# numamma/numamma

Measured on AMD Instinct MI355X. Metric: PEBS samples/s analysed (device-resident), higher is better.
Workload: dtype u64

## Files before the change

numamma_amd/csrc/nmg_engine_impl.h:

```cpp
#pragma once

#include <dlfcn.h>
#include <hip/hip_runtime.h>
#include <rccl/rccl.h>
#include <rocprofiler-sdk-roctx/roctx.h>

#include <algorithm>
#include <chrono>
#include <cinttypes>
#include <functional>
#include <cstdio>
#include <cstdlib>
#include <cstddef>
#include <cstring>
#include <condition_variable>
#include <memory>
#include <mutex>
#include <string>
#include <thread>
#include <vector>

#include "nmg_buffer.h"
#include "nmg_kernels.h"
#include "nmg_route.h"

using namespace nmg;

struct Range {
  explicit Range(const char* what) { roctxRangePushA(what); }
  ~Range() { roctxRangePop(); }
  Range(const Range&) = delete;
  Range& operator=(const Range&) = delete;
};

struct CopyPool {
  std::vector<std::thread> workers;
  std::mutex m;
  std::condition_variable wake, idle;
  std::function<void(uint32_t)> job;
  uint64_t gen = 0;
  uint32_t pending = 0;
  bool stop = false;

  explicit CopyPool(uint32_t n) {
    for (uint32_t w = 1; w < n; w++)
      workers.emplace_back([this, w] {
        uint64_t seen = 0;
        for (;;) {
          std::function<void(uint32_t)> f;
          {
            std::unique_lock<std::mutex> lk(m);
            wake.wait(lk, [&] { return stop || gen != seen; });
            if (stop) return;
            seen = gen;
            f = job;
          }
          f(w);
          std::lock_guard<std::mutex> lk(m);
          if (--pending == 0) idle.notify_one();
        }
      });
  }
  void run(const std::function<void(uint32_t)>& f) {
    {
      std::lock_guard<std::mutex> lk(m);
      job = f;
      pending = (uint32_t)workers.size();
      gen++;
    }
    wake.notify_all();
    f(0);
    std::unique_lock<std::mutex> lk(m);
    idle.wait(lk, [&] { return pending == 0; });
  }
  ~CopyPool() {
    {
      std::lock_guard<std::mutex> lk(m);
      stop = true;
    }
    wake.notify_all();
    for (auto& t : workers) t.join();
  }
};

struct nmg_engine;

struct LookupSet {
  DevBuf<uint64_t> keys;
  DevBuf<DevEntry> nodes;
  DevBuf<uint64_t> efences;
  DevBuf<DevEntry> enodes;
  DevBuf<uint64_t> ffences;
  DevBuf<uint8_t> fshift;
  DevBuf<uint2> dir;
  DevBuf<DevEntry> own_chain;
  DevEntry* chain = nullptr;
  uint32_t K = 0, elevels = 0, nb_fences = 0, fence_log2 = 0, dir_log2 = 0;
};

struct RouteTable {
  bool ok = false;
  uint32_t nparts = 0;
  DevBuf<PartInfo> d_parts;
  DevBuf<uint64_t> d_pbounds;
  DevBuf<uint16_t> d_pdir;
  DevBuf<uint32_t> d_pdead;
  DevBuf<uint64_t> d_pe_keys;
  DevBuf<uint4> d_pe_nodes;
  DevBuf<uint4> d_pe_pnode;
  DevBuf<uint4> d_pe_old;
  DevBuf<uint32_t> d_pe_oinf;
  DevBuf<uint2> d_pe_info;
  DevBuf<uint4> d_pe_dir;
  DevBuf<uint32_t> d_pe_ids;
  DevBuf<uint32_t> d_pe_lrel;
  DevBuf<uint32_t> d_pe_cmap;
};

struct RoutePool {
  DevBuf<uint4> d_rec16;
  DevBuf<uint32_t> d_cmeta;
  DevBuf<unsigned long long> d_cmatch;
  DevBuf<uint32_t> d_clist;
  DevBuf<uint4> d_items;
  DevBuf<uint32_t> d_chunk0;
  DevBuf<uint32_t> d_used;
  DevBuf<uint32_t> d_pcnt;
  DevBuf<uint32_t> d_pbase;
  DevBuf<uint32_t> d_ctl;
  DevBuf<uint4> d_ovf16;
  DevBuf<unsigned long long> d_ovfx;
};

struct EntryTable {
  std::vector<uint64_t> hist_base;
  std::vector<uint64_t> npages;
  std::vector<uint64_t> buffer_size, entry_addr;
  std::vector<nmg_object> objects;
  std::vector<DevEntry> dev_entries;
  std::vector<uint32_t> sparse_entries;
  CellCursor cur;

  uint64_t cells() const { return cur.cells; }
  void resize(uint32_t E) {
    const size_t E0 = dev_entries.size();
    hist_base.resize(E, kHistSparse);
    npages.resize(E, 1);
    buffer_size.resize(E, 0);
    entry_addr.resize(E, 0);
    objects.resize(E, nmg_object{0, 0, 0, 0});
    dev_entries.resize(E, DevEntry{0, 0, 0, 0, kHistSparse, ~0u, 0, 0, 0, 0});
    for (size_t e = E0; e < E; e++) dev_entries[e].id = (uint32_t)e;
  }
  void truncate(uint32_t E, const CellCursor& c) {
    resize(E);
    sparse_entries.resize(c.nsparse);
    cur = c;
  }
  void describe(uint32_t id, const nmg_object& o) {
    objects[id] = o;
    buffer_size[id] = o.buffer_size;
    entry_addr[id] = o.buffer_addr;
  }
  DevEntry dev_entry(uint32_t id, const nmg_object& o) const {
    DevEntry d = dev_entries[id];
    d.addr = o.buffer_addr;
    d.end = o.buffer_addr + o.buffer_size;
    d.alloc = o.alloc_date;
    d.free = o.free_date;
    return d;
  }
  Placement place(uint32_t id, uint64_t np, bool must_be_dense) {
    DevEntry& d = dev_entries[id];
    uint64_t base = kHistSparse;
    const Placement how = cur.place(np, must_be_dense, &base, &d.sidx);
    if (how == kPlaceDense) d.hist = hist_base[id] = base;
    if (how == kPlaceSparse) sparse_entries.push_back(id);
    return how;
  }
};

struct Counters {
  DevBuf<uint64_t> d_sum64, d_min64, d_max64;
  uint64_t n_sum64 = 0, n_min64 = 0, n_max64 = 0;
  void set_sizes(uint64_t E, bool levels) {
    n_sum64 = sum64_words(E, levels);
    n_min64 = min64_words(E);
    n_max64 = max64_words();
  }
  DevBuf<uint32_t> d_hist;
  DevBuf<uint64_t> d_sparse_keys;
  DevBuf<uint32_t> d_sparse_vals;
  DevBuf<uint64_t> d_objcw;
  DevBuf<uint64_t> d_sparse_ck;
  DevBuf<uint32_t> d_sparse_dirty;
  DevBuf<unsigned long long> d_pk64;
  DevBuf<uint4> d_tlog;
  DevBuf<uint32_t> d_tlog_cnt;
};

struct CellLayout {
  uint64_t E = 0, nsent = 0;
  bool meta_dirty = true;
  DevBuf<uint64_t> d_base, d_off, d_part, d_soff;
  DevBuf<uint32_t> d_np, d_cnt, d_sent;
  int ensure(nmg_engine* h, uint64_t E, uint64_t nsent);
};

struct Timeline {
  bool on = false;
  nmg_timeline_options opt{};
  uint64_t ncells = 0;
  uint32_t rounds = kTlRounds;
  DevBuf<uint32_t> d_cells;
  std::vector<uint32_t> ids, base, nrows;
  DevBuf<uint32_t> d_ids, d_base, d_nrows;
  DevBuf<uint32_t> d_cnt, d_rows;
  DevBuf<uint64_t> d_off, d_part;
  uint64_t rows_epoch = 0;
  int64_t n = 0;
};

struct nmg_engine {
  int device = 0;
  uint32_t flags = NMG_F_DEFAULT;
  uint32_t T = 1;
  hipStream_t stream = nullptr;
  hipEvent_t ev0 = nullptr, ev1 = nullptr;
  static constexpr int kRing = 64;
  hipEvent_t ring0[kRing] = {}, ring1[kRing] = {};
  hipEvent_t ringm[kRing] = {};
  hipEvent_t ringr[kRing] = {};
  uint64_t nlaunch = 0;
  int num_cus = 256;
  int blocks_per_cu = 0;
  bool launched = false;

  bool have_table = false;
  uint64_t epoch = 1, cells_epoch = 0;
  bool counters_fresh = false;
  struct HostReg {
    uintptr_t lo, hi;
    uint64_t dev;
    void* pages;
  };
  std::vector<HostReg> hostregs;
  std::vector<uint64_t> zc_dev;
  struct ResSnap {
    hipStream_t stream = nullptr;
    hipEvent_t ready = nullptr, copied = nullptr;
    bool pending = false;
    CellLayout lay;
    DevBuf<uint64_t> d_sum, d_min, d_max, d_objcw, d_found;
    DevBuf<uint32_t> d_bufcnt;
    DevBuf<uint64_t> d_ck;
    DevBuf<uint4> d_rows;
    PinBuf<uint64_t> h_sum, h_min, h_max, h_objcw, h_small, h_soff;
    PinBuf<uint32_t> h_bufcnt;
    PinBuf<uint32_t> h_rows;
    std::vector<uint32_t> sent_entry;
  } snap;
  uint64_t snap_nb = 0;
  struct CellsPrep {
    CellLayout lay;
    DevBuf<uint4> d_rows;
    int64_t n = 0;
    std::vector<uint64_t> sparse_kv, soff;
    std::vector<uint32_t> sent_entry;
  } cprep;
  uint32_t E = 0;
  LookupSet lk;
  DevBuf<DevEntry> d_entries;
  EntryTable tab;
  std::vector<uint32_t> order;
  uint64_t hist_budget = 4ull << 30;
  uint64_t sparse_cap = 1u << 20;

  Counters cnt;
  DevBuf<unsigned long long> d_found;
  DevBuf<uint64_t> d_scratch;
  DevBuf<uint32_t> d_smatch;
  Timeline tl;
  uint64_t nreset = 0;

  std::vector<BufDesc> descs;
  std::vector<uint64_t> buf_bytes;
  PinBuf<uint8_t> h_stage;
  size_t stage_len = 0;
  DevBuf<uint8_t> d_arena;
  const uint8_t* d_data = nullptr;
  bool external = false;
  bool staged_dirty = false;
  DevBuf<BufDesc> d_descs;
  DevBuf<BufDesc> d_sdescs;
  DevBuf<uint32_t> d_ranges;
  PinBuf<uint8_t> up_pin;
  size_t up_off = 0;
  hipEvent_t up_ev = nullptr;
  bool up_recorded = false;
  uint32_t sched_grid = 0;
  bool descs_dirty = false;
  bool multi_staged = false;
  DevBuf<uint32_t> d_bufcnt;
  size_t bufcnt_stride = 0;

  struct StreamSlot {
    PinBuf<uint8_t> h_stage;
    size_t len = 0;
    DevBuf<uint8_t> d_arena;
    PinBuf<uint8_t> h_sched;
    DevBuf<uint8_t> d_sched;
    std::vector<BufDesc> descs;
    hipEvent_t copied = nullptr;
    hipEvent_t done = nullptr;
    bool used = false;
  };
  bool streaming = false, streamed = false;
  uint64_t chunk_cap = 0;
  uint32_t copy_threads = 1;
  std::unique_ptr<CopyPool> pool;
  StreamSlot slots[2];
  int cur_slot = 0;
  hipStream_t copy_stream = nullptr;

  bool counts_override = false;
  std::vector<uint32_t> ov_samples, ov_found;
  std::vector<uint64_t> ov_bytes;

  std::string last_error;
  float last_ms = 0.f;

  std::vector<nmg_engine*> workers;
  std::vector<int> devices;
  bool multi = false, multi_distinct = false, multi_pending = false;
  uint64_t multi_found = 0;
  hipEvent_t merge_ev0 = nullptr, merge_ev1 = nullptr;
  bool merge_timed = false;
  uint64_t merge_bytes = 0;
  std::vector<void*> comms;
  std::vector<DevBuf<uint8_t>> warena;

  RouteTable rt;
  uint64_t route_launches = 0;
  RSeg rsegs[kRouteSegs];
  uint64_t route_tbase = 0;
  uint32_t nrsegs = 0;
  RoutePool rpool;
  bool sched_route = false;
  uint32_t route_sched_key = 0;
  bool route_pending = false;
  uint32_t route_grid = 0;
  XLayout route_xl{};

  DevBuf<uint64_t> d_dbg;
  size_t dbg_len = 0;
};

#define HIP_TRY(h, expr)                                                        \
  do {                                                                          \
    hipError_t _e = (expr);                                                     \
    if (_e != hipSuccess) {                                                     \
      (h)->last_error = std::string(#expr) + ": " + hipGetErrorString(_e);      \
      return NMG_ERR_HIP;                                                       \
    }                                                                           \
  } while (0)

struct CopyTask {
  uint8_t* dst;
  const uint8_t* src;
  uint64_t len;
};

struct RouteJob {
  const std::vector<BufDesc>* descs;
  const uint8_t* data;
  const BufDesc* sdescs;
  const uint32_t* ranges;
  const uint32_t* chunk0;
  uint32_t grid, index_base;
  bool settle_now;
};

#pragma GCC visibility push(hidden)
extern thread_local std::string g_create_error;
int fail(nmg_engine* h, int code, const std::string& msg);
int stage_h2d(nmg_engine* h, void* d_dst, const void* src, size_t n);
void stage_reset(nmg_engine* h);
void free_table(nmg_engine* h);
template <class T>
hipError_t alloc_copy(nmg_engine* h, DevBuf<T>& b, const T* src, size_t n) {
  const hipError_t e = b.alloc(n);
  if (e != hipSuccess || !n) return e;
  return hipMemcpyAsync(b, src, n * sizeof(T), hipMemcpyHostToDevice, h->stream);
}
template <class T>
hipError_t alloc_copy(nmg_engine* h, DevBuf<T>& b, const std::vector<T>& src) {
  return alloc_copy(h, b, src.data(), src.size());
}
int check_table(nmg_engine* h, const uint64_t* keys, const uint32_t* entry_off, uint32_t nb_keys,
                       uint32_t n);
int build_lookup(nmg_engine* h, LookupSet& l, const uint64_t* keys, const uint32_t* entry_off, uint32_t nb_keys,
                 const std::vector<DevEntry>& chain, DevEntry* chain_dev);
void route_segments(const uint64_t* b, uint32_t P, RSeg* seg, uint32_t* nseg, std::vector<uint16_t>& dir);
int build_partitions(nmg_engine* h, const uint64_t* keys, const uint32_t* entry_off, uint32_t K,
                            const std::vector<DevEntry>& dev, const uint32_t* ids);
int grow_entries(nmg_engine* h, uint32_t newE, const uint32_t* ids, const nmg_object* objs, uint32_t n);
int stage_reserve(nmg_engine* h, size_t need);
int append_desc(nmg_engine* h, uint64_t len, uint32_t thread_rank, uint32_t access);
uint64_t zero_copy_dev(nmg_engine* h, const void* p, uint64_t len);
int append_desc_zc(nmg_engine* h, uint64_t dev, uint64_t len, uint32_t thread_rank, uint32_t access);
int check_buffer_args(nmg_engine* h, uint64_t len, uint32_t thread_rank, uint32_t access);
void run_copies(nmg_engine* h, const std::vector<CopyTask>& tasks);
int slot_acquire(nmg_engine* h, int s);
int ensure_bufcnt(nmg_engine* h, size_t need);
int ensure_dbg(nmg_engine* h, size_t words);
int stream_flush(nmg_engine* h);
int stream_dst(nmg_engine* h, uint64_t len, uint8_t** dst, std::vector<CopyTask>* pending);
int stream_append(nmg_engine* h, uint64_t len, uint32_t thread_rank, uint32_t access);
int upload_buffers(nmg_engine* h);
void make_schedule(const std::vector<BufDesc>& descs, uint32_t grid, uint32_t index_base, BufDesc* sorted,
                          uint32_t* ranges, bool by_stream);
int build_schedule(nmg_engine* h, uint32_t grid, bool by_stream = true);
void ensure_occupancy(nmg_engine* h);
uint32_t attribution_grid(nmg_engine* h, uint32_t nb);
Params base_params(nmg_engine* h, const uint8_t* data, const BufDesc* sdescs, const uint32_t* ranges);
int launch_events(nmg_engine* h, int* slot_out);
int launch_attribution(nmg_engine* h, const uint8_t* data, const BufDesc* sdescs, const uint32_t* ranges,
                              uint32_t nb, uint32_t grid, uint64_t nbytes);
uint32_t bits_for(uint64_t v);
bool route_layout(nmg_engine* h, const std::vector<BufDesc>& descs, XLayout& xl);
bool route_eligible(nmg_engine* h, const std::vector<BufDesc>& descs);
bool route_eligible(nmg_engine* h);
int route_pool(nmg_engine* h, const std::vector<BufDesc>& descs, uint32_t grid, const uint32_t* ranges,
                      std::vector<uint32_t>& c0);
int route_prepare(nmg_engine* h, uint32_t grid, const std::vector<uint32_t>& ranges);
int route_analyze(nmg_engine* h, uint32_t nb, uint32_t grid);
int route_analyze_job(nmg_engine* h, const RouteJob& job);
int route_settle(nmg_engine* h);
int decode_error_word(nmg_engine* h, uint64_t w);
int cells_prepare(nmg_engine* h);
int cells_fill(nmg_engine* h, uint32_t* rows);
int collect_page_cells(nmg_engine* h, std::vector<uint32_t>* rows, int64_t* count);
int timeline_prepare(nmg_engine* h);
int collect_timeline_cells(nmg_engine* h, std::vector<uint32_t>* rows, int64_t* count);
void* array_ptr(nmg_engine* h, int which, size_t* bytes);
int scratch_u64(nmg_engine* h);
int sparse_nonempty(nmg_engine* h, bool* out);
int sparse_download(nmg_engine* h, std::vector<uint64_t>& k, std::vector<uint32_t>& v);
int multi_create(nmg_engine* h, const nmg_options* opt);
void multi_destroy(nmg_engine* h);
int multi_analyze(nmg_engine* h);
int multi_finish(nmg_engine* h);
int multi_buffer_found(nmg_engine* h, std::vector<uint32_t>& nf);
#pragma GCC visibility pop
```

numamma_amd/csrc/nmg_route.h:

```cpp
#pragma once

#include "nmg_kernels.h"

namespace nmg {

constexpr uint32_t kChunk = 64;
constexpr uint32_t kPartLevels = 11;
constexpr uint32_t kMaxParts = (1u << kPartLevels) - 1;
constexpr uint32_t kRouteDir = 4096;
constexpr uint32_t kRouteSegs = 8;
constexpr uint32_t kDirCntSat = 31;
struct RSeg {
  uint64_t start;
  uint32_t base;
  uint32_t nslots;
  uint32_t shift;
  uint32_t qlast;
};
constexpr uint32_t kPartKeys = 1023;
constexpr uint32_t kPartSlots = 1024;
constexpr uint32_t kPartDir = 1024;
constexpr uint32_t kDirInline = 6;
constexpr uint32_t kPnQShift = 8;
constexpr uint32_t kPnOlder = 1u << 11, kPnExact = 1u << 12;
constexpr uint32_t kOldLds = 512;
constexpr uint32_t kPnOldLds = 1u << 13, kPnOldShift = 16;
constexpr uint32_t kPartEntries = 1536;
constexpr uint32_t kPartCells = 28672;
constexpr uint32_t kItemChunks = 1023;
static_assert((uint64_t)kItemChunks * kChunk < (1ull << (64 - kPackShift)), "packed count per item");
static_assert((uint64_t)kItemChunks * kChunk < 65536u, "a u16 page cell cannot wrap within one item");
constexpr uint32_t kChunkIdBits = 25;
constexpr uint32_t kFoundLds = 16384;
constexpr uint32_t kDbgNoRoute = 0x10000;
constexpr uint32_t kDbgTinyPool = 0x20000;
constexpr uint32_t kDbgTinyOvf = 0x80000;
constexpr uint32_t kDbgLapNoWait = 0x100000;
constexpr uint32_t kDbgLocalNoWork = 0x400000;
constexpr uint32_t kDbgRouteTiming = 0x800000;
constexpr uint32_t kDbgLocalNoObj = 0x1000000;
constexpr uint32_t kDbgLocalNoPage = 0x2000000;
constexpr uint32_t kDbgLocalNoGlobal = 0x4000000;
constexpr uint32_t kDbgLocalNoSearch = 0x8000000;
constexpr uint32_t kDbgNoLines = 0x20000000;
constexpr uint32_t kDbgLocalAtomics = 0x80000000u;
constexpr uint32_t kDbgLocalTiming = 0x10000000;
constexpr int kRouteTimingWords = 16;

struct PartInfo {
  uint32_t k0, nk, e0, ne;
  uint64_t cb;
  uint32_t span;
  uint32_t dshift;
  uint32_t pages_lds;
  uint32_t cmap;
  uint32_t pad[2];
};
static_assert(sizeof(PartInfo) == 48, "PartInfo");

constexpr uint32_t kAddrBits = 40;
constexpr uint32_t kMinWeightBits = 11;
constexpr uint32_t kTsBits = 40;
struct XLayout {
  uint32_t gbits, obits, tbits, wbits;
  uint64_t wesc;
  uint64_t tbase;
};

struct RouteParams {
  Params p;
  const uint64_t* pbounds;
  const uint16_t* pdir;
  const uint32_t* pdead;
  RSeg seg[kRouteSegs];
  uint32_t nseg;
  uint32_t nparts;
  XLayout xl;
  uint64_t seq0;
  uint4* rec16;
  uint32_t* cmeta;
  const uint32_t* chunk0;
  uint32_t* used;
  uint4* ovf16;
  unsigned long long* ovfx;
  uint32_t* ovf_cnt;
  uint32_t ovf_cap;
};

struct PlanParams {
  uint32_t* pcnt;
  uint32_t* pbase;
  uint4* items;
  uint32_t* ctl;
  uint32_t grid, nparts;
};

struct ScatterParams {
  const uint32_t* cmeta;
  const uint32_t* chunk0;
  const uint32_t* used;
  const uint32_t* pcnt;
  const uint32_t* pbase;
  uint32_t* clist;
  uint32_t nparts;
};

struct LocalParams {
  Params p;
  const PartInfo* parts;
  const uint64_t* pe_keys;
  const uint4* pe_nodes;
  const uint4* pe_pnode;
  const uint4* pe_old;
  const uint32_t* pe_oinf;
  const uint2* pe_info;
  const uint4* pe_dir;
  const uint32_t* pe_ids;
  const uint32_t* pe_lrel;
  const uint32_t* pe_cmap;
  const uint4* rec16;
  const uint32_t* cmeta;
  const uint32_t* clist;
  const uint4* items;
  uint32_t* ctl;
  unsigned long long* cmatch;
  const BufDesc* descs;
  XLayout xl;
  uint64_t seq0;
  uint32_t fresh;
};

struct FoundParams {
  const uint32_t* ranges;
  const uint32_t* chunk0;
  const uint32_t* used;
  const uint32_t* cmeta;
  const unsigned long long* cmatch;
  const uint4* rec16;
  uint32_t* bufcnt;
  uint32_t nb_bufs, gbits, gshift;
};

hipError_t launch_route(uint32_t grid, hipStream_t s, const RouteParams& r);
hipError_t launch_overflow(hipStream_t s, const RouteParams& r);
struct CountParams {
  ScatterParams sc;
};
hipError_t launch_count(uint32_t grid, hipStream_t s, const CountParams& r);
hipError_t launch_plan(hipStream_t s, const PlanParams& r);
hipError_t launch_scatter(uint32_t grid, hipStream_t s, const ScatterParams& r);
hipError_t launch_local(uint32_t grid, hipStream_t s, const LocalParams& r);
hipError_t launch_found(uint32_t grid, hipStream_t s, const FoundParams& r);

}
```

numamma_amd/csrc/nmg_route.hip:

```cpp
#include <algorithm>

#include "nmg_device.h"
#include "nmg_route.h"

namespace nmg {

static_assert((uint64_t)kItemChunks * kChunk * kLaneMaxWeight < (1ull << kPackShift), "packed weight per item");


struct XRec {
  uint64_t addr, ts, w;
  uint64_t loc;
  uint32_t th, acc;
  bool esc;
  __device__ __forceinline__ uint32_t g(const XLayout& xl) const { return uint32_t(loc >> xl.obits); }
  __device__ __forceinline__ uint32_t off(const XLayout& xl) const {
    return uint32_t(loc & ((1ull << xl.obits) - 1)) << 3;
  }
};

__device__ __forceinline__ uint4 x_encode(const XLayout& xl, uint64_t pb, uint64_t addr, uint64_t ts, uint64_t w,
                                          uint32_t g, uint32_t off, uint32_t th, uint32_t acc) {
  const uint64_t ar = addr - pb, tr = ts - xl.tbase;
  const bool fit = (ar >> kAddrBits) == 0 && ts >= xl.tbase && (tr >> kTsBits) == 0 && w < xl.wesc;
  const uint64_t a = fit ? ar : 0ull, t = fit ? tr : 0ull, wq = fit ? w : xl.wesc;
  const uint64_t loc = uint64_t(off >> 3) | (uint64_t(g) << xl.obits);
  const uint64_t lo = a | (t << kAddrBits);
  const uint64_t hi = (t >> (64 - kAddrBits)) | (wq << 16) | (loc << (16 + xl.wbits)) |
                      (uint64_t(th) << (63 - xl.tbits)) | (uint64_t(acc) << 63);
  return make_uint4((uint32_t)lo, (uint32_t)(lo >> 32), (uint32_t)hi, (uint32_t)(hi >> 32));
}

__device__ __forceinline__ XRec x_decode_rel(const XLayout& xl, uint4 v) {
  XRec r;
  r.addr = u64of(v.x, v.y & 0xffu);
  r.ts = u64of(__builtin_amdgcn_alignbit(v.z, v.y, 8), (v.z >> 8) & 0xffu);
  const uint32_t wesc = (uint32_t)xl.wesc;
  r.w = __builtin_amdgcn_alignbit(v.w, v.z, 16) & wesc;
  r.esc = r.w == wesc;
  r.loc = (u64of(v.z, v.w) >> (16 + xl.wbits)) & ((1ull << (xl.obits + xl.gbits)) - 1);
  r.th = (v.w >> (31 - xl.tbits)) & ((1u << xl.tbits) - 1);
  r.acc = v.w >> 31;
  return r;
}

__device__ __forceinline__ XRec x_decode(const XLayout& xl, uint64_t pb, uint4 v) {
  XRec r = x_decode_rel(xl, v);
  r.addr += pb;
  r.ts += xl.tbase;
  return r;
}

__device__ __forceinline__ void x_resolve(XRec& r, const XLayout& xl, const uint8_t* data, const BufDesc* descs) {
  const uint64_t* q = reinterpret_cast<const uint64_t*>(data + descs[r.g(xl)].offset + r.off(xl));
  r.ts = q[1];
  r.addr = q[2];
  r.w = q[3];
}

__device__ __forceinline__ uint32_t raw_mem_lvl(const uint8_t* data, uint64_t pos) {
  return uint32_t(reinterpret_cast<const uint64_t*>(data + pos)[4] >> 5) & 0x3fff;
}

template <bool TL>
__device__ __forceinline__ void direct_attribute(const Params& p, uint64_t addr, uint64_t ts, uint64_t w, uint32_t th,
                                                 uint32_t acc, uint32_t lvl, uint64_t seq, uint32_t off,
                                                 uint32_t slot) {
  if (p.nb_keys == 0 || p.keys[0] > addr) return;
  uint32_t lo = 0, n = p.nb_keys;
  while (n > 1) {
    const uint32_t half = n >> 1;
    if (p.keys[lo + half] <= addr) {
      lo += half;
      n -= half;
    } else {
      n = half;
    }
  }
  const uint4* q = reinterpret_cast<const uint4*>(p.nodes + lo);
  const uint4 a = q[0], b = q[1], c = q[2];
  Match m;
  m.e = -1;
  m.baddr = 0;
  m.hist = kHistSparse;
  if (entry_match(a, b, addr, ts)) {
    m.e = c.w;
    m.baddr = u64of(a.x, a.y);
    m.hist = u64of(c.x, c.y);
  } else {
    const uint4 d = q[3];
    if (d.x > 1) match_older(p, d.y, d.x, addr, ts, m);
  }
  if (p.smatch) p.smatch[(p.sbufs[slot].offset + off) >> 3] = m.e >= 0 ? (uint32_t)m.e + 1u : 0u;
  if (m.e < 0) return;
  const uint64_t e = (uint64_t)m.e;
  if (p.flags & NMG_F_OBJECT_LEVELS) level_count(p, e, acc, lvl, w);
  atomicAdd(p.bufcnt + p.nb_bufs + slot, 1u);
  atomicAdd(p.found, 1ull);
  atomicAdd(reinterpret_cast<unsigned long long*>(p.sum64 + objcw_index(e, acc, 0, p.nb_entries)), 1ull);
  if (w) atomicAdd(reinterpret_cast<unsigned long long*>(p.sum64 + objcw_index(e, acc, 1, p.nb_entries)),
                   (unsigned long long)w);
  atomicMin(reinterpret_cast<unsigned long long*>(p.min64 + kFirstBase + e), (unsigned long long)((seq << 32) | off));
  if (!(p.flags & NMG_F_PAGE_HIST)) return;
  const uint32_t page = uint32_t(int(uint64_t(addr - m.baddr) / kPageSize));
  if (m.hist != kHistSparse) {
    atomicAdd(p.hist + uint64_t(th) * p.hist_cells + m.hist + page, 1u);
  } else {
    const uint32_t sidx = p.entries[e].sidx;
    if (sidx != ~0u) sparse_add(p, sparse_key(sidx, th, page), seq, off, 1u);
  }
  if (TL && p.tl) {
    const uint64_t pad = p.entries[e].pad1;
    timeline_add(p, pad != kTlNone, timeline_cell(p, pad, ts, th, page), 0);
  }
}


struct RDesc {
  uint64_t offset;
  uint32_t len, ta, pad;
  __device__ __forceinline__ uint32_t thread_rank() const { return ta & 0xffffu; }
  __device__ __forceinline__ uint32_t access() const { return ta >> 16; }
};

constexpr int kRtGroups = 7;
__device__ __forceinline__ uint32_t rt_class(uint32_t lvl) {
  const uint32_t x = lvl >> 3;
  return (lvl & LVL_HIT) ? x : (lvl & LVL_MISS) ? x << 11 : 0u;
}
constexpr uint32_t kRtMask[kRtGroups] = {1u, 2u, 4u, 8u, 16u, 0x60u, 8u << 11};
constexpr uint32_t kRtBucketNib = 0xB542130u;
constexpr uint32_t kRtKnown = 0x7fu | (8u << 11);
constexpr uint32_t kRouteDrain = 128;
constexpr uint32_t kRtOne = 1u << 24;
struct RouteAcc {
  uint32_t tot, na, g[kRtGroups];
};
__device__ __forceinline__ void racc_clear(RouteAcc& a) {
  a.tot = a.na = 0;
#pragma unroll
  for (int g = 0; g < kRtGroups; g++) a.g[g] = 0;
}

template <uint32_t ACC>
__device__ __forceinline__ void route_count(RouteAcc& a, unsigned long long (*sums)[kGlobalSums],
                                            unsigned long long (*mins)[kBuckets], unsigned long long (*maxs)[kBuckets],
                                            bool valid, uint32_t lvl, uint64_t w) {
  const uint32_t cls = rt_class(lvl);
  const bool big = w >= (1u << 16);
  const uint32_t term = (valid && !big) ? (uint32_t)w + kRtOne : 0u;
  a.tot += term;
  a.na += (valid && !big) ? (lvl & LVL_NA) : 0u;
  uint32_t gm = 0;
#pragma unroll
  for (int g = 0; g < kRtGroups; g++) {
    const bool in = (cls & kRtMask[g]) != 0;
    a.g[g] += in ? term : 0u;
    gm |= in ? 1u << g : 0u;
  }
  const uint32_t fb = gm ? (kRtBucketNib >> (4 * __builtin_ctz(gm))) & 15u : 0xffu;
  if (valid && gm && !big) {
    const unsigned long long mn = mins[ACC][fb], mx = maxs[ACC][fb];
    if (w < mn) atomicMin(&mins[ACC][fb], (unsigned long long)w);
    if (w > mx) atomicMax(&maxs[ACC][fb], (unsigned long long)w);
  }
  const bool rare = valid && (big || (cls & ~kRtKnown) || (gm & (gm - 1)));
  if (__ballot(rare)) {
    if (rare) {
      if (big) {
        atomicAdd(&sums[ACC][0], 1ull);
        atomicAdd(&sums[ACC][1], (unsigned long long)w);
        if (lvl & LVL_NA) atomicAdd(&sums[ACC][2], 1ull);
      }
      for (uint32_t m = bucket_mask(lvl); m; m &= m - 1) {
        const uint32_t bk = (uint32_t)__builtin_ctz(m);
        bool reg = false;
#pragma unroll
        for (int g = 0; g < kRtGroups; g++) reg |= ((gm >> g) & 1u) && ((kRtBucketNib >> (4 * g)) & 15u) == bk;
        if (big || !reg) {
          atomicAdd(&sums[ACC][3 + 2 * bk], 1ull);
          if (w) atomicAdd(&sums[ACC][4 + 2 * bk], (unsigned long long)w);
        }
        if (bk != fb || big) {
          atomicMin(&mins[ACC][bk], (unsigned long long)w);
          atomicMax(&maxs[ACC][bk], (unsigned long long)w);
        }
      }
    }
  }
}

__device__ __forceinline__ void racc_drain(RouteAcc& a, unsigned long long* sums, int lane) {
  if (__ballot(a.tot != 0) == 0) {
    racc_clear(a);
    return;
  }
  auto add = [&](uint32_t v, int word) {
    if (__ballot(v != 0) == 0) return;
    const uint32_t c = wave_sum_u32(v >> 24), wt = wave_sum_u32(v & (kRtOne - 1));
    if (lane == 0) {
      atomicAdd(&sums[word], (unsigned long long)c);
      if (wt) atomicAdd(&sums[word + 1], (unsigned long long)wt);
    }
  };
  add(a.tot, 0);
  const uint32_t na = wave_sum_u32(a.na);
  if (lane == 0 && na) atomicAdd(&sums[2], (unsigned long long)na);
#pragma unroll
  for (int g = 0; g < kRtGroups; g++) add(a.g[g], 3 + 2 * int((kRtBucketNib >> (4 * g)) & 15u));
  racc_clear(a);
}

struct RTimer {
  uint64_t acc[12];
  uint64_t last;
};
template <bool TIMING>
__device__ __forceinline__ void rt_stamp(RTimer& t, int i) {
  if (TIMING) {
    const uint64_t now = stamp();
    t.acc[i] += now - t.last;
    t.last = now;
  }
}

constexpr uint32_t kDescLds = 512;

__device__ __forceinline__ RDesc route_desc(const RouteParams& rp, const uint4* s_desc, uint32_t r0, uint32_t i) {
  RDesc d;
  if (i - r0 < kDescLds) {
    const uint4 l = s_desc[i - r0];
    d.offset = u64of(__builtin_amdgcn_readfirstlane(l.x), __builtin_amdgcn_readfirstlane(l.y));
    d.len = __builtin_amdgcn_readfirstlane(l.z);
    d.ta = __builtin_amdgcn_readfirstlane(l.w);
    d.pad = i;
    return d;
  }
  const BufDesc g = rp.p.sbufs[i];
  vm_drain();
  d.offset = u64of(__builtin_amdgcn_readfirstlane((uint32_t)g.offset),
                   __builtin_amdgcn_readfirstlane((uint32_t)(g.offset >> 32)));
  d.len = __builtin_amdgcn_readfirstlane(g.len);
  d.ta = __builtin_amdgcn_readfirstlane(g.thread_rank | (g.access << 16));
  d.pad = i;
  return d;
}


constexpr uint32_t kR2WG = 768;
constexpr uint32_t kLineParts = 1280;
typedef unsigned long long LineWord;
constexpr uint32_t kLwMaskShift = 24, kLwSShift = 52, kLwLineMask = 4095, kLwAhead = 8;
constexpr LineWord kLwBroken = 1ull << 28;
constexpr LineWord kLwOne = 1;
__device__ __forceinline__ uint32_t lw_count(LineWord w, uint32_t l) { return uint32_t(w >> (3 * (l & (kLwAhead - 1)))) & 7u; }
__device__ __forceinline__ uint32_t lw_s(LineWord w) { return uint32_t(w >> kLwSShift); }
__device__ __forceinline__ uint32_t lw_mask(LineWord w) { return uint32_t(w >> kLwMaskShift) & 15u; }
constexpr uint32_t kWaves = kR2WG / 64;
constexpr uint32_t kWaveWinBytes = 64 * kRecBytes;
constexpr uint32_t kNoBuf = 0xffffffffu;

__device__ __forceinline__ RDesc no_buf() {
  RDesc d;
  d.offset = 0;
  d.len = 0;
  d.ta = 0;
  d.pad = kNoBuf;
  return d;
}

__device__ __forceinline__ void wload(const uint8_t* data, uint64_t off, uint32_t len, uint32_t c, int lane,
                                      RawRec& r) {
  off = u64of(__builtin_amdgcn_readfirstlane((uint32_t)off), __builtin_amdgcn_readfirstlane((uint32_t)(off >> 32)));
  len = __builtin_amdgcn_readfirstlane(len);
  c = __builtin_amdgcn_readfirstlane(c);
  const __amdgpu_buffer_rsrc_t rs =
      __builtin_amdgcn_make_buffer_rsrc((void*)(data + off), (short)0, (int)len, 0x00020000);
  const uint32_t pos = c + uint32_t(lane) * kRecBytes;
  const uint32_t odd = (pos >> 3) & 1;
  const auto x = __builtin_amdgcn_raw_buffer_load_b128(rs, pos + (odd ? 8 : 0), 0, 0);
  const auto y = __builtin_amdgcn_raw_buffer_load_b128(rs, pos + (odd ? 24 : 16), 0, 0);
  const auto z = __builtin_amdgcn_raw_buffer_load_b64(rs, pos + (odd ? 0 : 32), 0, 0);
  r.x = make_uint4(x[0], x[1], x[2], x[3]);
  r.y = make_uint4(y[0], y[1], y[2], y[3]);
  r.z = make_uint2(z[0], z[1]);
}

struct SegL {
  uint4 a;
  uint4 b;
};
__device__ __forceinline__ uint32_t route_partition_l(const SegL* s_seg, const uint64_t* s_segst, uint32_t nseg,
                                                      const uint64_t* s_pb, const uint16_t* s_pdir, uint64_t addr) {
  uint32_t k = 0;
  uint64_t st[kRouteSegs];
#pragma unroll
  for (uint32_t j = 1; j < kRouteSegs; j++) st[j] = s_segst[j];
#pragma unroll
  for (uint32_t j = 1; j < kRouteSegs; j++) k += (uint32_t)(addr >= st[j]);
  k = min(k, nseg - 1);
  const uint4 ak = s_seg[k].a, bk = s_seg[k].b;
  const uint64_t s0 = u64of(ak.x, ak.y);
  const uint32_t base = ak.z, ns = ak.w, sh = bk.x, ql = bk.y;
  const uint64_t rel = (addr - s0) >> sh;
  const uint32_t e = s_pdir[base + (rel < ns ? (uint32_t)rel : ns - 1)];
  uint32_t q = e & 2047u;
  const uint32_t c = e >> 11;
  uint32_t n = (c == kDirCntSat ? ql - q : c) + 1;
  while (n > 1) {
    const uint32_t half = n >> 1;
    if (s_pb[q + half] <= addr) {
      q += half;
      n -= half;
    } else {
      n = half;
    }
  }
  return q;
}

constexpr uint32_t kStNone = 0xfffffu, kStOvf = 0xffffeu, kStMaxLocal = 0xffffdu;
__device__ __forceinline__ uint32_t st_cnt(uint64_t s) { return uint32_t(s) & 0xffffu; }
__device__ __forceinline__ uint32_t st_gen(uint64_t s) { return (uint32_t(s) >> 16) & 0xffu; }
__device__ __forceinline__ uint32_t st_next(uint64_t s) { return uint32_t(s >> 24) & 0xfffffu; }
__device__ __forceinline__ uint32_t st_cur(uint64_t s) { return uint32_t(s >> 44); }
__device__ __forceinline__ uint64_t st_pack(uint32_t cur, uint32_t next, uint32_t gen, uint32_t cnt) {
  return (uint64_t(cur) << 44) | (uint64_t(next) << 24) | (uint64_t(gen & 0xffu) << 16) | cnt;
}
__device__ __forceinline__ uint32_t route2_take(uint32_t& taken, uint32_t cap) {
  const uint32_t t = atomicAdd(&taken, 1u);
  return t < cap ? t : kStOvf;
}
__device__ __forceinline__ void route2_advance(unsigned long long* st, uint32_t g, uint32_t n1, uint32_t n2,
                                               bool first, unsigned long long hint) {
  unsigned long long cur = hint;
  while (true) {
    const uint32_t f = st_cnt(cur);
    const unsigned long long nw = first ? st_pack(n1, n2, g + 1, 1u)
                                        : st_pack(st_next(cur), n2, g + 1, min(f, 2 * kChunk) - kChunk);
    const unsigned long long prev = atomicCAS(st, cur, nw);
    if (prev == cur) break;
    cur = prev;
  }
}

struct Claim {
  uint64_t dst;
  uint32_t lid, waitg;
  bool ovf, ok;
};
__device__ __forceinline__ Claim route2_settle(uint64_t old, uint32_t q, unsigned long long* s_state, uint32_t& taken,
                                               uint32_t capl, uint32_t* cmeta, uint32_t c0) {
  Claim r;
  r.dst = ~0ull;
  r.lid = 0;
  r.waitg = 0;
  r.ovf = false;
  r.ok = true;
  const uint32_t f = st_cnt(old), g = st_gen(old), cu = st_cur(old), nx = st_next(old);
  if (cu != kStNone && f < 2 * kChunk) {
    const uint32_t c = f < kChunk ? cu : nx;
    if (c == kStOvf) r.ovf = true;
    else r.dst = uint64_t(c0 + c) * kChunk + (f & (kChunk - 1));
    r.lid = ((g << 6) + f) >> 2;
    if (f == kChunk + kChunk / 2) {
      const uint32_t n2 = route2_take(taken, capl);
      if (n2 != kStOvf) cmeta[c0 + n2] = q | (kChunk << 24);
      route2_advance(&s_state[q], g, n2, n2, false, old + 1);
    }
  } else if (cu == kStNone && f == 2 * kChunk) {
    const uint32_t n1 = route2_take(taken, capl);
    const uint32_t n2 = n1 == kStOvf ? kStOvf : route2_take(taken, capl);
    if (n1 != kStOvf) cmeta[c0 + n1] = q | (kChunk << 24);
    if (n2 != kStOvf) cmeta[c0 + n2] = q | (kChunk << 24);
    route2_advance(&s_state[q], g, n1, n2, true, old + 1);
    if (n1 == kStOvf) r.ovf = true;
    else r.dst = uint64_t(c0 + n1) * kChunk;
    r.lid = (g + 1) << 4;
  } else {
    r.waitg = g;
    r.ok = false;
  }
  return r;
}

struct XF {
  uint4 a;
  uint32_t q;
  uint32_t lvl;
  bool routed;
};

template <bool TIMING, bool TL>
__global__ __launch_bounds__(kR2WG, 1) void route2_kernel(RouteParams rp) {
  __shared__ uint64_t s_pb[kMaxParts + 1];
  __shared__ uint16_t s_pdir[kRouteDir];
  __shared__ uint32_t s_dead[(kMaxParts + 1) / 32];
  __shared__ unsigned long long s_state[kMaxParts + 1];
  __shared__ uint4 s_desc[kDescLds];
  __shared__ uint32_t s_wlist[kWaves][64];
  __shared__ uint32_t s_taken, s_bnext;
  __shared__ unsigned long long s_gsums[2][kGlobalSums], s_gmins[2][kBuckets], s_gmaxs[2][kBuckets];
  __shared__ SegL s_seg[kRouteSegs];
  __shared__ uint64_t s_segst[kRouteSegs];
  __shared__ uint4 s_line[kLineParts * 4];
  __shared__ LineWord s_lw[kLineParts];
  __shared__ uint32_t s_ldst[kLineParts];
  __shared__ uint2 s_tab[kWaves][64];

  Params& p = rp.p;
  const int tid = threadIdx.x;
  const int lane = tid & 63, wave = tid >> 6;
  if (tid < (int)kRouteSegs) {
    const RSeg g = rp.seg[tid];
    s_seg[tid].a = make_uint4((uint32_t)g.start, (uint32_t)(g.start >> 32), g.base, g.nslots);
    s_seg[tid].b = make_uint4(g.shift, g.qlast, 0, 0);
    s_segst[tid] = tid < rp.nseg ? g.start : ~0ull;
  }
  const uint32_t nseg = rp.nseg;
  const uint64_t first_start = rp.seg[0].start;
  const uint32_t P = rp.nparts;
  const uint32_t c0 = rp.chunk0[blockIdx.x];
  const uint32_t cap = rp.chunk0[blockIdx.x + 1] - c0;
  const uint32_t capl = min(cap, kStMaxLocal + 1);
  for (uint32_t i = tid; i < kMaxParts + 1; i += kR2WG) s_pb[i] = rp.pbounds[i];
  for (uint32_t i = tid; i < kRouteDir; i += kR2WG) s_pdir[i] = rp.pdir[i];
  if (tid < (int)((kMaxParts + 1) / 32)) s_dead[tid] = rp.pdead[tid];
  for (uint32_t i = tid; i < P; i += kR2WG) s_state[i] = st_pack(kStNone, kStNone, 0, 2 * kChunk);
  const uint32_t nlp = !(p.flags & kDbgNoLines) ? min(P, kLineParts) : 0u;
  for (uint32_t i = tid; i < nlp; i += kR2WG) s_lw[i] = LineWord(kChunk / 4) << kLwSShift;
  const uint32_t ahead_max = (p.flags & kDbgLapNoWait) ? 1u : kLwAhead;
  const uint32_t r0 = p.ranges[blockIdx.x], r1 = p.ranges[blockIdx.x + 1];
  for (uint32_t i = r0 + tid; i < r1 && i - r0 < kDescLds; i += kR2WG) {
    const BufDesc d = p.sbufs[i];
    s_desc[i - r0] = make_uint4((uint32_t)d.offset, (uint32_t)(d.offset >> 32), d.len, d.thread_rank | (d.access << 16));
  }
  if (tid == 0) {
    s_taken = 0;
    s_bnext = r0;
  }
  if (tid < (int)kGlobalSums) s_gsums[0][tid] = s_gsums[1][tid] = 0;
  if (tid < (int)kBuckets) {
    s_gmins[0][tid] = s_gmins[1][tid] = ~0ull;
    s_gmaxs[0][tid] = s_gmaxs[1][tid] = 0;
  }
  RouteAcc gacc[2];
  racc_clear(gacc[0]);
  racc_clear(gacc[1]);
  uint32_t gwin = 0;
  lds_sync();

  if (r0 < r1) {
    auto dequeue = [&](RDesc& d) {
      uint32_t i = 0;
      if (lane == 0) i = atomicAdd(&s_bnext, 1u);
      i = __builtin_amdgcn_readfirstlane(i);
      if (i < r1) d = route_desc(rp, s_desc, r0, i);
      else d = no_buf();
    };
    RDesc d0, d1 = no_buf();
    dequeue(d0);
    bool have1 = false;
    uint32_t cur = 0;
    uint32_t ns = 0;
    uint32_t pidx, pcur;
    uint64_t eoff;
    uint32_t elen;
    auto predict = [&]() {
      if (d0.pad == kNoBuf) {
        pidx = kNoBuf;
        pcur = 0;
        eoff = 0;
        elen = 0;
      } else if (cur + kWaveWinBytes < d0.len) {
        pidx = d0.pad;
        pcur = cur + kWaveWinBytes;
        eoff = d0.offset;
        elen = d0.len;
      } else {
        if (!have1) {
          dequeue(d1);
          have1 = true;
        }
        pidx = d1.pad;
        pcur = 0;
        eoff = d1.offset;
        elen = d1.len;
      }
    };
    RawRec ra, rb;
    wload(p.data, d0.offset, d0.len, 0, lane, ra);
    predict();
    wload(p.data, eoff, elen, pcur, lane, rb);

    RTimer rt;
#pragma unroll
    for (int k = 0; k < 12; k++) rt.acc[k] = 0;
    rt.last = TIMING ? stamp() : 0;
    uint32_t nwin = 0;

    auto uni = [&](RDesc& d) {
      d.offset = u64of(__builtin_amdgcn_readfirstlane((uint32_t)d.offset),
                       __builtin_amdgcn_readfirstlane((uint32_t)(d.offset >> 32)));
      d.len = __builtin_amdgcn_readfirstlane(d.len);
      d.ta = __builtin_amdgcn_readfirstlane(d.ta);
      d.pad = __builtin_amdgcn_readfirstlane(d.pad);
    };
    auto front = [&](RawRec& A, RawRec& B, XF& X) {
      uni(d0);
      uni(d1);
      cur = __builtin_amdgcn_readfirstlane(cur);
      ns = __builtin_amdgcn_readfirstlane(ns);
      const RDesc dw = d0;
      const uint32_t pos = cur + uint32_t(lane) * kRecBytes;
      const bool cand = pos < dw.len;
      if (TIMING) {
        asm volatile("s_waitcnt vmcnt(3)" ::: "memory");
        nwin++;
      }
      rt_stamp<TIMING>(rt, 0);
      Rec rec = decode_rec(A, pos);
      const bool bad = cand && (uint64_t(pos) + kRecBytes > dw.len || (rec.hdr >> 48) != kRecBytes);
      bool valid;
      uint32_t roff = pos, ncur;
      if (!__ballot(bad) && !(cur & 7)) {
        valid = cand && uint32_t(rec.hdr) == kSampleType;
        ncur = cur + kWaveWinBytes;
      } else {
        const uint8_t* base = p.data + dw.offset;
        const uint64_t len = dw.len;
        uint64_t q0 = cur;
        uint32_t n = 0, err = 0;
        if (cur & 7) err = kErrUnaligned;
        while (!err && q0 < len && n < 64) {
          const uint64_t q = q0 + uint64_t(lane) * kRecBytes;
          const uint64_t hdr = (q + 8 <= len) ? *reinterpret_cast<const uint64_t*>(base + q) : 0;
          const bool reg = q + kRecBytes <= len && (hdr >> 48) == kRecBytes;
          const uint64_t rm = __ballot(reg);
          const uint32_t run = ~rm ? (uint32_t)__builtin_ctzll(~rm) : 64u;
          const uint32_t take = min(run, 64u - n);
          const bool smp = (uint32_t)lane < take && uint32_t(hdr) == kSampleType;
          const uint64_t sm = __ballot(smp);
          if (smp) s_wlist[wave][n + (uint32_t)__popcll(sm & ((1ull << lane) - 1))] = (uint32_t)q;
          n += (uint32_t)__popcll(sm);
          q0 += uint64_t(take) * kRecBytes;
          if (take < run || run == 64 || q0 >= len || n >= 64) continue;
          if (q0 + 8 > len) {
            err = kErrTruncated;
            break;
          }
          const uint64_t h = (uint64_t)__shfl(hdr, (int)run, 64);
          const uint32_t size = uint32_t(h >> 48);
          if (size == 0) {
            err = kErrZeroSize;
            break;
          }
          if (size & 7) {
            err = kErrUnaligned;
            break;
          }
          if (uint32_t(h) == kSampleType) {
            if (q0 + kRecBytes > len || q0 + size > len) {
              err = kErrTruncated;
              break;
            }
            if (lane == 0) s_wlist[wave][n] = (uint32_t)q0;
            n++;
          }
          q0 += size;
        }
        if (err && lane == 0) set_error(p, rp.seq0 + dw.pad, (uint32_t)q0, err);
        __builtin_amdgcn_fence(__ATOMIC_RELEASE, "wavefront", "local");
        __builtin_amdgcn_wave_barrier();
        __builtin_amdgcn_fence(__ATOMIC_ACQUIRE, "wavefront", "local");
        ncur = err ? (uint32_t)len : (uint32_t)min(q0, len);
        valid = (uint32_t)lane < n;
        roff = valid ? s_wlist[wave][lane] : 0u;
        RawRec rr;
        load_rec(base, roff, valid ? len : 0, rr);
        rec = decode_rec(rr, roff);
        vm_drain();
      }
      ns += (uint32_t)__popcll(__ballot(valid));
      if (dw.pad != kNoBuf) {
        if (ncur >= dw.len) {
          if (lane == 0 && ns) atomicAdd(p.bufcnt + dw.pad, ns);
          ns = 0;
          cur = 0;
          if (have1) {
            d0 = d1;
          } else {
            dequeue(d0);
          }
          have1 = false;
          d1 = no_buf();
        } else {
          cur = ncur;
        }
      }
      if (d0.pad != pidx || (d0.pad != kNoBuf && cur != pcur)) {
        wload(p.data, d0.offset, d0.len, cur, lane, B);
        vm_drain();
      }
      predict();
      wload(p.data, eoff, elen, pcur, lane, A);

      rt_stamp<TIMING>(rt, 1);
      const uint32_t acc_l = dw.access();
      if (acc_l == 0) {
        route_count<0>(gacc[0], s_gsums, s_gmins, s_gmaxs, valid, uint32_t(rec.dsrc >> 5) & 0x3fff, rec.w);
      } else {
        route_count<1>(gacc[1], s_gsums, s_gmins, s_gmaxs, valid, uint32_t(rec.dsrc >> 5) & 0x3fff, rec.w);
      }
      if (++gwin == kRouteDrain) {
        racc_drain(gacc[0], s_gsums[0], lane);
        racc_drain(gacc[1], s_gsums[1], lane);
        gwin = 0;
      }
      rt_stamp<TIMING>(rt, 2);
      bool routed = valid && rec.addr >= first_start;
      const uint32_t q = routed ? route_partition_l(s_seg, s_segst, nseg, s_pb, s_pdir, rec.addr) : 0u;
      routed = routed && (rec.ts == 0 || !((s_dead[q >> 5] >> (q & 31)) & 1u));
      if (TIMING) (void)__builtin_amdgcn_readfirstlane(__ballot(q != 0));
      rt_stamp<TIMING>(rt, 3);
      X.a = make_uint4(0, 0, 0, 0);
      X.q = q;
      X.lvl = uint32_t(rec.dsrc >> 5) & 0x3fff;
      X.routed = routed;
      if (routed) X.a = x_encode(rp.xl, s_pb[q], rec.addr, rec.ts, rec.w, dw.pad, roff, dw.thread_rank(), acc_l);
      rt_stamp<TIMING>(rt, 4);
    };

    auto back = [&](const XF& X) {
      uint64_t dst = ~0ull;
      uint32_t lid = 0;
      bool ovf = false, todo = false;
      uint32_t waitg = 0;
      const bool lined = X.routed && X.q < nlp;
      const LineWord lw = lined ? s_lw[X.q] : LineWord(0);
      const unsigned long long old = X.routed ? atomicAdd(&s_state[X.q], 1ull) : 0ull;
      auto settle = [&](unsigned long long st) {
        const Claim c = route2_settle(st, X.q, s_state, s_taken, capl, rp.cmeta, c0);
        dst = c.dst;
        lid = c.lid;
        ovf = c.ovf;
        waitg = c.waitg;
        todo = !c.ok;
      };
      if (X.routed) settle(old);
      {
        bool spin = todo;
        while (__ballot(todo)) {
          if (!todo) continue;
          if (!spin) {
            settle(atomicAdd(&s_state[X.q], 1ull));
            spin = todo;
          } else {
            const uint64_t st = __hip_atomic_load(&s_state[X.q], __ATOMIC_RELAXED, __HIP_MEMORY_SCOPE_WORKGROUP);
            spin = st_gen(st) == waitg;
          }
        }
      }
      rt_stamp<TIMING>(rt, 5);
      bool staged = false, counts = false;
      if (__ballot(lined)) {
        lid &= kLwLineMask;
        const uint32_t j = (uint32_t)dst & 3u, S = lw_s(lw), ahead = (lid - S) & kLwLineMask;
        counts = lined && !(lw & kLwBroken) && ahead < ahead_max;
        staged = counts && ahead == 0 && dst != ~0ull;
        if (lined && !(lw & kLwBroken) && ahead >= ahead_max) atomicOr(&s_lw[X.q], kLwBroken);
        if (staged) {
          s_line[X.q * 4 + j] = X.a;
          s_ldst[X.q] = (uint32_t)(dst >> 2);
        }
        __builtin_amdgcn_fence(__ATOMIC_RELEASE, "workgroup", "local");
        LineWord o = 0;
        if (counts)
          o = atomicAdd(&s_lw[X.q], (kLwOne << (3 * (lid & (kLwAhead - 1)))) +
                                        (staged ? kLwOne << (kLwMaskShift + j) : LineWord(0)));
        const bool done = counts && lw_count(o, lid) == 3 && lw_s(o) == lid;
        const uint32_t dmask = counts ? lw_mask(o) | (staged ? 1u << j : 0u) : 0u;
        if (TIMING) rt.acc[8] += (uint64_t)__popcll(__ballot(counts && !staged));
        const uint64_t dm = __ballot(done);
        if (dm) {
          if (done)
            s_tab[wave][__popcll(dm & ((1ull << lane) - 1))] =
                make_uint2(X.q | (dmask << 11) | (lid << 16), (uint32_t)(dst >> 2));
          __builtin_amdgcn_fence(__ATOMIC_RELEASE, "wavefront", "local");
          __builtin_amdgcn_wave_barrier();
          __builtin_amdgcn_fence(__ATOMIC_ACQUIRE, "wavefront", "local");
          const uint32_t nd = (uint32_t)__popcll(dm);
          auto piece_done = [&](uint2 t, uint32_t k) {
            __builtin_amdgcn_fence(__ATOMIC_RELEASE, "workgroup", "local");
            if (k == 0) {
              const uint32_t tq = t.x & 2047u;
              uint32_t l = t.x >> 16, m = (t.x >> 11) & 15u;
              while (true) {
                const LineWord ow = atomicAdd(&s_lw[tq], (kLwOne << kLwSShift) - (LineWord(4) << (3 * (l & (kLwAhead - 1)))) -
                                                            (LineWord(m) << kLwMaskShift));
                l = (l + 1) & kLwLineMask;
                if (lw_count(ow, l) != 4) break;
                m = 0;
              }
            }
          };
          for (uint32_t j0 = 0; j0 < nd; j0 += 16) {
            const uint32_t jj = j0 + ((uint32_t)lane >> 2);
            if (jj < nd) {
              const uint2 t = s_tab[wave][jj];
              const uint32_t tq = t.x & 2047u, tm = (t.x >> 11) & 15u, k = lane & 3;
              if ((tm >> k) & 1) rp.rec16[uint64_t(t.y) * 4 + k] = s_line[tq * 4 + k];
              piece_done(t, k);
            }
          }
          __builtin_amdgcn_fence(__ATOMIC_RELEASE, "wavefront", "local");
          __builtin_amdgcn_wave_barrier();
          __builtin_amdgcn_fence(__ATOMIC_ACQUIRE, "wavefront", "local");
        }
      }
      rt_stamp<TIMING>(rt, 9);
      const bool straight = dst != ~0ull && !counts;
      const bool alone = straight || (counts && !staged && dst != ~0ull);
      if (alone) rp.rec16[dst] = X.a;
      if (TIMING) {
        rt.acc[6] += (uint64_t)__popcll(__ballot(staged));
        rt.acc[7] += (uint64_t)__popcll(__ballot(straight));
      }
      if (__ballot(ovf)) {
        if (ovf) {
          const uint64_t pbq = s_pb[X.q];
          const uint32_t o = atomicAdd(rp.ovf_cnt, 1u);
          if (o < rp.ovf_cap) {
            rp.ovf16[o] = X.a;
            rp.ovfx[o] = pbq;
          } else {
            XRec xr = x_decode(rp.xl, pbq, X.a);
            if (xr.esc) x_resolve(xr, rp.xl, p.data, p.sbufs);
            direct_attribute<TL>(p, xr.addr, xr.ts, xr.w, xr.th, xr.acc, X.lvl, rp.seq0 + xr.g(rp.xl), xr.off(rp.xl),
                             xr.g(rp.xl));
          }
        }
        vm_drain();
      }
      rt_stamp<TIMING>(rt, 10);
    };

    XF X;
    do {
      front(ra, rb, X);
      back(X);
      front(rb, ra, X);
      back(X);
    } while (d0.pad != kNoBuf);

    if (TIMING && lane == 0) {
      unsigned long long* o = p.dbg + (uint64_t(blockIdx.x) * (kWG / 64) + tid / 64) * kRouteTimingWords;
      for (int k = 0; k < 9; k++) o[k] = rt.acc[k];
      o[9] = nwin;
      uint32_t nb = 0;
      if (wave == 0)
        for (uint32_t q = 0; q < nlp; q++) nb += (s_lw[q] & kLwBroken) ? 1u : 0u;
      o[10] = nb;
      o[11] = rt.acc[9];
      o[12] = rt.acc[10];
    }
  }
  racc_drain(gacc[0], s_gsums[0], lane);
  racc_drain(gacc[1], s_gsums[1], lane);
  lds_sync();
#pragma unroll
  for (uint32_t a = 0; a < 2; a++) {
    if (tid < (int)kGlobalSums && s_gsums[a][tid])
      atomicAdd(reinterpret_cast<unsigned long long*>(p.sum64 + gsum_index(a, tid)), s_gsums[a][tid]);
    if (tid < (int)kBuckets && s_gsums[a][3 + 2 * tid]) {
      atomicMin(reinterpret_cast<unsigned long long*>(p.min64 + a * kBuckets + tid), s_gmins[a][tid]);
      atomicMax(reinterpret_cast<unsigned long long*>(p.max64 + a * kBuckets + tid), s_gmaxs[a][tid]);
    }
  }
  for (uint32_t q = tid; q < P; q += kR2WG) {
    const unsigned long long st = s_state[q];
    const uint32_t f = st_cnt(st), cu = st_cur(st), nx = st_next(st);
    if (cu == kStNone) continue;
    if (cu != kStOvf) rp.cmeta[c0 + cu] = q | (min(f, kChunk) << 24);
    if (nx != kStOvf) rp.cmeta[c0 + nx] = q | ((f > kChunk ? f - kChunk : 0u) << 24);
    if (q < nlp) {
      const uint32_t m = lw_mask(s_lw[q]);
      for (uint32_t j = 0; j < 4; j++)
        if ((m >> j) & 1u) rp.rec16[uint64_t(s_ldst[q]) * 4 + j] = s_line[q * 4 + j];
    }
  }
  if (tid == 0) rp.used[blockIdx.x] = min(s_taken, capl);
}


__global__ __launch_bounds__(256) void overflow_kernel(RouteParams rp) {
  const uint32_t n = min(*rp.ovf_cnt, rp.ovf_cap);
  for (uint32_t i = blockIdx.x * 256 + threadIdx.x; i < n; i += gridDim.x * 256) {
    XRec xr = x_decode(rp.xl, rp.ovfx[i], rp.ovf16[i]);
    if (xr.esc) x_resolve(xr, rp.xl, rp.p.data, rp.p.sbufs);
    const uint32_t lvl = (rp.p.flags & NMG_F_OBJECT_LEVELS)
                             ? raw_mem_lvl(rp.p.data, rp.p.sbufs[xr.g(rp.xl)].offset + xr.off(rp.xl))
                             : 0u;
    direct_attribute<true>(rp.p, xr.addr, xr.ts, xr.w, xr.th, xr.acc, lvl, rp.seq0 + xr.g(rp.xl), xr.off(rp.xl),
                     xr.g(rp.xl));
  }
}


__global__ __launch_bounds__(kWG) void count_kernel(CountParams cp) {
  __shared__ uint32_t s_cnt[kMaxParts + 1];
  const ScatterParams& r = cp.sc;
  const uint32_t tid = threadIdx.x, w = blockIdx.x, P = r.nparts;
  for (uint32_t q = tid; q < P; q += kWG) s_cnt[q] = 0;
  __syncthreads();
  const uint32_t c0 = r.chunk0[w], n = r.used[w];
  constexpr uint32_t kU = 8;
  for (uint32_t b = 0; b < n; b += kU * kWG) {
    uint32_t m[kU];
#pragma unroll
    for (uint32_t u = 0; u < kU; u++) {
      const uint32_t i = b + u * kWG + tid;
      m[u] = i < n ? r.cmeta[c0 + i] : 0u;
    }
#pragma unroll
    for (uint32_t u = 0; u < kU; u++)
      if (m[u] >> 24) atomicAdd(&s_cnt[m[u] & 0xffffffu], 1u);
  }
  __syncthreads();
  uint32_t* out = const_cast<uint32_t*>(r.pcnt) + uint64_t(w) * P;
  for (uint32_t q = tid; q < P; q += kWG) out[q] = s_cnt[q];
}

constexpr uint32_t kPlanRowGroups = kWG / 64;
__global__ __launch_bounds__(kWG) void plan_cols_kernel(PlanParams r) {
  __shared__ uint32_t s_sum[kPlanRowGroups][64];
  const uint32_t tid = threadIdx.x, c = tid & 63, rg = tid >> 6;
  const uint32_t P = r.nparts, q = blockIdx.x * 64 + c;
  const uint32_t per = (r.grid + kPlanRowGroups - 1) / kPlanRowGroups, w0 = rg * per;
  constexpr uint32_t kU = 16;
  uint32_t sum = 0;
  for (uint32_t b = 0; b < per; b += kU) {
    uint32_t v[kU];
#pragma unroll
    for (uint32_t u = 0; u < kU; u++) {
      const uint32_t w = w0 + b + u;
      v[u] = (q < P && b + u < per && w < r.grid) ? r.pcnt[uint64_t(w) * P + q] : 0u;
    }
#pragma unroll
    for (uint32_t u = 0; u < kU; u++) sum += v[u];
  }
  s_sum[rg][c] = sum;
  __syncthreads();
  uint32_t run = 0;
  for (uint32_t g = 0; g < rg; g++) run += s_sum[g][c];
  for (uint32_t b = 0; b < per; b += kU) {
    uint32_t v[kU];
#pragma unroll
    for (uint32_t u = 0; u < kU; u++) {
      const uint32_t w = w0 + b + u;
      v[u] = (q < P && b + u < per && w < r.grid) ? r.pcnt[uint64_t(w) * P + q] : 0u;
    }
#pragma unroll
    for (uint32_t u = 0; u < kU; u++) {
      const uint32_t w = w0 + b + u;
      if (q < P && b + u < per && w < r.grid) r.pcnt[uint64_t(w) * P + q] = run;
      run += v[u];
    }
  }
  if (q < P && rg == kPlanRowGroups - 1) r.pbase[q] = run;
}

__global__ __launch_bounds__(kWG) void plan_kernel(PlanParams r) {
  __shared__ uint32_t s_tot[kMaxParts + 1], s_nit[kMaxParts + 1], s_wsum[2][kWG / 64];
  const int tid = threadIdx.x, lane = tid & 63, wave = tid >> 6;
  const uint32_t P = r.nparts;
  for (uint32_t q = tid; q < P; q += kWG) {
    const uint32_t run = r.pbase[q];
    s_tot[q] = run;
    s_nit[q] = (run + kItemChunks - 1) / kItemChunks;
  }
  __syncthreads();
  const uint32_t i0 = 2 * (uint32_t)tid;
  const uint32_t t0 = i0 < P ? s_tot[i0] : 0u, t1 = i0 + 1 < P ? s_tot[i0 + 1] : 0u;
  const uint32_t n0 = i0 < P ? s_nit[i0] : 0u, n1 = i0 + 1 < P ? s_nit[i0 + 1] : 0u;
  uint32_t it = t0 + t1, in = n0 + n1;
#pragma unroll
  for (int o = 1; o < 64; o <<= 1) {
    const uint32_t a = __shfl_up(it, o, 64), b = __shfl_up(in, o, 64);
    if (lane >= o) {
      it += a;
      in += b;
    }
  }
  if (lane == 63) {
    s_wsum[0][wave] = it;
    s_wsum[1][wave] = in;
  }
  __syncthreads();
  uint32_t wt = 0, wn = 0;
  for (int w2 = 0; w2 < wave; w2++) {
    wt += s_wsum[0][w2];
    wn += s_wsum[1][w2];
  }
  const uint32_t tb = wt + it - (t0 + t1), nb = wn + in - (n0 + n1);
  for (uint32_t k = 0; k < 2; k++) {
    const uint32_t q = i0 + k;
    if (q >= P) break;
    const uint32_t base = tb + (k ? t0 : 0u), ibase = nb + (k ? n0 : 0u), tot = k ? t1 : t0;
    r.pbase[q] = base;
    for (uint32_t j = 0; j * kItemChunks < tot; j++)
      r.items[ibase + j] = make_uint4(q, base + j * kItemChunks, base + min(tot, (j + 1) * kItemChunks),
                                      tot <= kItemChunks ? 1u : 0u);
  }
  if (tid == kWG - 1) {
    r.ctl[0] = wn + in;
    r.ctl[1] = 0;
    r.ctl[3] = r.ctl[2];
    r.ctl[2] = 0;
  }
}

__global__ __launch_bounds__(kWG) void scatter_kernel(ScatterParams r) {
  __shared__ uint32_t s_cnt[kMaxParts + 1];
  const uint32_t tid = threadIdx.x, w = blockIdx.x, P = r.nparts;
  const uint32_t* off = r.pcnt + uint64_t(w) * P;
  for (uint32_t q = tid; q < P; q += kWG) s_cnt[q] = r.pbase[q] + off[q];
  __syncthreads();
  const uint32_t c0 = r.chunk0[w], n = r.used[w];
  constexpr uint32_t kU = 8;
  for (uint32_t b = 0; b < n; b += kU * kWG) {
    uint32_t m[kU];
#pragma unroll
    for (uint32_t u = 0; u < kU; u++) {
      const uint32_t i = b + u * kWG + tid;
      m[u] = i < n ? r.cmeta[c0 + i] : 0u;
    }
#pragma unroll
    for (uint32_t u = 0; u < kU; u++) {
      if (!(m[u] >> 24)) continue;
      const uint32_t k = atomicAdd(&s_cnt[m[u] & 0xffffffu], 1u);
      r.clist[k] = (c0 + b + u * kWG + tid) | ((m[u] >> 24) << kChunkIdBits);
    }
  }
}


constexpr uint32_t kLWG = 1024;
constexpr int kLC = 2;

template <typename T>
__device__ __forceinline__ T l2_load(const T* p) {
  return __hip_atomic_load(p, __ATOMIC_RELAXED, __HIP_MEMORY_SCOPE_AGENT);
}

__device__ __forceinline__ uint64_t entry_id(const LocalParams& lp, uint32_t pos) {
  return lp.pe_ids ? lp.pe_ids[pos] : pos;
}

__device__ __forceinline__ int32_t match_older_pos(const Params& p, uint32_t first, uint32_t count, uint64_t addr,
                                                   uint64_t ts, uint64_t& baddr, uint64_t& hist) {
  for (uint32_t j = first + 1; j < first + count; j++) {
    const uint4* r = reinterpret_cast<const uint4*>(p.chain + j);
    const uint4 ra = r[0], rb = r[1];
    if (entry_match(ra, rb, addr, ts)) {
      const uint4 rc = r[2];
      baddr = u64of(ra.x, ra.y);
      hist = u64of(rc.x, rc.y);
      return (int32_t)j;
    }
  }
  return -1;
}

template <bool TIMING, bool PACKED, bool EXTRA>
__global__ __launch_bounds__(kLWG, 1) void local_kernel(LocalParams lp) {
  __shared__ uint64_t s_keys[kPartSlots];
  __shared__ uint4 s_pn[kPartSlots];
  __shared__ uint2 s_info[kPartSlots];
  __shared__ uint4 s_dir[kPartDir];
  __shared__ uint4 s_old[kOldLds];
  __shared__ uint32_t s_oinf[kOldLds];
  __shared__ unsigned long long s_owt[2][kPartEntries];
  __shared__ unsigned long long s_first[kPartEntries];
  __shared__ uint32_t s_pg[kPartCells / 2];
  __shared__ uint32_t s_clist[kItemChunks];
  __shared__ uint32_t s_item, s_cnext, s_nfound, s_big, s_took;
  __shared__ uint4 s_nx[4];

  Params& p = lp.p;
  const int tid = threadIdx.x, lane = tid & 63;
  const uint32_t nitems = lp.ctl[0];
  const uint32_t T = p.nb_threads;
  const bool pages = (p.flags & NMG_F_PAGE_HIST) != 0;
  RTimer rt;
#pragma unroll
  for (int k = 0; k < 12; k++) rt.acc[k] = 0;
  rt.last = TIMING ? stamp() : 0;
  uint32_t nchunks = 0, nit = 0;
  uint64_t textra = 0;
  uint32_t nfound = 0;
  if (tid == 0) s_nfound = 0;
  for (uint32_t i = tid; i < kPartEntries; i += kLWG) {
    s_owt[0][i] = s_owt[1][i] = 0;
    s_first[i] = ~0ull;
  }
  for (uint32_t i = tid; i < kPartCells / 2; i += kLWG) s_pg[i] = 0;
  static_assert(sizeof(PartInfo) == 48, "PartInfo: three uint4");
  auto take_next = [&]() {
    uint32_t idx = 0;
    if (lane == 0) idx = atomicAdd(lp.ctl + 1, 1u);
    idx = __builtin_amdgcn_readfirstlane(idx);
    if (lane == 0) s_item = idx;
    if (idx < nitems) {
      const uint4 nx = lp.items[idx];
      const uint32_t nq = __builtin_amdgcn_readfirstlane(nx.x);
      if (lane == 0) s_nx[0] = nx;
      if (lane < 3) s_nx[1 + lane] = reinterpret_cast<const uint4*>(lp.parts + nq)[lane];
    }
  };
  if (tid < 64) take_next();
  if (tid == 0) s_took = 0;
  while (true) {
    lds_sync();
    const uint32_t it = __builtin_amdgcn_readfirstlane(s_item);
    rt_stamp<TIMING>(rt, 6);
    if (it >= nitems) break;
    nit++;
    const uint4 item = s_nx[0];
    const uint32_t q = __builtin_amdgcn_readfirstlane(item.x);
    PartInfo pi;
    {
      uint4* pw = reinterpret_cast<uint4*>(&pi);
      pw[0] = s_nx[1];
      pw[1] = s_nx[2];
      pw[2] = s_nx[3];
    }
    const uint32_t dshift = __builtin_amdgcn_readfirstlane(pi.dshift);
    {
      static_assert(kPartKeys <= kLWG && kPartDir == kLWG && kOldLds <= kLWG, "one table element per thread");
      constexpr uint32_t kClPer = (kItemChunks + kLWG - 1) / kLWG;
      const uint32_t nk = pi.nk, nold = min(pi.ne - nk, kOldLds), ncl = item.z - item.y;
      uint64_t key = 0;
      uint4 pn = make_uint4(0, 0, 0, 0), od = pn;
      uint2 inf = make_uint2(0, 0);
      uint32_t oi = 0, cl[kClPer];
      if (tid < nk) {
        key = lp.pe_keys[uint64_t(q) * kPartSlots + tid];
        pn = lp.pe_pnode[uint64_t(q) * kPartSlots + tid];
        inf = lp.pe_info[uint64_t(q) * kPartSlots + tid];
      }
      const uint4 dd = lp.pe_dir[uint64_t(q) * kPartDir + tid];
      if (tid < nold) {
        od = lp.pe_old[uint64_t(q) * kOldLds + tid];
        oi = lp.pe_oinf[uint64_t(q) * kOldLds + tid];
      }
#pragma unroll
      for (uint32_t u = 0; u < kClPer; u++) cl[u] = tid + u * kLWG < ncl ? lp.clist[item.y + tid + u * kLWG] : 0u;
      if (tid < nk) {
        s_keys[tid] = key;
        s_pn[tid] = pn;
        s_info[tid] = inf;
      }
      s_dir[tid] = dd;
      if (tid < nold) {
        s_old[tid] = od;
        s_oinf[tid] = oi;
      }
#pragma unroll
      for (uint32_t u = 0; u < kClPer; u++)
        if (tid + u * kLWG < ncl) s_clist[tid + u * kLWG] = cl[u];
    }
    if (tid == 0) {
      s_cnext = 0;
      s_took = 0;
    }
    const uint32_t ncell = (pages && pi.pages_lds) ? T * pi.span : 0u;
    const bool excl = item.w != 0 && !(p.flags & kDbgLocalAtomics);
    if (tid == 0) s_big = 0;
    lds_sync();
    const uint64_t k0key = u64of(__builtin_amdgcn_readfirstlane((uint32_t)s_keys[0]),
                                 __builtin_amdgcn_readfirstlane((uint32_t)(s_keys[0] >> 32)));
    rt_stamp<TIMING>(rt, 7);

    const uint32_t nl = item.z - item.y;
    auto chunk_load = [&](uint32_t l, uint4& a) {
      const uint32_t e = l < nl ? s_clist[l] : 0u;
      a = lp.rec16[uint64_t(e & ((1u << kChunkIdBits) - 1)) * kChunk + lane];
    };
    auto process = [&](uint32_t l0, const uint4 (&a16)[kLC]) {
      uint32_t li[kLC];
      bool valid[kLC];
      uint64_t addr[kLC], ts[kLC], w[kLC];
      XRec xr[kLC];
#pragma unroll
      for (int j = 0; j < kLC; j++) {
        li[j] = l0 + j;
        const uint32_t fill = li[j] < nl ? s_clist[li[j]] >> kChunkIdBits : 0u;
        valid[j] = (uint32_t)lane < fill;
      }
      if (TIMING) {
        asm volatile("s_waitcnt vmcnt(2)" ::: "memory");
        nchunks += kLC;
      }
      rt_stamp<TIMING>(rt, 0);
      if (p.flags & kDbgLocalNoWork) {
#pragma unroll
        for (int j = 0; j < kLC; j++)
          if (lane == 0 && li[j] < nl)
            lp.cmatch[s_clist[li[j]] & ((1u << kChunkIdBits) - 1)] = a16[j].x ^ a16[j].y ^ a16[j].z ^ a16[j].w;
        return;
      }
      bool esc = false;
#pragma unroll
      for (int j = 0; j < kLC; j++) {
        xr[j] = x_decode_rel(lp.xl, a16[j]);
        esc |= valid[j] && xr[j].esc;
      }
      if (__ballot(esc)) {
#pragma unroll
        for (int j = 0; j < kLC; j++)
          if (valid[j] && xr[j].esc) {
            x_resolve(xr[j], lp.xl, p.data, lp.descs);
            xr[j].addr -= k0key;
          }
        vm_drain();
      }
#pragma unroll
      for (int j = 0; j < kLC; j++) {
        addr[j] = xr[j].addr;
        ts[j] = xr[j].ts;
        w[j] = valid[j] ? xr[j].w : 0ull;
      }
      rt_stamp<TIMING>(rt, 1);
      int32_t r[kLC];
      uint32_t sa[kLC], sn[kLC];
#pragma unroll
      for (int j = 0; j < kLC; j++) {
        r[j] = -1;
        sa[j] = sn[j] = 0;
        if (valid[j]) {
          const uint32_t slot = (uint32_t)min(addr[j] >> dshift, (uint64_t)(kPartDir - 1));
          const uint4 de = s_dir[slot];
          const uint32_t lo = de.x & 1023u, n = (de.x >> 10) & 2047u;
          uint32_t a = lo, m = n;
          if (n && ((de.x >> 21) & 1u)) {
            const uint64_t rs64 = addr[j] - (uint64_t(slot) << dshift);
            const uint32_t rs = rs64 >> 16 ? 0x10000u : (uint32_t)rs64;
            const uint32_t c = (uint32_t)((de.y & 0xffffu) <= rs) + (uint32_t)((de.y >> 16) <= rs) +
                               (uint32_t)((de.z & 0xffffu) <= rs) + (uint32_t)((de.z >> 16) <= rs) +
                               (uint32_t)((de.w & 0xffffu) <= rs) + (uint32_t)((de.w >> 16) <= rs);
            a = lo + min(c, n);
            m = (c == kDirInline && n > kDirInline) ? n - kDirInline : 0u;
          }
          sa[j] = a;
          sn[j] = m;
          r[j] = 0;
        }
      }
      if (TIMING) {
#pragma unroll
        for (int j = 0; j < kLC; j++) rt.acc[11] += (uint64_t)__popcll(__ballot(sn[j] != 0));
      }
#pragma unroll
      for (int j = 0; j < kLC; j++) {
        uint32_t a = sa[j], n = sn[j];
        while (n) {
          const uint32_t half = (n + 1) >> 1;
          if (s_keys[a + half] - k0key <= addr[j]) {
            a += half;
            n -= half;
          } else {
            n = half - 1;
          }
        }
        if (r[j] >= 0) r[j] = (int32_t)a;
      }
      if (TIMING) {
        bool any = false;
#pragma unroll
        for (int j = 0; j < kLC; j++) any |= r[j] >= 0;
        (void)__builtin_amdgcn_readfirstlane(__ballot(any));
      }
      rt_stamp<TIMING>(rt, 2);
      int32_t erel[kLC];
      uint64_t pofs[kLC];
      uint32_t hrel[kLC], pnw[kLC], tq[kLC];
      bool older[kLC], amb[kLC];
#pragma unroll
      for (int j = 0; j < kLC; j++) {
        erel[j] = -1;
        pofs[j] = 0;
        hrel[j] = kEmpty32;
        older[j] = false;
        amb[j] = false;
        pnw[j] = 0;
        tq[j] = __builtin_amdgcn_alignbit((uint32_t)(ts[j] >> 32), (uint32_t)ts[j], kPnQShift);
        if (r[j] >= 0 && !(p.flags & kDbgLocalNoSearch)) {
          const uint4 pn = s_pn[r[j]];
          const uint2 inf = s_info[r[j]];
          pnw[j] = pn.w;
          const bool in = addr[j] >= (uint64_t)inf.y && addr[j] < (uint64_t)pn.x;
          amb[j] = xr[j].esc || (pn.w & kPnExact) || (in && (tq[j] == pn.y || tq[j] == pn.z));
          if (!amb[j] && in && tq[j] > pn.y && tq[j] < pn.z) {
            erel[j] = (int32_t)(pn.w & 2047u);
            pofs[j] = addr[j] - inf.y;
            hrel[j] = inf.x;
          } else if (!amb[j]) {
            older[j] = (pn.w & kPnOlder) != 0;
          }
        }
      }
      bool anyamb = false;
#pragma unroll
      for (int j = 0; j < kLC; j++) {
        anyamb |= amb[j];
        if (TIMING) rt.acc[10] += (uint64_t)__popcll(__ballot(amb[j]));
      }
      if (__ballot(anyamb)) {
#pragma unroll
        for (int j = 0; j < kLC; j++) {
          if (!amb[j]) continue;
          const uint64_t fa = k0key + addr[j], ft = xr[j].esc ? ts[j] : lp.xl.tbase + ts[j];
          const uint4* gq = lp.pe_nodes + (uint64_t(q) * kPartSlots + (uint32_t)r[j]) * 2;
          const uint4 na = gq[0], nb = gq[1];
          if (entry_match(na, nb, fa, ft)) {
            erel[j] = (int32_t)(s_pn[r[j]].w & 2047u);
            pofs[j] = fa - u64of(na.x, na.y);
            hrel[j] = s_info[r[j]].x;
          } else {
            older[j] = (s_pn[r[j]].w & kPnOlder) != 0;
          }
        }
        vm_drain();
      }
      bool anyold = false;
#pragma unroll
      for (int j = 0; j < kLC; j++) anyold |= older[j];
      if (__ballot(anyold)) {
#pragma unroll
        for (int j = 0; j < kLC; j++) {
          if (!older[j] || xr[j].esc || !(pnw[j] & kPnOldLds)) continue;
          const uint32_t e = pnw[j] & 2047u, base = e - (uint32_t)r[j], c = (pnw[j] >> kPnOldShift) & 2047u;
          bool glob = false;
          for (uint32_t i = 0; i < c; i++) {
            const uint4 o = s_old[base + i];
            const bool in = addr[j] >= (uint64_t)o.w && addr[j] < (uint64_t)o.x;
            if (in && (tq[j] == o.y || tq[j] == o.z)) {
              glob = true;
              break;
            }
            if (in && tq[j] > o.y && tq[j] < o.z) {
              erel[j] = (int32_t)(e + 1 + i);
              pofs[j] = addr[j] - o.w;
              hrel[j] = s_oinf[base + i];
              break;
            }
          }
          older[j] = glob;
        }
        anyold = false;
#pragma unroll
        for (int j = 0; j < kLC; j++) anyold |= older[j];
      }
      if (__ballot(anyold)) {
#pragma unroll
        for (int j = 0; j < kLC; j++) {
          if (!older[j]) continue;
          const uint64_t fa = k0key + addr[j], ft = xr[j].esc ? ts[j] : lp.xl.tbase + ts[j];
          const uint4 d = reinterpret_cast<const uint4*>(p.nodes + pi.k0 + (uint32_t)r[j])[3];
          uint64_t hist = kHistSparse, baddr = 0;
          const int32_t pos = match_older_pos(p, d.y, d.x, fa, ft, baddr, hist);
          if (pos >= 0) {
            erel[j] = pos - (int32_t)pi.e0;
            pofs[j] = fa - baddr;
            hrel[j] = hist == kHistSparse ? kEmpty32
                      : PACKED && pi.cmap != ~0u ? lp.pe_lrel[pos]
                                         : (uint32_t)(hist - pi.cb);
          }
        }
        vm_drain();
      }
      {
        uint64_t mine = 0;
        uint32_t ml = 0;
#pragma unroll
        for (int j = 0; j < kLC; j++) {
          const uint64_t fm = __ballot(erel[j] >= 0);
          nfound += (uint32_t)__popcll(fm);
          mine = lane == j ? fm : mine;
          ml = lane == j ? li[j] : ml;
        }
        if (lane < kLC && ml < nl) lp.cmatch[s_clist[ml] & ((1u << kChunkIdBits) - 1)] = mine;
      }
      rt_stamp<TIMING>(rt, 3);
      const bool noobj = (p.flags & kDbgLocalNoObj) != 0;
#pragma unroll
      for (int j = 0; j < kLC; j++) {
        bool ok = erel[j] >= 0 && !noobj && w[j] < kLaneMaxWeight;
        if (ok) atomicAdd(&s_owt[xr[j].acc][erel[j]], (1ull << kPackShift) | w[j]);
      }
      bool anybig = false;
#pragma unroll
      for (int j = 0; j < kLC; j++) anybig |= erel[j] >= 0 && w[j] >= kLaneMaxWeight;
      if (__ballot(anybig) && !noobj) {
        if (lane == 0) s_big = 1;
#pragma unroll
        for (int j = 0; j < kLC; j++) {
          if (erel[j] < 0 || w[j] < kLaneMaxWeight) continue;
          const uint64_t e = entry_id(lp, pi.e0 + (uint32_t)erel[j]);
          atomicAdd(reinterpret_cast<unsigned long long*>(p.sum64 + objcw_index(e, xr[j].acc, 0, p.nb_entries)), 1ull);
          atomicAdd(reinterpret_cast<unsigned long long*>(p.sum64 + objcw_index(e, xr[j].acc, 1, p.nb_entries)),
                    (unsigned long long)w[j]);
        }
        vm_drain();
      }
      if (!noobj) {
        unsigned long long cur[kLC];
#pragma unroll
        for (int j = 0; j < kLC; j++) cur[j] = erel[j] >= 0 ? s_first[erel[j]] : 0ull;
#pragma unroll
        for (int j = 0; j < kLC; j++)
          if (erel[j] >= 0 && xr[j].loc < cur[j]) atomicMin(&s_first[erel[j]], (unsigned long long)xr[j].loc);
      }
      rt_stamp<TIMING>(rt, 4);
      if (pages && !(p.flags & kDbgLocalNoPage)) {
        uint32_t page[kLC];
        bool glob = false;
#pragma unroll
        for (int j = 0; j < kLC; j++) {
          page[j] = uint32_t(int(pofs[j] / kPageSize));
          if (erel[j] >= 0 && hrel[j] != kEmpty32 && ncell) {
            const uint32_t c = xr[j].th * pi.span + hrel[j] + page[j], sh = 16 * (c & 1);
            atomicAdd(&s_pg[c >> 1], 1u << sh);
          }
          glob |= erel[j] >= 0 && (hrel[j] == kEmpty32 || !ncell);
        }
        if (__ballot(glob)) {
#pragma unroll
          for (int j = 0; j < kLC; j++) {
            if (erel[j] < 0) continue;
            if (hrel[j] != kEmpty32 && !ncell) {
              atomicAdd(p.hist + uint64_t(xr[j].th) * p.hist_cells + pi.cb + hrel[j] + page[j], 1u);
            } else if (hrel[j] == kEmpty32) {
              const uint32_t sidx = p.entries[entry_id(lp, pi.e0 + (uint32_t)erel[j])].sidx;
              if (sidx != ~0u)
                sparse_add(p, sparse_key(sidx, xr[j].th, page[j]), lp.seq0 + xr[j].g(lp.xl), xr[j].off(lp.xl), 1u);
            }
          }
          vm_drain();
        }
      }
      rt_stamp<TIMING>(rt, 5);
      if (EXTRA) {
        const bool lev = (p.flags & NMG_F_OBJECT_LEVELS) != 0;
        const bool tlon = p.tl != nullptr;
        bool need[kLC], any = false;
#pragma unroll
        for (int j = 0; j < kLC; j++) {
          need[j] = valid[j] && (p.smatch != nullptr || ((lev || tlon) && erel[j] >= 0));
          any |= need[j];
        }
        if (__ballot(any)) {
          uint64_t eid[kLC];
          uint32_t lvl[kLC];
          bool row[kLC];
#pragma unroll
          for (int j = 0; j < kLC; j++) {
            eid[j] = 0;
            lvl[j] = 0;
            row[j] = false;
            if (!need[j]) continue;
            const uint64_t pos = lp.descs[xr[j].g(lp.xl)].offset + xr[j].off(lp.xl);
            const bool hit = erel[j] >= 0;
            if (hit) eid[j] = entry_id(lp, pi.e0 + (uint32_t)erel[j]);
            if (p.smatch) p.smatch[pos >> 3] = hit ? (uint32_t)eid[j] + 1u : 0u;
            if (lev && hit) {
              lvl[j] = raw_mem_lvl(p.data, pos);
              row[j] = true;
            }
          }
          if (lev) {
#pragma unroll
            for (int j = 0; j < kLC; j++) {
              const uint32_t key = ((uint32_t)erel[j] << 15) | (xr[j].acc << 14) | lvl[j];
              const bool small = row[j] && w[j] < kLaneMaxWeight;
              uint64_t todo = __ballot(small);
              while (todo) {
                const uint32_t lead = __builtin_amdgcn_readfirstlane((uint32_t)__builtin_ctzll(todo));
                const uint32_t k = (uint32_t)__builtin_amdgcn_readlane((int)key, (int)lead);
                const bool same = small && key == k;
                const uint64_t sm = __ballot(same);
                const uint32_t ws = wave_sum_u32(same ? (uint32_t)w[j] : 0u);
                if ((uint32_t)lane == lead)
                  level_count(p, eid[j], xr[j].acc, lvl[j], ws, (unsigned long long)__popcll(sm));
                todo &= ~sm;
              }
              if (row[j] && !small) level_count(p, eid[j], xr[j].acc, lvl[j], w[j]);
            }
          }
          if (tlon) {
            uint64_t pad[kLC];
#pragma unroll
            for (int j = 0; j < kLC; j++)
              pad[j] = need[j] && erel[j] >= 0 ? p.entries[eid[j]].pad1 : kTlNone;
#pragma unroll
            for (int j = 0; j < kLC; j++) {
              const uint64_t ft = xr[j].esc ? ts[j] : lp.xl.tbase + ts[j];
              timeline_add(p, pad[j] != kTlNone,
                           timeline_cell(p, pad[j], ft, xr[j].th, uint32_t(int(pofs[j] / kPageSize))), p.tl_rounds);
            }
          }
          vm_drain();
        }
        if (TIMING) {
          const uint64_t now = stamp();
          textra += now - rt.last;
          rt.last = now;
        }
      }
    };
    uint4 A[kLC], B[kLC];
    auto grab = [&]() -> uint32_t {
      uint32_t t = 0;
      if (lane == 0) t = atomicAdd(&s_cnext, (uint32_t)kLC);
      return __builtin_amdgcn_readfirstlane(t);
    };
    uint32_t la = grab(), lb = grab();
#pragma unroll
    for (int j = 0; j < kLC; j++) chunk_load(la + j, A[j]);
#pragma unroll
    for (int j = 0; j < kLC; j++) chunk_load(lb + j, B[j]);
    while (la < nl) {
      process(la, A);
      la = grab();
#pragma unroll
      for (int j = 0; j < kLC; j++) chunk_load(la + j, A[j]);
      if (lb < nl) process(lb, B);
      lb = grab();
#pragma unroll
      for (int j = 0; j < kLC; j++) chunk_load(lb + j, B[j]);
    }
    uint32_t won = 0;
    if (lane == 0) won = atomicExch(&s_took, 1u) == 0 ? 1u : 0u;
    if (__builtin_amdgcn_readfirstlane(won)) take_next();
    lds_sync();
    rt_stamp<TIMING>(rt, 9);
    const bool clean =excl && lp.fresh && __builtin_amdgcn_readfirstlane(lp.ctl[3]) == 0;
    const bool clean_obj = clean && __builtin_amdgcn_readfirstlane(s_big) == 0;
    for (uint32_t i = tid; i < pi.ne; i += kLWG) {
      const uint64_t e = entry_id(lp, pi.e0 + i);
#pragma unroll
      for (uint32_t a = 0; a < 2; a++) {
        const uint64_t v = s_owt[a][i];
        if (!v) continue;
        s_owt[a][i] = 0;
        const uint64_t cnt = v >> kPackShift, wt = v & ((1ull << kPackShift) - 1);
        uint64_t* pc = p.sum64 + objcw_index(e, a, 0, p.nb_entries);
        uint64_t* pw = p.sum64 + objcw_index(e, a, 1, p.nb_entries);
        if (clean_obj) {
          *pc = cnt;
          if (wt) *pw = wt;
        } else if (excl) {
          *pc = l2_load(pc) + cnt;
          if (wt) *pw = l2_load(pw) + wt;
        } else {
          atomicAdd(reinterpret_cast<unsigned long long*>(pc), (unsigned long long)cnt);
          if (wt) atomicAdd(reinterpret_cast<unsigned long long*>(pw), (unsigned long long)wt);
        }
      }
      const uint64_t floc = s_first[i];
      if (floc != ~0ull) {
        s_first[i] = ~0ull;
        const uint64_t fo = ((lp.seq0 + (floc >> lp.xl.obits)) << 32) | ((floc & ((1ull << lp.xl.obits) - 1)) << 3);
        uint64_t* pf = p.min64 + kFirstBase + e;
        if (clean) *pf = fo;
        else if (excl) *pf = min(l2_load(pf), fo);
        else atomicMin(reinterpret_cast<unsigned long long*>(pf), (unsigned long long)fo);
      }
    }
    {
      const uint32_t nw = (ncell + 1) / 2, span = pi.span;
      const uint32_t cmap = PACKED ? __builtin_amdgcn_readfirstlane(pi.cmap) : ~0u;
      const uint32_t smag = span ? 0xffffffffu / span + 1u : 0u;
      constexpr uint32_t kU = 4;
      for (uint32_t j0 = tid; j0 < nw; j0 += kU * kLWG) {
        uint32_t cnt[kU][2], old[kU][2];
        uint32_t* pc[kU][2];
#pragma unroll
        for (uint32_t u = 0; u < kU; u++) {
          const uint32_t j = j0 + u * kLWG;
          const uint32_t v = j < nw ? s_pg[j] : 0u;
          if (v) s_pg[j] = 0;
#pragma unroll
          for (uint32_t h = 0; h < 2; h++) {
            cnt[u][h] = (v >> (16 * h)) & 0xffffu;
            const uint32_t li = 2 * j + h, th = __umulhi(li, smag), rel = li - th * span;
            uint64_t cell = pi.cb + rel;
            if (cmap != ~0u) cell = cnt[u][h] ? lp.pe_cmap[cmap + rel] : 0u;
            pc[u][h] = p.hist + uint64_t(th) * p.hist_cells + cell;
            old[u][h] = (excl && !clean && cnt[u][h]) ? l2_load(pc[u][h]) : 0u;
          }
        }
#pragma unroll
        for (uint32_t u = 0; u < kU; u++)
#pragma unroll
          for (uint32_t h = 0; h < 2; h++) {
            if (!cnt[u][h]) continue;
            if (excl) *pc[u][h] = old[u][h] + cnt[u][h];
            else atomicAdd(pc[u][h], cnt[u][h]);
          }
      }
    }
    lds_sync();
    rt_stamp<TIMING>(rt, 8);
  }
  if (lane == 0 && nfound) atomicAdd(&s_nfound, nfound);
  lds_sync();
  if (tid == 0 && s_nfound) atomicAdd(p.found, (unsigned long long)s_nfound);
  if (TIMING && lane == 0) {
    unsigned long long* o = p.dbg + (uint64_t(blockIdx.x) * (kWG / 64) + tid / 64) * kRouteTimingWords;
    for (int k = 0; k < 9; k++) o[k] = rt.acc[k];
    o[9] = nchunks;
    o[10] = nit;
    o[11] = rt.acc[9];
    o[12] = rt.acc[10];
    o[13] = rt.acc[11];
    o[14] = textra;
  }
}


__global__ __launch_bounds__(kWG) void found_kernel(FoundParams r) {
  __shared__ uint32_t s_found[kFoundLds];
  const int tid = threadIdx.x, lane = tid & 63;
  const uint32_t w = blockIdx.x;
  const uint32_t g0 = r.ranges[w], nbuf = r.ranges[w + 1] - g0, nl = min(nbuf, kFoundLds);
  for (uint32_t i = tid; i < nl; i += kWG) s_found[i] = 0;
  __syncthreads();
  const uint64_t k0 = uint64_t(r.chunk0[w]) * kChunk, k1 = k0 + uint64_t(r.used[w]) * kChunk;
  const uint64_t gmask = (1ull << r.gbits) - 1;
  constexpr int kU = 4;
  for (uint64_t k = k0 + tid; k < k1; k += kU * kWG) {
    uint64_t bits[kU], xw[kU];
#pragma unroll
    for (int u = 0; u < kU; u++) {
      const uint64_t kk = k + u * kWG;
      bits[u] = kk < k1 && (r.cmeta[kk / kChunk] >> 24) ? r.cmatch[kk / kChunk] : 0ull;
      xw[u] = ((bits[u] >> lane) & 1) ? reinterpret_cast<const uint64_t*>(r.rec16)[2 * kk + 1] >> r.gshift : 0ull;
    }
#pragma unroll
    for (int u = 0; u < kU; u++) {
      if (!((bits[u] >> lane) & 1)) continue;
      const uint32_t g = (uint32_t)(xw[u] & gmask);
      if (g - g0 < nl) atomicAdd(&s_found[g - g0], 1u);
      else atomicAdd(r.bufcnt + r.nb_bufs + g, 1u);
    }
  }
  __syncthreads();
  for (uint32_t i = tid; i < nl; i += kWG)
    if (s_found[i]) atomicAdd(r.bufcnt + r.nb_bufs + g0 + i, s_found[i]);
}


hipError_t launch_route(uint32_t grid, hipStream_t s, const RouteParams& r) {
  const bool timing = (r.p.flags & kDbgRouteTiming) != 0, tl = r.p.tl != nullptr;
  if (timing && tl) hipLaunchKernelGGL((route2_kernel<true, true>), dim3(grid), dim3(kR2WG), 0, s, r);
  else if (timing) hipLaunchKernelGGL((route2_kernel<true, false>), dim3(grid), dim3(kR2WG), 0, s, r);
  else if (tl) hipLaunchKernelGGL((route2_kernel<false, true>), dim3(grid), dim3(kR2WG), 0, s, r);
  else hipLaunchKernelGGL((route2_kernel<false, false>), dim3(grid), dim3(kR2WG), 0, s, r);
  return hipGetLastError();
}

hipError_t launch_plan(hipStream_t s, const PlanParams& r) {
  if (r.nparts) hipLaunchKernelGGL(plan_cols_kernel, dim3((r.nparts + 63) / 64), dim3(kWG), 0, s, r);
  hipLaunchKernelGGL(plan_kernel, dim3(1), dim3(kWG), 0, s, r);
  return hipGetLastError();
}

hipError_t launch_overflow(hipStream_t s, const RouteParams& r) {
  hipLaunchKernelGGL(overflow_kernel, dim3(1024), dim3(256), 0, s, r);
  return hipGetLastError();
}

hipError_t launch_count(uint32_t grid, hipStream_t s, const CountParams& r) {
  hipLaunchKernelGGL(count_kernel, dim3(grid), dim3(kWG), 0, s, r);
  return hipGetLastError();
}

hipError_t launch_scatter(uint32_t grid, hipStream_t s, const ScatterParams& r) {
  hipLaunchKernelGGL(scatter_kernel, dim3(grid), dim3(kWG), 0, s, r);
  return hipGetLastError();
}

template <bool TIMING, bool PACKED>
static void launch_local_as(bool extra, uint32_t grid, hipStream_t s, const LocalParams& r) {
  if (extra) hipLaunchKernelGGL((local_kernel<TIMING, PACKED, true>), dim3(grid), dim3(kLWG), 0, s, r);
  else hipLaunchKernelGGL((local_kernel<TIMING, PACKED, false>), dim3(grid), dim3(kLWG), 0, s, r);
}

hipError_t launch_local(uint32_t grid, hipStream_t s, const LocalParams& r) {
  const bool timing = (r.p.flags & kDbgLocalTiming) != 0, packed = r.pe_cmap != nullptr;
  const bool extra = (r.p.flags & NMG_F_OBJECT_LEVELS) != 0 || r.p.smatch != nullptr || r.p.tl != nullptr;
  if (packed) {
    if (timing) launch_local_as<true, true>(extra, grid, s, r);
    else launch_local_as<false, true>(extra, grid, s, r);
  } else {
    if (timing) launch_local_as<true, false>(extra, grid, s, r);
    else launch_local_as<false, false>(extra, grid, s, r);
  }
  return hipGetLastError();
}

hipError_t launch_found(uint32_t grid, hipStream_t s, const FoundParams& r) {
  hipLaunchKernelGGL(found_kernel, dim3(grid), dim3(kWG), 0, s, r);
  return hipGetLastError();
}

}
```

numamma_amd/csrc/nmg_route_host.hip:

```cpp
#include "nmg_engine_impl.h"


uint32_t bits_for(uint64_t v) {
  uint32_t b = 0;
  while (b < 64 && (v >> b) != 0) b++;
  return b;
}

bool route_layout(nmg_engine* h, const std::vector<BufDesc>& descs, XLayout& xl) {
  uint64_t maxlen = 1;
  for (const BufDesc& d : descs) maxlen = std::max<uint64_t>(maxlen, d.len);
  xl.gbits = bits_for(descs.size() - 1);
  xl.obits = bits_for((maxlen - 1) / 8);
  xl.tbits = bits_for(h->T - 1);
  const uint32_t loc = xl.gbits + xl.obits + xl.tbits + 1;
  if (loc > 48 - kMinWeightBits || xl.gbits > 31 || xl.obits > 31 || xl.tbits > 31) return false;
  xl.wbits = std::min<uint32_t>(48 - loc, 16);
  xl.wesc = (1ull << xl.wbits) - 1;
  xl.tbase = h->route_tbase;
  return true;
}

bool route_eligible(nmg_engine* h, const std::vector<BufDesc>& descs) {
  constexpr uint32_t kLegacyOnly = kDbgLoadOnly | kDbgNoGlobal | kDbgNoFlush | kDbgNoTables | kDbgTiming |
                                   kDbgTinyLog | kDbgNoPack | kDbgNoDir | kDbgNoRoute | NMG_F_SINGLE_PASS;
  if (!h->rt.ok || (h->flags & kLegacyOnly) || descs.empty()) return false;
  uint64_t bytes = 0;
  for (size_t i = 0; i < descs.size(); i++) {
    if (descs[i].seq != descs[0].seq + i) return false;
    bytes += descs[i].len;
  }
  const uint64_t chunks = (bytes / kRecBytes + descs.size()) / kChunk + (uint64_t)h->num_cus * (2 * h->rt.nparts + 2);
  if (chunks >= (1ull << kChunkIdBits)) return false;
  XLayout xl;
  return route_layout(h, descs, xl);
}
bool route_eligible(nmg_engine* h) { return route_eligible(h, h->descs); }

int route_pool(nmg_engine* h, const std::vector<BufDesc>& descs, uint32_t grid, const uint32_t* ranges,
                      std::vector<uint32_t>& c0) {
  const uint32_t P = h->rt.nparts;
  c0.assign(grid + 1, 0);
  uint64_t tot = 0;
  for (uint32_t w = 0; w < grid; w++) {
    uint64_t rec = 0;
    for (uint32_t b = ranges[w]; b < ranges[w + 1]; b++) rec += (descs[b].len + kRecBytes - 1) / kRecBytes;
    const uint64_t cap = (h->flags & kDbgTinyPool) ? 2 : (rec + kChunk - 1) / kChunk + 2 * P;
    c0[w] = (uint32_t)tot;
    tot += cap;
  }
  c0[grid] = (uint32_t)tot;
  if (tot >= (1ull << kChunkIdBits)) return fail(h, NMG_ERR_RANGE, "partition-first chunk pool too large");
  const size_t items = tot / kItemChunks + P + 1;
  uint64_t recs = 0;
  for (const BufDesc& d : descs) recs += (d.len + kRecBytes - 1) / kRecBytes;
  const size_t ovf = (size_t)((h->flags & kDbgTinyPool) ? recs : recs / 4 + std::min<uint64_t>(3 * recs, 4u << 20)) + 65536;
  RoutePool& rp = h->rpool;
  if (tot > rp.d_cmeta.cap() || items > rp.d_items.cap() || grid > rp.d_used.cap() || ovf > rp.d_ovfx.cap()) {
    HIP_TRY(h, hipStreamSynchronize(h->stream));
    rp = RoutePool();
    const size_t cap = std::max<size_t>(tot, 1);
    HIP_TRY(h, rp.d_rec16.alloc(cap * kChunk));
    HIP_TRY(h, rp.d_cmeta.alloc(cap));
    HIP_TRY(h, rp.d_cmatch.alloc(cap));
    HIP_TRY(h, rp.d_clist.alloc(cap));
    HIP_TRY(h, rp.d_items.alloc(items));
    HIP_TRY(h, rp.d_chunk0.alloc(grid + 1));
    HIP_TRY(h, rp.d_used.alloc(grid));
    HIP_TRY(h, rp.d_pcnt.alloc((size_t)grid * (kMaxParts + 1)));
    HIP_TRY(h, rp.d_pbase.alloc(kMaxParts + 1));
    HIP_TRY(h, rp.d_ctl.alloc(4));
    HIP_TRY(h, hipMemset(rp.d_ctl, 0, 4 * 4));
    HIP_TRY(h, rp.d_ovf16.alloc(ovf));
    HIP_TRY(h, rp.d_ovfx.alloc(ovf));
  }
  return NMG_OK;
}

int route_prepare(nmg_engine* h, uint32_t grid, const std::vector<uint32_t>& ranges) {
  std::vector<uint32_t> c0;
  const int rc = route_pool(h, h->descs, grid, ranges.data(), c0);
  if (rc) return rc;
  const int rc2 = stage_h2d(h, h->rpool.d_chunk0, c0.data(), (grid + 1) * 4);
  if (rc2) return rc2;
  h->route_sched_key = h->rt.nparts | ((h->flags & kDbgTinyPool) ? 0x80000000u : 0u);
  return NMG_OK;
}


int route_analyze(nmg_engine* h, uint32_t nb, uint32_t grid) {
  (void)nb;
  RouteJob job{&h->descs, h->d_data, h->d_sdescs, h->d_ranges, h->rpool.d_chunk0, grid, 0, false};
  return route_analyze_job(h, job);
}

int route_analyze_job(nmg_engine* h, const RouteJob& job) {
  Range range("nmg_route");
  XLayout xl;
  if (!route_layout(h, *job.descs, xl)) return fail(h, NMG_ERR_STATE, "route layout");
  const uint32_t grid = job.grid;
  Params base = base_params(h, job.data, job.sdescs, job.ranges);
  base.bufcnt = h->d_bufcnt + job.index_base;
  const uint64_t seq0 = (*job.descs)[0].seq;
  h->route_launches++;
  int slot = 0;
  int rc = launch_events(h, &slot);
  if (rc) return rc;
  HIP_TRY(h, hipEventRecord(h->ring0[slot], h->stream));
  RouteParams rp;
  memset(&rp, 0, sizeof(rp));
  rp.p = base;
  rp.pbounds = h->rt.d_pbounds;
  rp.pdir = h->rt.d_pdir;
  rp.pdead = h->rt.d_pdead;
  for (uint32_t k = 0; k < kRouteSegs; k++) rp.seg[k] = h->rsegs[k];
  rp.nseg = h->nrsegs;
  rp.nparts = h->rt.nparts;
  rp.xl = xl;
  rp.seq0 = seq0;
  rp.rec16 = h->rpool.d_rec16;
  rp.cmeta = h->rpool.d_cmeta;
  rp.chunk0 = job.chunk0;
  rp.used = h->rpool.d_used;
  rp.ovf16 = h->rpool.d_ovf16;
  rp.ovfx = h->rpool.d_ovfx;
  rp.ovf_cnt = h->rpool.d_ctl + 2;
  rp.ovf_cap = (uint32_t)std::min<size_t>(h->rpool.d_ovfx.cap(), 0xffffffffu);
  if (h->flags & kDbgTinyOvf) rp.ovf_cap = std::min<uint32_t>(rp.ovf_cap, 64);
  if (h->flags & kDbgRouteTiming) {
    rc = ensure_dbg(h, (size_t)grid * (kWG / 64) * kRouteTimingWords);
    if (rc) return rc;
    rp.p.dbg = reinterpret_cast<unsigned long long*>(h->d_dbg.get());
  }
  HIP_TRY(h, launch_route(grid, h->stream, rp));
  HIP_TRY(h, hipEventRecord(h->ringr[slot], h->stream));
  HIP_TRY(h, launch_overflow(h->stream, rp));
  ScatterParams sc;
  sc.cmeta = h->rpool.d_cmeta;
  sc.chunk0 = job.chunk0;
  sc.used = h->rpool.d_used;
  sc.pcnt = h->rpool.d_pcnt;
  sc.pbase = h->rpool.d_pbase;
  sc.clist = h->rpool.d_clist;
  sc.nparts = h->rt.nparts;
  CountParams cp;
  memset(&cp, 0, sizeof(cp));
  cp.sc = sc;
  HIP_TRY(h, launch_count(grid, h->stream, cp));
  PlanParams pl;
  pl.pcnt = h->rpool.d_pcnt;
  pl.pbase = h->rpool.d_pbase;
  pl.items = h->rpool.d_items;
  pl.ctl = h->rpool.d_ctl;
  pl.grid = grid;
  pl.nparts = h->rt.nparts;
  HIP_TRY(h, launch_plan(h->stream, pl));
  HIP_TRY(h, launch_scatter(grid, h->stream, sc));
  LocalParams lp;
  memset(&lp, 0, sizeof(lp));
  lp.p = base;
  lp.parts = h->rt.d_parts;
  lp.pe_keys = h->rt.d_pe_keys;
  lp.pe_nodes = h->rt.d_pe_nodes;
  lp.pe_info = h->rt.d_pe_info;
  lp.pe_pnode = h->rt.d_pe_pnode;
  lp.pe_old = h->rt.d_pe_old;
  lp.pe_oinf = h->rt.d_pe_oinf;
  lp.pe_dir = h->rt.d_pe_dir;
  lp.pe_ids = h->rt.d_pe_ids;
  lp.pe_lrel = h->rt.d_pe_lrel;
  lp.pe_cmap = h->rt.d_pe_cmap;
  lp.rec16 = h->rpool.d_rec16;
  lp.cmeta = h->rpool.d_cmeta;
  lp.clist = h->rpool.d_clist;
  lp.items = h->rpool.d_items;
  lp.ctl = h->rpool.d_ctl;
  lp.cmatch = h->rpool.d_cmatch;
  lp.descs = job.sdescs;
  lp.xl = xl;
  lp.seq0 = seq0;
  lp.fresh = h->counters_fresh ? 1u : 0u;
  h->counters_fresh = false;
  if ((h->flags & kDbgLocalTiming) && !(h->flags & kDbgRouteTiming)) {
    rc = ensure_dbg(h, (size_t)h->num_cus * (kWG / 64) * kRouteTimingWords);
    if (rc) return rc;
    lp.p.dbg = reinterpret_cast<unsigned long long*>(h->d_dbg.get());
  }
  HIP_TRY(h, launch_local((uint32_t)h->num_cus, h->stream, lp));
  HIP_TRY(h, hipEventRecord(h->ringm[slot], h->stream));
  HIP_TRY(h, hipEventRecord(h->ring1[slot], h->stream));
  h->nlaunch++;
  h->launched = true;
  if (job.settle_now) {
    FoundParams f;
    f.ranges = job.ranges;
    f.chunk0 = job.chunk0;
    f.used = h->rpool.d_used;
    f.cmeta = h->rpool.d_cmeta;
    f.cmatch = h->rpool.d_cmatch;
    f.rec16 = h->rpool.d_rec16;
    f.bufcnt = h->d_bufcnt + job.index_base;
    f.nb_bufs = (uint32_t)h->bufcnt_stride;
    f.gbits = xl.gbits;
    f.gshift = 16 + xl.wbits + xl.obits;
    HIP_TRY(h, launch_found(grid, h->stream, f));
    return NMG_OK;
  }
  h->route_pending = true;
  h->route_grid = grid;
  h->route_xl = xl;
  return NMG_OK;
}

int route_settle(nmg_engine* h) {
  if (!h->route_pending) return NMG_OK;
  h->route_pending = false;
  FoundParams f;
  f.ranges = h->d_ranges;
  f.chunk0 = h->rpool.d_chunk0;
  f.used = h->rpool.d_used;
  f.cmeta = h->rpool.d_cmeta;
  f.cmatch = h->rpool.d_cmatch;
  f.rec16 = h->rpool.d_rec16;
  f.bufcnt = h->d_bufcnt;
  f.nb_bufs = (uint32_t)h->bufcnt_stride;
  f.gbits = h->route_xl.gbits;
  f.gshift = 16 + h->route_xl.wbits + h->route_xl.obits;
  HIP_TRY(h, hipSetDevice(h->device));
  HIP_TRY(h, launch_found(h->route_grid, h->stream, f));
  return NMG_OK;
}
```

numamma_amd/csrc/nmg_submit.hip:

```cpp
#include "nmg_engine_impl.h"

int stage_reserve(nmg_engine* h, size_t need) {
  if (need <= h->h_stage.cap()) return NMG_OK;
  PinBuf<uint8_t> p(h->multi ? PinMem::portable() : PinMem());
  HIP_TRY(h, p.alloc(std::max(need, h->h_stage.cap() * 2 + (1u << 20))));
  if (h->stage_len) memcpy(p, h->h_stage, h->stage_len);
  if (h->h_stage) HIP_TRY(h, hipStreamSynchronize(h->stream));
  h->h_stage = std::move(p);
  return NMG_OK;
}

int append_desc(nmg_engine* h, uint64_t len, uint32_t thread_rank, uint32_t access) {
  if (!h->zc_dev.empty()) h->zc_dev.push_back(0);
  BufDesc d;
  d.offset = h->stage_len;
  d.len = (uint32_t)len;
  d.thread_rank = thread_rank;
  d.access = access;
  d.pad = 0;
  d.seq = h->descs.size();
  h->descs.push_back(d);
  h->buf_bytes.push_back(len);
  h->stage_len = (h->stage_len + len + 15) & ~size_t(15);
  h->staged_dirty = true;
  h->descs_dirty = true;
  h->multi_staged = false;
  return NMG_OK;
}

uint64_t zero_copy_dev(nmg_engine* h, const void* p, uint64_t len) {
  if (h->hostregs.empty() || h->streaming || h->multi || (h->flags & NMG_F_SAMPLE_MATCHES)) return 0;
  const uintptr_t a = (uintptr_t)p;
  for (const auto& r : h->hostregs)
    if (a >= r.lo && a + len <= r.hi) {
      const uint64_t dev = r.dev + (a - r.lo);
      return (dev & 15) ? 0 : dev;
    }
  return 0;
}

int append_desc_zc(nmg_engine* h, uint64_t dev, uint64_t len, uint32_t thread_rank, uint32_t access) {
  if (h->zc_dev.size() < h->descs.size()) h->zc_dev.resize(h->descs.size(), 0);
  h->zc_dev.push_back(dev);
  BufDesc d;
  d.offset = 0;
  d.len = (uint32_t)len;
  d.thread_rank = thread_rank;
  d.access = access;
  d.pad = 0;
  d.seq = h->descs.size();
  h->descs.push_back(d);
  h->buf_bytes.push_back(len);
  h->descs_dirty = true;
  h->multi_staged = false;
  return NMG_OK;
}

int check_buffer_args(nmg_engine* h, uint64_t len, uint32_t thread_rank, uint32_t access) {
  if (access > 1) return fail(h, NMG_ERR_INVALID, "access_type must be 0 (read) or 1 (write)");
  if (thread_rank >= h->T)
    return fail(h, NMG_ERR_RANGE, "thread_rank >= nb_threads (set nmg_options.nb_threads)");
  if (len >= (1ull << 32)) return fail(h, NMG_ERR_RANGE, "buffer >= 4 GiB (unsigned cursors, mem_sampling.c:831-834)");
  if (h->external) return fail(h, NMG_ERR_STATE, "device buffers are set; call nmg_clear_buffers first");
  if (h->streamed && !h->streaming) return fail(h, NMG_ERR_STATE, "stream ended; call nmg_clear_buffers first");
  return NMG_OK;
}


extern "C" int nmg_register_host(nmg_engine* h, void* ptr, uint64_t bytes) {
  if (!h || !ptr || !bytes) return NMG_ERR_INVALID;
  if (h->multi) return fail(h, NMG_ERR_STATE, "nmg_register_host: single-GPU engines only");
  if ((uintptr_t)ptr & 4095) return fail(h, NMG_ERR_INVALID, "nmg_register_host: ptr must be page-aligned (4 KiB)");
  const uintptr_t a = (uintptr_t)ptr;
  for (const auto& r : h->hostregs)
    if ((a & ~uintptr_t(4095)) < ((r.hi + 4095) & ~uintptr_t(4095)) && ((uintptr_t)r.pages) < a + bytes)
      return fail(h, NMG_ERR_INVALID, "nmg_register_host: overlaps (shares a page with) a registered range");
  const uintptr_t pg = 4096, p0 = a, p1 = (a + bytes + pg - 1) & ~(pg - 1);
  HIP_TRY(h, hipSetDevice(h->device));
  HIP_TRY(h, hipHostRegister((void*)p0, p1 - p0, hipHostRegisterMapped));
  void* dev = nullptr;
  if (hipHostGetDevicePointer(&dev, (void*)p0, 0) != hipSuccess || !dev) {
    (void)hipHostUnregister((void*)p0);
    return fail(h, NMG_ERR_HIP, "nmg_register_host: no device address for the range");
  }
  h->hostregs.push_back({a, a + bytes, (uint64_t)(uintptr_t)dev + (a - p0), (void*)p0});
  return NMG_OK;
}

extern "C" int nmg_unregister_host(nmg_engine* h, void* ptr) {
  if (!h || !ptr) return NMG_ERR_INVALID;
  for (size_t i = 0; i < h->hostregs.size(); i++) {
    if (h->hostregs[i].lo != (uintptr_t)ptr) continue;
    HIP_TRY(h, hipSetDevice(h->device));
    HIP_TRY(h, hipStreamSynchronize(h->stream));
    for (uint64_t z : h->zc_dev)
      if (z && z - h->hostregs[i].dev < h->hostregs[i].hi - h->hostregs[i].lo)
        return fail(h, NMG_ERR_STATE, "nmg_unregister_host: submitted buffers lie in the range; nmg_clear_buffers first");
    HIP_TRY(h, hipHostUnregister(h->hostregs[i].pages));
    h->hostregs.erase(h->hostregs.begin() + i);
    return NMG_OK;
  }
  return fail(h, NMG_ERR_INVALID, "nmg_unregister_host: not a registered range");
}

extern "C" int nmg_submit_buffer(nmg_engine* h, const void* bytes, uint64_t len, uint32_t thread_rank,
                                 uint32_t access_type) {
  if (!h || (len && !bytes)) return NMG_ERR_INVALID;
  int rc = check_buffer_args(h, len, thread_rank, access_type);
  if (rc) return rc;
  if (len == 0) return NMG_OK;
  if (const uint64_t dev = zero_copy_dev(h, bytes, len)) return append_desc_zc(h, dev, len, thread_rank, access_type);
  if (h->streaming) {
    uint8_t* dst = nullptr;
    rc = stream_dst(h, len, &dst, nullptr);
    if (rc) return rc;
    memcpy(dst, bytes, len);
    return stream_append(h, len, thread_rank, access_type);
  }
  rc = stage_reserve(h, h->stage_len + len + 16);
  if (rc) return rc;
  memcpy(h->h_stage + h->stage_len, bytes, len);
  return append_desc(h, len, thread_rank, access_type);
}

extern "C" int nmg_submit_ring(nmg_engine* h, const void* ring, uint64_t ring_size, uint64_t data_tail,
                               uint64_t data_head, uint32_t thread_rank, uint32_t access_type) {
  if (!h || !ring || data_tail > ring_size || data_head > ring_size) return NMG_ERR_INVALID;
  if (data_head == data_tail) return NMG_OK;
  uint64_t len = data_head - data_tail;
  if (data_head < data_tail) len = ring_size - data_tail + data_head;
  int rc = check_buffer_args(h, len, thread_rank, access_type);
  if (rc) return rc;
  if (data_head > data_tail)
    if (const uint64_t dev = zero_copy_dev(h, (const uint8_t*)ring + data_tail, len))
      return append_desc_zc(h, dev, len, thread_rank, access_type);
  uint8_t* dst = nullptr;
  if (h->streaming) {
    rc = stream_dst(h, len, &dst, nullptr);
  } else {
    rc = stage_reserve(h, h->stage_len + len + 16);
    dst = h->h_stage + h->stage_len;
  }
  if (rc) return rc;
  const uint8_t* r = (const uint8_t*)ring;
  if (data_head < data_tail) {
    uint64_t first = ring_size - data_tail;
    memcpy(dst, r + data_tail, first);
    memcpy(dst + first, r, data_head);
  } else {
    memcpy(dst, r + data_tail, len);
  }
  return h->streaming ? stream_append(h, len, thread_rank, access_type) : append_desc(h, len, thread_rank, access_type);
}


void run_copies(nmg_engine* h, const std::vector<CopyTask>& tasks) {
  if (tasks.empty()) return;
  uint64_t total = 0;
  for (const auto& t : tasks) total += t.len;
  const uint32_t nthreads = h->copy_threads;
  if (nthreads <= 1 || total < (2u << 20)) {
    for (const auto& t : tasks) memcpy(t.dst, t.src, t.len);
    return;
  }
  if (!h->pool) h->pool.reset(new CopyPool(nthreads));
  const uint32_t T = nthreads;
  std::vector<size_t> cut(T + 1, tasks.size());
  cut[0] = 0;
  uint64_t acc = 0;
  uint32_t k = 1;
  for (size_t i = 0; i < tasks.size() && k < T; i++) {
    acc += tasks[i].len;
    if (acc * T >= total * k) cut[k++] = i + 1;
  }
  h->pool->run([&](uint32_t w) {
    for (size_t i = cut[w]; i < cut[w + 1]; i++) memcpy(tasks[i].dst, tasks[i].src, tasks[i].len);
  });
}


int slot_acquire(nmg_engine* h, int s) {
  auto& sl = h->slots[s];
  if (sl.used) HIP_TRY(h, hipEventSynchronize(sl.copied));
  sl.len = 0;
  sl.descs.clear();
  return NMG_OK;
}

int ensure_bufcnt(nmg_engine* h, size_t need) {
  if (need <= h->bufcnt_stride) return NMG_OK;
  const size_t old_cap = h->d_bufcnt.cap() / 2;
  if (h->bufcnt_stride == 0 && need <= old_cap) {
    h->bufcnt_stride = old_cap;
    HIP_TRY(h, hipMemsetAsync(h->d_bufcnt, 0, old_cap * 2 * 4, h->stream));
    return NMG_OK;
  }
  const size_t cap = std::max<size_t>({need, old_cap * 2, (size_t)4096});
  DevBuf<uint32_t> nb;
  HIP_TRY(h, hipStreamSynchronize(h->stream));
  HIP_TRY(h, nb.alloc(cap * 2));
  HIP_TRY(h, hipMemsetAsync(nb, 0, cap * 2 * 4, h->stream));
  if (h->d_bufcnt && h->bufcnt_stride) {
    HIP_TRY(h, hipMemcpyAsync(nb, h->d_bufcnt, h->bufcnt_stride * 4, hipMemcpyDeviceToDevice, h->stream));
    HIP_TRY(h, hipMemcpyAsync(nb + cap, h->d_bufcnt + h->bufcnt_stride, h->bufcnt_stride * 4,
                              hipMemcpyDeviceToDevice, h->stream));
  }
  HIP_TRY(h, hipStreamSynchronize(h->stream));
  h->d_bufcnt = std::move(nb);
  h->bufcnt_stride = cap;
  return NMG_OK;
}

int stream_flush(nmg_engine* h) {
  if (h) h->epoch++;
  Range range("nmg_stream_chunk");
  auto& sl = h->slots[h->cur_slot];
  if (sl.descs.empty()) return NMG_OK;
  const uint32_t nb = (uint32_t)sl.descs.size();
  const uint32_t grid = attribution_grid(h, nb);
  int rc = ensure_bufcnt(h, h->descs.size());
  if (rc) return rc;
  const bool route = route_eligible(h, sl.descs);
  const size_t sched_bytes = nb * sizeof(BufDesc) + (grid + 1) * 4 * (route ? 2 : 1);
  if (sched_bytes > sl.h_sched.cap())
    HIP_TRY(h, sl.h_sched.reserve(std::max<size_t>(sched_bytes * 2, 64 << 10)));
  const uint32_t index_base = (uint32_t)(h->descs.size() - nb);
  BufDesc* h_sdescs = reinterpret_cast<BufDesc*>(sl.h_sched.get());
  uint32_t* h_ranges = reinterpret_cast<uint32_t*>(h_sdescs + nb);
  make_schedule(sl.descs, grid, index_base, h_sdescs, h_ranges, !route);
  if (route) {
    std::vector<uint32_t> c0;
    rc = route_pool(h, sl.descs, grid, h_ranges, c0);
    if (rc) return rc;
    memcpy(h_ranges + grid + 1, c0.data(), (grid + 1) * 4);
  }
  if (sl.len + 64 > sl.d_arena.cap() || sched_bytes > sl.d_sched.cap()) {
    if (sl.used) HIP_TRY(h, hipEventSynchronize(sl.done));
    if (sl.len + 64 > sl.d_arena.cap()) HIP_TRY(h, sl.d_arena.reserve(std::max<size_t>(sl.len + 64, sl.h_stage.cap() + 64)));
    if (sched_bytes > sl.d_sched.cap()) HIP_TRY(h, sl.d_sched.reserve(sl.h_sched.cap()));
  }
  if (sl.used) HIP_TRY(h, hipStreamWaitEvent(h->copy_stream, sl.done, 0));
  HIP_TRY(h, hipMemcpyAsync(sl.d_arena, sl.h_stage, sl.len, hipMemcpyHostToDevice, h->copy_stream));
  HIP_TRY(h, hipMemcpyAsync(sl.d_sched, sl.h_sched, sched_bytes, hipMemcpyHostToDevice, h->copy_stream));
  HIP_TRY(h, hipEventRecord(sl.copied, h->copy_stream));
  HIP_TRY(h, hipStreamWaitEvent(h->stream, sl.copied, 0));
  const BufDesc* d_sdescs = reinterpret_cast<const BufDesc*>(sl.d_sched.get());
  const uint32_t* d_ranges = reinterpret_cast<const uint32_t*>(d_sdescs + nb);
  if (route) {
    const RouteJob job{&sl.descs, sl.d_arena, d_sdescs, d_ranges, d_ranges + grid + 1, grid, index_base, true};
    rc = route_analyze_job(h, job);
  } else {
    rc = launch_attribution(h, sl.d_arena, d_sdescs, d_ranges, nb, grid, sl.len);
  }
  if (rc) return rc;
  HIP_TRY(h, hipEventRecord(sl.done, h->stream));
  sl.used = true;
  h->cur_slot ^= 1;
  return slot_acquire(h, h->cur_slot);
}

int stream_dst(nmg_engine* h, uint64_t len, uint8_t** dst, std::vector<CopyTask>* pending) {
  auto* sl = &h->slots[h->cur_slot];
  if (!sl->descs.empty() && sl->len + len + 16 > h->chunk_cap) {
    if (pending) {
      run_copies(h, *pending);
      pending->clear();
    }
    int rc = stream_flush(h);
    if (rc) return rc;
    sl = &h->slots[h->cur_slot];
  }
  if (sl->len + len + 16 > sl->h_stage.cap()) {
    PinBuf<uint8_t> p;
    HIP_TRY(h, p.alloc(std::max<size_t>(h->chunk_cap, sl->len + len + 16)));
    if (sl->len) {
      if (pending) {
        run_copies(h, *pending);
        pending->clear();
      }
      memcpy(p, sl->h_stage, sl->len);
    }
    sl->h_stage = std::move(p);
  }
  *dst = sl->h_stage + sl->len;
  return NMG_OK;
}

int stream_append(nmg_engine* h, uint64_t len, uint32_t thread_rank, uint32_t access) {
  auto& sl = h->slots[h->cur_slot];
  BufDesc d;
  d.offset = sl.len;
  d.len = (uint32_t)len;
  d.thread_rank = thread_rank;
  d.access = access;
  d.pad = 0;
  d.seq = h->descs.size();
  sl.descs.push_back(d);
  h->descs.push_back(d);
  h->buf_bytes.push_back(len);
  sl.len = (sl.len + len + 15) & ~size_t(15);
  return NMG_OK;
}

extern "C" int nmg_stream_begin(nmg_engine* h, uint64_t chunk_bytes, uint32_t copy_threads) {
  if (!h || copy_threads == 0) return NMG_ERR_INVALID;
  if (h->multi) return fail(h, NMG_ERR_STATE, "streaming is single-GPU (nmg_options.nb_gpus <= 1)");
  if (h->external) return fail(h, NMG_ERR_STATE, "device buffers are set; call nmg_clear_buffers first");
  if (h->flags & NMG_F_SAMPLE_MATCHES)
    return fail(h, NMG_ERR_STATE, "dump modes (NMG_F_SAMPLE_MATCHES) need nmg_analyze over submitted buffers");
  if (h->staged_dirty || (!h->streaming && !h->streamed && !h->descs.empty()))
    return fail(h, NMG_ERR_STATE, "buffers already submitted; call nmg_clear_buffers first");
  HIP_TRY(h, hipSetDevice(h->device));
  if (!h->copy_stream) {
    HIP_TRY(h, hipStreamCreateWithFlags(&h->copy_stream, hipStreamNonBlocking));
    for (auto& sl : h->slots) {
      HIP_TRY(h, hipEventCreateWithFlags(&sl.copied, hipEventDisableTiming));
      HIP_TRY(h, hipEventCreateWithFlags(&sl.done, hipEventDisableTiming));
    }
  }
  h->chunk_cap = std::max<uint64_t>(chunk_bytes, 64 << 10);
  if (copy_threads != h->copy_threads) h->pool.reset();
  h->copy_threads = copy_threads;
  h->streaming = true;
  h->streamed = true;
  return NMG_OK;
}

extern "C" int nmg_stream_end(nmg_engine* h) {
  if (!h) return NMG_ERR_INVALID;
  if (!h->streaming) return NMG_OK;
  HIP_TRY(h, hipSetDevice(h->device));
  int rc = h->have_table ? stream_flush(h) : NMG_OK;
  h->streaming = false;
  return rc;
}

extern "C" int nmg_submit_buffers(nmg_engine* h, uint32_t n, const void* const* bytes, const uint64_t* lens,
                                  const uint32_t* thread_ranks, const uint32_t* access_types) {
  if (!h || (n && (!bytes || !lens || !thread_ranks || !access_types))) return NMG_ERR_INVALID;
  for (uint32_t i = 0; i < n; i++) {
    if (lens[i] && !bytes[i]) return NMG_ERR_INVALID;
    int rc = check_buffer_args(h, lens[i], thread_ranks[i], access_types[i]);
    if (rc) return rc;
  }
  std::vector<CopyTask> tasks;
  tasks.reserve(n);
  if (!h->streaming) {
    uint64_t total = 0;
    for (uint32_t i = 0; i < n; i++) total += (lens[i] + 15) & ~uint64_t(15);
    int rc = stage_reserve(h, h->stage_len + total + 16);
    if (rc) return rc;
    for (uint32_t i = 0; i < n; i++) {
      if (!lens[i]) continue;
      if (const uint64_t dev = zero_copy_dev(h, bytes[i], lens[i])) {
        append_desc_zc(h, dev, lens[i], thread_ranks[i], access_types[i]);
        continue;
      }
      tasks.push_back({h->h_stage + h->stage_len, (const uint8_t*)bytes[i], lens[i]});
      append_desc(h, lens[i], thread_ranks[i], access_types[i]);
    }
    run_copies(h, tasks);
    return NMG_OK;
  }
  for (uint32_t i = 0; i < n; i++) {
    if (!lens[i]) continue;
    uint8_t* dst = nullptr;
    int rc = stream_dst(h, lens[i], &dst, &tasks);
    if (rc) return rc;
    tasks.push_back({dst, (const uint8_t*)bytes[i], lens[i]});
    stream_append(h, lens[i], thread_ranks[i], access_types[i]);
  }
  run_copies(h, tasks);
  return NMG_OK;
}

extern "C" int nmg_set_device_buffers(nmg_engine* h, const void* d_data, const uint64_t* offsets,
                                      const uint64_t* lengths, const uint32_t* thread_ranks,
                                      const uint32_t* access_types, uint32_t nb_buffers, uint64_t seq_base) {
  if (!h || (nb_buffers && (!d_data || !offsets || !lengths || !thread_ranks || !access_types)))
    return NMG_ERR_INVALID;
  if (h->multi) return fail(h, NMG_ERR_STATE, "a multi-GPU engine takes host buffers (nmg_submit_*)");
  if (h->streaming || h->streamed) return fail(h, NMG_ERR_STATE, "streaming buffers are set; call nmg_clear_buffers first");
  std::vector<BufDesc> descs;
  std::vector<uint64_t> bytes;
  descs.reserve(nb_buffers);
  for (uint32_t b = 0; b < nb_buffers; b++) {
    if (offsets[b] & 15) return fail(h, NMG_ERR_INVALID, "device buffer offsets must be 16-byte aligned");
    if (access_types[b] > 1) return fail(h, NMG_ERR_INVALID, "access_type must be 0 or 1");
    if (thread_ranks[b] >= h->T) return fail(h, NMG_ERR_RANGE, "thread_rank >= nb_threads");
    if (lengths[b] >= (1ull << 32)) return fail(h, NMG_ERR_RANGE, "buffer >= 4 GiB");
    if (lengths[b] == 0) continue;
    BufDesc d;
    d.offset = offsets[b];
    d.len = (uint32_t)lengths[b];
    d.thread_rank = thread_ranks[b];
    d.access = access_types[b];
    d.pad = 0;
    d.seq = seq_base + descs.size();
    descs.push_back(d);
    bytes.push_back(lengths[b]);
  }
  h->descs.swap(descs);
  h->zc_dev.clear();
  h->buf_bytes.swap(bytes);
  h->d_data = (const uint8_t*)d_data;
  h->external = true;
  h->staged_dirty = false;
  h->descs_dirty = true;
  h->multi_staged = false;
  h->stage_len = 0;
  return NMG_OK;
}

extern "C" int nmg_clear_buffers(nmg_engine* h) {
  if (!h) return NMG_ERR_INVALID;
  if (h->route_pending) {
    const int rc = route_settle(h);
    if (rc) return rc;
  }
  if (h->streaming || h->streamed) {
    HIP_TRY(h, hipSetDevice(h->device));
    HIP_TRY(h, hipStreamSynchronize(h->stream));
    HIP_TRY(h, hipStreamSynchronize(h->copy_stream));
    for (auto& sl : h->slots) {
      sl.descs.clear();
      sl.len = 0;
      sl.used = false;
    }
    h->streamed = false;
    h->bufcnt_stride = 0;
  }
  for (nmg_engine* w : h->workers) nmg_clear_buffers(w);
  h->descs.clear();
  h->buf_bytes.clear();
  h->zc_dev.clear();
  h->stage_len = 0;
  h->external = false;
  h->d_data = nullptr;
  h->descs_dirty = true;
  h->multi_staged = false;
  h->counts_override = false;
  return NMG_OK;
}

int stage_h2d(nmg_engine* h, void* d_dst, const void* src, size_t n) {
  if (!n) return NMG_OK;
  const size_t need = (n + 255) & ~size_t(255);
  if (h->up_off + need > h->up_pin.cap()) {
    if (h->up_recorded) HIP_TRY(h, hipEventSynchronize(h->up_ev));
    h->up_off = 0;
    if (need > h->up_pin.cap()) HIP_TRY(h, h->up_pin.reserve(std::max<size_t>(need * 2, 4u << 20)));
  }
  if (!h->up_ev) HIP_TRY(h, hipEventCreateWithFlags(&h->up_ev, hipEventDisableTiming));
  uint8_t* p = h->up_pin + h->up_off;
  memcpy(p, src, n);
  HIP_TRY(h, hipMemcpyAsync(d_dst, p, n, hipMemcpyHostToDevice, h->stream));
  HIP_TRY(h, hipEventRecord(h->up_ev, h->stream));
  h->up_recorded = true;
  h->up_off += need;
  return NMG_OK;
}

void stage_reset(nmg_engine* h) {
  if (h->up_recorded) (void)hipEventSynchronize(h->up_ev);
  h->up_off = 0;
}

int upload_buffers(nmg_engine* h) {
  Range range("nmg_stage_h2d");
  if (!h->external && h->staged_dirty) {
    if (h->stage_len + 64 > h->d_arena.cap()) {
      HIP_TRY(h, hipStreamSynchronize(h->stream));
      HIP_TRY(h, h->d_arena.reserve(h->stage_len + 64));
    }
    if (h->stage_len) HIP_TRY(h, hipMemcpyAsync(h->d_arena, h->h_stage, h->stage_len, hipMemcpyHostToDevice, h->stream));
    h->d_data = h->d_arena;
    h->staged_dirty = false;
  }
  if (h->descs_dirty) {
    size_t n = h->descs.size();
    for (size_t i = 0; i < h->zc_dev.size() && i < n; i++)
      if (h->zc_dev[i]) h->descs[i].offset = h->zc_dev[i] - (uint64_t)(uintptr_t)h->d_data;
    if (n > h->d_descs.cap()) {
      HIP_TRY(h, hipStreamSynchronize(h->stream));
      h->d_bufcnt.reset();
      HIP_TRY(h, h->d_descs.alloc(n));
      HIP_TRY(h, h->d_bufcnt.alloc(n * 2));
    }
    h->bufcnt_stride = n;
    if (n) {
      stage_reset(h);
      const int rc = stage_h2d(h, h->d_descs, h->descs.data(), n * sizeof(BufDesc));
      if (rc) return rc;
      HIP_TRY(h, hipMemsetAsync(h->d_bufcnt, 0, n * 2 * 4, h->stream));
    }
    h->descs_dirty = false;
  }
  return NMG_OK;
}

void make_schedule(const std::vector<BufDesc>& descs, uint32_t grid, uint32_t index_base, BufDesc* sorted,
                          uint32_t* ranges, bool by_stream) {
  const uint32_t nb = (uint32_t)descs.size();
  std::vector<uint32_t> order(nb);
  for (uint32_t i = 0; i < nb; i++) order[i] = i;
  if (by_stream) std::stable_sort(order.begin(), order.end(), [&](uint32_t a, uint32_t b) {
    const BufDesc &x = descs[a], &y = descs[b];
    if (x.access != y.access) return x.access < y.access;
    return x.thread_rank < y.thread_rank;
  });
  std::vector<uint64_t> csum(nb + 1, 0);
  for (uint32_t i = 0; i < nb; i++) csum[i + 1] = csum[i] + descs[order[i]].len + 64;
  ranges[0] = 0;
  for (uint32_t w = 1; w < grid; w++) {
    const uint64_t target = csum[nb] * w / grid;
    uint32_t c = (uint32_t)(std::lower_bound(csum.begin(), csum.end(), target) - csum.begin());
    ranges[w] = std::max(ranges[w - 1], std::min(c, nb));
  }
  ranges[grid] = nb;
  for (uint32_t i = 0; i < nb; i++) {
    sorted[i] = descs[order[i]];
    sorted[i].pad = index_base + order[i];
  }
}

int build_schedule(nmg_engine* h, uint32_t grid, bool by_stream) {
  const uint32_t nb = (uint32_t)h->descs.size();
  std::vector<uint32_t> ranges(grid + 1, 0);
  std::vector<BufDesc> sorted(nb);
  make_schedule(h->descs, grid, 0, sorted.data(), ranges.data(), by_stream);
  if (nb > h->d_sdescs.cap() || grid + 1 > h->d_ranges.cap()) {
    HIP_TRY(h, hipStreamSynchronize(h->stream));
    h->d_ranges.reset();
    HIP_TRY(h, h->d_sdescs.alloc(std::max<size_t>(nb, 1)));
    HIP_TRY(h, h->d_ranges.alloc(grid + 1));
  }
  int rc = stage_h2d(h, h->d_sdescs, sorted.data(), nb * sizeof(BufDesc));
  if (!rc) rc = stage_h2d(h, h->d_ranges, ranges.data(), (grid + 1) * 4);
  if (rc) return rc;
  h->sched_grid = grid;
  h->sched_route = !by_stream;
  if (!by_stream) return route_prepare(h, grid, ranges);
  return NMG_OK;
}

void ensure_occupancy(nmg_engine* h) {
  if (h->blocks_per_cu <= 0) {
    h->blocks_per_cu = attribute_blocks_per_cu();
  }
}

uint32_t attribution_grid(nmg_engine* h, uint32_t nb) {
  ensure_occupancy(h);
  return nb ? std::min<uint32_t>(nb, (uint32_t)(h->num_cus * h->blocks_per_cu)) : 0;
}

Params base_params(nmg_engine* h, const uint8_t* data, const BufDesc* sdescs, const uint32_t* ranges) {
  Params p;
  memset(&p, 0, sizeof(p));
  p.data = data;
  p.sbufs = sdescs;
  p.ranges = ranges;
  p.nb_bufs = (uint32_t)h->bufcnt_stride;
  p.nb_keys = h->lk.K;
  p.keys = h->lk.keys;
  p.nodes = h->lk.nodes;
  p.entries = h->d_entries;
  p.chain = h->lk.chain;
  p.ffences = h->lk.ffences;
  p.fshift = h->lk.fshift;
  p.dir = h->lk.dir;
  p.nb_fences = h->lk.nb_fences;
  p.fence_log2 = h->lk.fence_log2;
  p.dir_log2 = h->lk.dir_log2;
  p.nb_threads = h->T;
  p.flags = h->flags;
  p.nb_entries = h->E;
  p.lds_nodes = h->lk.K <= kLdsNodes;
  p.elevels = h->lk.elevels;
  p.efences = h->lk.efences;
  p.enodes = h->lk.enodes;
  p.sparse_mask = (uint32_t)(h->sparse_cap - 1);
  p.hist_cells = h->tab.cells();
  p.sum64 = h->cnt.d_sum64;
  p.min64 = h->cnt.d_min64;
  p.max64 = h->cnt.d_max64;
  p.hist = h->cnt.d_hist;
  p.bufcnt = h->d_bufcnt;
  p.found = h->d_found;
  p.sparse_keys = h->cnt.d_sparse_keys;
  p.sparse_vals = h->cnt.d_sparse_vals;
  p.sparse_dirty = h->cnt.d_sparse_dirty ? h->cnt.d_sparse_dirty + (h->nreset & 1) : nullptr;
  p.smatch = (h->flags & NMG_F_SAMPLE_MATCHES) ? h->d_smatch : nullptr;
  if (h->tl.on) {
    p.tl = h->tl.d_cells;
    p.tl_t0 = h->tl.opt.t0;
    p.tl_bin_shift = h->tl.opt.bin_shift;
    p.tl_nb_bins = h->tl.opt.nb_bins;
    p.tl_row_shift = h->tl.opt.row_shift;
    p.tl_rounds = h->tl.rounds;
  }
  return p;
}

int launch_events(nmg_engine* h, int* slot_out) {
  const int slot = (int)(h->nlaunch % nmg_engine::kRing);
  if (!h->ring0[slot]) {
    HIP_TRY(h, hipEventCreate(&h->ring0[slot]));
    HIP_TRY(h, hipEventCreate(&h->ringr[slot]));
    HIP_TRY(h, hipEventCreate(&h->ringm[slot]));
    HIP_TRY(h, hipEventCreate(&h->ring1[slot]));
  }
  *slot_out = slot;
  return NMG_OK;
}

int ensure_dbg(nmg_engine* h, size_t words) {
  HIP_TRY(h, h->d_dbg.reserve(words));
  HIP_TRY(h, hipMemsetAsync(h->d_dbg, 0, words * 8, h->stream));
  h->dbg_len = words;
  return NMG_OK;
}

int launch_attribution(nmg_engine* h, const uint8_t* data, const BufDesc* sdescs, const uint32_t* ranges,
                              uint32_t nb, uint32_t grid, uint64_t nbytes) {
  Range range("nmg_attribute");
  Params p = base_params(h, data, sdescs, ranges);
  const int mode = (h->E <= kObjSlots ? kModeDenseObj : 0) | (h->tab.cells() <= kDensePageCells ? kModeDensePage : 0) |
                   (p.lds_nodes ? 0 : kModeLarge);
  if (!(mode & kModeDenseObj) && h->cnt.d_pk64 && !(h->flags & kDbgNoPack)) {
    const uint32_t cbits = 64 - (uint32_t)__builtin_clzll(nbytes / kRecBytes + 1);
    if (2 * cbits < 64) {
      p.pk64 = h->cnt.d_pk64;
      p.pk_shift = 64 - cbits;
      p.pk_wlim = 1ull << (64 - 2 * cbits);
    }
  }
  if (!(mode & kModeDenseObj) && nb && grid <= kLogMaxGrid && (h->flags & NMG_F_MATCH_SAMPLES) &&
      nbytes / 8 < (1ull << 32)) {
    uint32_t rshift = 0;
    while ((((uint64_t)h->E + (1ull << rshift) - 1) >> rshift) > kLogParts) rshift++;
    const uint32_t parts = (uint32_t)(((uint64_t)h->E + (1ull << rshift) - 1) >> rshift);
    const uint64_t cap = (h->flags & kDbgTinyLog)
                             ? 2
                             : std::min<uint64_t>(1u << 20, (nbytes / kRecBytes) / ((uint64_t)grid * parts) * 5 / 4 + 32);
    const size_t logs = (size_t)grid * parts, need = logs * cap;
    if (need > h->cnt.d_tlog.cap() || logs > h->cnt.d_tlog_cnt.cap()) {
      HIP_TRY(h, hipStreamSynchronize(h->stream));
      HIP_TRY(h, h->cnt.d_tlog.reserve(need));
      HIP_TRY(h, h->cnt.d_tlog_cnt.reserve(logs));
    }
    p.tlog = h->cnt.d_tlog;
    p.tlog_cnt = h->cnt.d_tlog_cnt;
    p.tlog_cap = (uint32_t)cap;
    p.tlog_rshift = rshift;
    p.tlog_parts = parts;
  }
  int slot = 0;
  int rc = launch_events(h, &slot);
  if (rc) return rc;
  HIP_TRY(h, hipEventRecord(h->ring0[slot], h->stream));
  if (nb) {
    if (h->flags & kDbgTiming) {
      rc = ensure_dbg(h, (size_t)grid * (kWG / 64) * kTimingWords);
      if (rc) return rc;
      p.dbg = reinterpret_cast<unsigned long long*>(h->d_dbg.get());
      h->counters_fresh = false;
      HIP_TRY(h, launch_attribute(true, mode, grid, h->stream, p));
    } else {
      h->counters_fresh = false;
      HIP_TRY(h, launch_attribute(false, mode, grid, h->stream, p));
    }
    HIP_TRY(h, hipEventRecord(h->ringr[slot], h->stream));
    HIP_TRY(h, hipEventRecord(h->ringm[slot], h->stream));
    if (p.tlog) {
      TlogParams r;
      r.tlog = p.tlog;
      r.tlog_cnt = p.tlog_cnt;
      r.sum64 = h->cnt.d_sum64;
      r.min64 = h->cnt.d_min64;
      r.pk64 = p.pk64;
      r.grid = grid;
      r.parts = p.tlog_parts;
      r.cap = p.tlog_cap;
      r.rshift = p.tlog_rshift;
      r.nb_entries = h->E;
      r.pk_shift = p.pk_shift;
      HIP_TRY(h, launch_tlog_reduce(p.tlog_parts, h->stream, r));
    } else if (p.pk64) {
      const uint32_t blocks = (uint32_t)std::min<uint64_t>(2048, (2ull * h->E + 255) / 256);
      HIP_TRY(h, launch_unpack(blocks, h->stream, h->cnt.d_sum64, p.pk64, h->E, p.pk_shift));
    }
  }
  if (!nb) {
    HIP_TRY(h, hipEventRecord(h->ringr[slot], h->stream));
    HIP_TRY(h, hipEventRecord(h->ringm[slot], h->stream));
  }
  HIP_TRY(h, hipEventRecord(h->ring1[slot], h->stream));
  h->nlaunch++;
  h->launched = true;
  return NMG_OK;
}
```

numamma_amd/csrc/nmg_table.hip:

```cpp
#include "nmg_engine_impl.h"

struct BigLookup {
  uint32_t nb_fences = 0, fence_log2 = 0, dir_log2 = 0;
  std::vector<uint64_t> efences;
  std::vector<uint8_t> shift;
  std::vector<uint2> dir;
};

static void build_big_lookup(const uint64_t* keys, uint32_t K, bool no_dir, BigLookup& bl) {
  while (((uint64_t)K + (1u << bl.fence_log2) - 1) >> bl.fence_log2 > kMaxFences) bl.fence_log2++;
  const uint32_t S = 1u << bl.fence_log2;
  bl.nb_fences = (uint32_t)(((uint64_t)K + S - 1) >> bl.fence_log2);
  bl.efences.assign(kMaxFences + 1, ~0ull);
  {
    uint32_t r = 0, i = 1;
    std::vector<uint32_t> stack;
    while (i <= kMaxFences || !stack.empty()) {
      while (i <= kMaxFences) {
        stack.push_back(i);
        i = 2 * i;
      }
      i = stack.back();
      stack.pop_back();
      if (r < bl.nb_fences) bl.efences[i] = keys[(uint64_t)r << bl.fence_log2];
      r++;
      i = 2 * i + 1;
    }
  }
  bl.shift.assign(bl.nb_fences, kShiftSearch);
  if (S == 1 || S > (1u << 16) || no_dir) return;
  bl.dir_log2 = bl.fence_log2 + 1;
  const uint32_t D = 1u << bl.dir_log2;
  bl.dir.assign((size_t)bl.nb_fences << bl.dir_log2, make_uint2(0, 0));
  for (uint32_t b = 0; b < bl.nb_fences; b++) {
    const uint32_t k0 = b * S, k1 = std::min<uint64_t>((uint64_t)k0 + S, K);
    const uint64_t f = keys[k0], span = keys[k1 - 1] - f;
    uint32_t sh = 0;
    while (sh < 64 && (span >> sh) >= D) sh++;
    if (sh > 32) continue;
    bl.shift[b] = (uint8_t)sh;
    uint2* dd = &bl.dir[(size_t)b << bl.dir_log2];
    uint32_t k = k0;
    for (uint32_t j = 0; j < D; j++) {
      const uint64_t s0 = (uint64_t)j << sh;
      while (k + 1 < k1 && keys[k + 1] - f <= s0) k++;
      uint32_t c = 0;
      while (k + 1 + c < k1 && (j == D - 1 || keys[k + 1 + c] - f < s0 + (1ull << sh))) c++;
      dd[j].x = (k - k0) | (std::min<uint32_t>(c, 0xffffu) << 16);
      dd[j].y = c ? (uint32_t)(keys[k + 1] - f - s0) : 0u;
    }
  }
}

int build_lookup(nmg_engine* h, LookupSet& l, const uint64_t* keys, const uint32_t* entry_off, uint32_t nb_keys,
                 const std::vector<DevEntry>& chain, DevEntry* chain_dev) {
  l.K = nb_keys;
  std::vector<DevEntry> nodes(nb_keys);
  for (uint32_t k = 0; k < nb_keys; k++) {
    nodes[k] = chain[entry_off[k]];
    nodes[k].first = entry_off[k];
    nodes[k].count = entry_off[k + 1] - entry_off[k];
  }
  HIP_TRY(h, alloc_copy(h, l.keys, keys, nb_keys));
  HIP_TRY(h, alloc_copy(h, l.nodes, nodes));
  if (!chain_dev) HIP_TRY(h, alloc_copy(h, l.own_chain, chain));
  l.chain = chain_dev ? chain_dev : l.own_chain.get();
  if (nb_keys <= kLdsNodes) {
    l.elevels = 0;
    while (((1u << l.elevels) - 1) < nb_keys) l.elevels++;
    const uint32_t n = 1u << l.elevels;
    std::vector<uint64_t> ef(n, ~0ull);
    std::vector<DevEntry> en(n);
    memset(en.data(), 0, n * sizeof(DevEntry));
    uint32_t r = 0;
    std::vector<uint32_t> stack;
    uint32_t i = 1;
    while (i < n || !stack.empty()) {
      while (i < n) {
        stack.push_back(i);
        i = 2 * i;
      }
      i = stack.back();
      stack.pop_back();
      if (r < nb_keys) {
        ef[i] = keys[r];
        en[i] = nodes[r];
      } else if (nb_keys) {
        en[i] = nodes[nb_keys - 1];
      }
      r++;
      i = 2 * i + 1;
    }
    HIP_TRY(h, alloc_copy(h, l.efences, ef));
    HIP_TRY(h, alloc_copy(h, l.enodes, en));
  }
  l.nb_fences = l.fence_log2 = l.dir_log2 = 0;
  if (nb_keys > kLdsNodes) {
    BigLookup bl;
    build_big_lookup(keys, nb_keys, (h->flags & kDbgNoDir) != 0, bl);
    l.nb_fences = bl.nb_fences;
    l.fence_log2 = bl.fence_log2;
    l.dir_log2 = bl.dir_log2;
    HIP_TRY(h, alloc_copy(h, l.ffences, bl.efences));
    HIP_TRY(h, alloc_copy(h, l.fshift, bl.shift));
    HIP_TRY(h, alloc_copy(h, l.dir, bl.dir));
  }
  return NMG_OK;
}

void route_segments(const uint64_t* b, uint32_t P, RSeg* seg, uint32_t* nseg, std::vector<uint16_t>& dir) {
  std::vector<uint32_t> cuts{0};
  if (P > 1) {
    std::vector<uint64_t> gaps(P - 1);
    for (uint32_t q = 0; q + 1 < P; q++) gaps[q] = b[q + 1] - b[q];
    std::vector<uint64_t> med(gaps);
    std::nth_element(med.begin(), med.begin() + med.size() / 2, med.end());
    const uint64_t m = std::max<uint64_t>(med[med.size() / 2], 1);
    std::vector<uint32_t> idx(P - 1);
    for (uint32_t q = 0; q + 1 < P; q++) idx[q] = q;
    std::sort(idx.begin(), idx.end(), [&](uint32_t x, uint32_t y) { return gaps[x] > gaps[y]; });
    for (uint32_t i = 0; i < idx.size() && cuts.size() < kRouteSegs; i++) {
      if (gaps[idx[i]] / 64 <= m) break;
      cuts.push_back(idx[i] + 1);
    }
    std::sort(cuts.begin(), cuts.end());
  }
  const uint32_t S = (uint32_t)cuts.size();
  dir.assign(kRouteDir, 0);
  uint32_t used = 0;
  for (uint32_t k = 0; k < kRouteSegs; k++) {
    if (k >= S) {
      seg[k] = RSeg{~0ull, 0, 1, 0, 0};
      continue;
    }
    const uint32_t qa = cuts[k], qb = k + 1 < S ? cuts[k + 1] : P;
    const uint32_t ns = (uint32_t)((uint64_t)(kRouteDir - S) * (qb - qa) / P) + 1;
    const uint64_t span = b[qb - 1] - b[qa];
    uint32_t sh = 0;
    while (sh < 63 && (span >> sh) >= ns) sh++;
    seg[k] = RSeg{b[qa], used, ns, sh, qb - 1};
    uint32_t q = qa;
    for (uint32_t j = 0; j < ns; j++) {
      const unsigned __int128 s0 = (unsigned __int128)j << sh, s1 = (unsigned __int128)(j + 1) << sh;
      while (q + 1 < qb && (unsigned __int128)(b[q + 1] - b[qa]) <= s0) q++;
      uint32_t c = 0;
      if (j == ns - 1) c = qb - 1 - q;
      else
        while (q + 1 + c < qb && (unsigned __int128)(b[q + 1 + c] - b[qa]) < s1) c++;
      dir[used + j] = (uint16_t)(q | (std::min(c, kDirCntSat) << 11));
    }
    used += ns;
  }
  *nseg = S;
}

int build_partitions(nmg_engine* h, const uint64_t* keys, const uint32_t* entry_off, uint32_t K,
                            const std::vector<DevEntry>& dev, const uint32_t* ids) {
  h->rt = RouteTable();
  if (K <= kLdsNodes || !(h->flags & NMG_F_MATCH_SAMPLES)) return NMG_OK;
  if (ids) {
    uint32_t e = 0;
    while (e < entry_off[K] && ids[e] == e) e++;
    if (e == entry_off[K]) ids = nullptr;
  }
  if (ids && h->tab.cells() >= (1ull << 31)) return NMG_OK;
  const uint64_t T = h->T;
  std::vector<PartInfo> parts;
  std::vector<uint32_t> lrel, cmap;
  if (ids) lrel.assign(entry_off[K], kEmpty32);
  uint32_t k = 0;
  while (k < K) {
    PartInfo pi;
    memset(&pi, 0, sizeof(pi));
    pi.k0 = k;
    pi.e0 = entry_off[k];
    pi.cmap = ~0u;
    uint64_t cb = ~0ull, ce = 0, cc = 0;
    while (k < K && k - pi.k0 < kPartKeys) {
      if (k > pi.k0 && keys[k] - keys[pi.k0] >= (1ull << (kAddrBits - 1))) break;
      const uint32_t ea = entry_off[k], eb = entry_off[k + 1];
      if (eb - pi.e0 > kPartEntries) {
        if (k == pi.k0) return NMG_OK;
        break;
      }
      uint64_t ncb = cb, nce = ce, ncc = cc;
      for (uint32_t e = ea; e < eb; e++)
        if (dev[e].hist != kHistSparse) {
          const uint64_t np = h->tab.npages[dev[e].id];
          ncb = std::min<uint64_t>(ncb, dev[e].hist);
          nce = std::max<uint64_t>(nce, dev[e].hist + np);
          ncc += np;
        }
      if (k > pi.k0 && ncb != ~0ull && (ids ? ncc : nce - ncb) * T > kPartCells)
        break;
      cb = ncb;
      ce = nce;
      cc = ncc;
      k++;
    }
    pi.nk = k - pi.k0;
    pi.ne = entry_off[k] - pi.e0;
    pi.cb = cb == ~0ull ? 0 : cb;
    pi.span = cb == ~0ull ? 0 : (uint32_t)(ce - cb);
    pi.pages_lds = pi.span && (uint64_t)pi.span * T <= kPartCells;
    if (ids && cc && cc * T <= kPartCells) {
      pi.cmap = (uint32_t)cmap.size();
      pi.span = (uint32_t)cc;
      pi.pages_lds = 1;
      uint32_t off = 0;
      for (uint32_t e = pi.e0; e < pi.e0 + pi.ne; e++)
        if (dev[e].hist != kHistSparse) {
          const uint32_t np = (uint32_t)h->tab.npages[dev[e].id];
          lrel[e] = off;
          for (uint32_t g = 0; g < np; g++) cmap.push_back((uint32_t)(dev[e].hist + g));
          off += np;
        }
    }
    const uint64_t kspan = keys[k - 1] - keys[pi.k0];
    while (pi.dshift < 63 && (kspan >> pi.dshift) >= kPartDir) pi.dshift++;
    parts.push_back(pi);
    if (parts.size() > kMaxParts) return NMG_OK;
  }
  const uint32_t P = (uint32_t)parts.size();
  h->route_tbase = ~0ull;
  for (const DevEntry& d : dev)
    if (d.alloc) h->route_tbase = std::min<uint64_t>(h->route_tbase, d.alloc);
  if (h->route_tbase == ~0ull) h->route_tbase = 0;
  const uint64_t tb = h->route_tbase;
  std::vector<uint64_t> pk((size_t)P * kPartSlots, ~0ull);
  std::vector<uint4> pn((size_t)P * kPartSlots * 2, make_uint4(0, 0, 0, 0));
  std::vector<uint4> ppn((size_t)P * kPartSlots, make_uint4(0, 0, 0, 0));
  std::vector<uint2> pinf((size_t)P * kPartSlots, make_uint2(kEmpty32, 0));
  std::vector<uint4> pdir((size_t)P * kPartDir, make_uint4(0, 0, 0, 0));
  std::vector<uint4> pold((size_t)P * kOldLds, make_uint4(0, 0, 0, 0));
  std::vector<uint32_t> poinf((size_t)P * kOldLds, kEmpty32);
  auto cell_rel = [&](const PartInfo& pi, uint32_t e) -> uint32_t {
    const DevEntry& d = dev[e];
    return d.hist == kHistSparse ? kEmpty32 : pi.cmap != ~0u ? lrel[e] : (uint32_t)(d.hist - pi.cb);
  };
  auto qdates = [&](const DevEntry& d, uint64_t tb, uint32_t& aq, uint32_t& fq) {
    if (d.free < tb) {
      aq = 0xffffffffu;
      fq = 0;
    } else {
      aq = (uint32_t)std::min<uint64_t>((d.alloc > tb ? d.alloc - tb : 0) >> kPnQShift, 0xffffffffull);
      fq = (uint32_t)std::min<uint64_t>((d.free - tb) >> kPnQShift, 0xffffffffull);
    }
  };
  for (uint32_t q = 0; q < P; q++) {
    const PartInfo& pi = parts[q];
    const uint64_t f = keys[pi.k0];
    for (uint32_t r = 0; r < pi.nk; r++) {
      const uint32_t kk = pi.k0 + r;
      const DevEntry& d = dev[entry_off[kk]];
      const size_t o = (size_t)q * kPartSlots + r;
      pk[o] = keys[kk];
      pn[2 * o] = make_uint4((uint32_t)d.addr, (uint32_t)(d.addr >> 32), (uint32_t)d.end, (uint32_t)(d.end >> 32));
      pn[2 * o + 1] = make_uint4((uint32_t)d.alloc, (uint32_t)(d.alloc >> 32), (uint32_t)d.free, (uint32_t)(d.free >> 32));
      const uint32_t older = entry_off[kk + 1] - entry_off[kk] > 1 ? 1u : 0u;
      const uint32_t hrel = cell_rel(pi, entry_off[kk]);
      const uint64_t erel = d.end - f, brel = d.addr - f;
      const bool never = d.free < tb;
      const bool exact = !never && (d.addr < f || d.end < d.addr || (erel >> 32) != 0 || (brel >> 32) != 0);
      uint32_t aq, fq;
      qdates(d, tb, aq, fq);
      const uint32_t nold = entry_off[kk + 1] - entry_off[kk] - 1, lbase = entry_off[kk] - pi.e0 - r;
      bool old_lds = nold > 0 && nold < 2048 && lbase + nold <= kOldLds;
      for (uint32_t i = 1; old_lds && i <= nold; i++) {
        const uint32_t e = entry_off[kk] + i;
        const DevEntry& od = dev[e];
        uint32_t oa, of;
        qdates(od, tb, oa, of);
        uint4 v = make_uint4(0, oa, of, 0);
        if (od.free >= tb) {
          if (od.addr < f || od.end < od.addr || ((od.end - f) >> 32) != 0) {
            old_lds = false;
            break;
          }
          v.x = (uint32_t)(od.end - f);
          v.w = (uint32_t)(od.addr - f);
        }
        pold[(size_t)q * kOldLds + lbase + i - 1] = v;
        poinf[(size_t)q * kOldLds + lbase + i - 1] = cell_rel(pi, e);
      }
      ppn[o] = make_uint4(exact || never ? 0u : (uint32_t)erel, aq, fq,
                          (entry_off[kk] - pi.e0) | (older ? kPnOlder : 0u) | (exact ? kPnExact : 0u) |
                              (old_lds ? kPnOldLds | (nold << kPnOldShift) : 0u));
      pinf[o] = make_uint2(hrel, exact || never ? 0u : (uint32_t)brel);
    }
    uint32_t lo = 0;
    for (uint32_t j = 0; j < kPartDir; j++) {
      const uint64_t s0 = (uint64_t)j << pi.dshift;
      while (lo + 1 < pi.nk && keys[pi.k0 + lo + 1] - f <= s0) lo++;
      uint32_t c = 0;
      while (lo + 1 + c < pi.nk &&
             (j == kPartDir - 1 || keys[pi.k0 + lo + 1 + c] - f < s0 + (1ull << pi.dshift)))
        c++;
      uint32_t off[kDirInline];
      bool inl = true;
      for (uint32_t i = 0; i < kDirInline; i++) {
        off[i] = 0xffffu;
        if (i < c) {
          const uint64_t v = keys[pi.k0 + lo + 1 + i] - f - s0;
          if (v >> 16) inl = false;
          else off[i] = (uint32_t)v;
        }
      }
      pdir[(size_t)q * kPartDir + j] =
          make_uint4(lo | (c << 10) | ((inl && c ? 1u : 0u) << 21), off[0] | (off[1] << 16), off[2] | (off[3] << 16),
                     off[4] | (off[5] << 16));
    }
  }
  std::vector<uint64_t> pb(kMaxParts + 1, ~0ull);
  for (uint32_t q = 0; q < P; q++) pb[q] = keys[parts[q].k0];
  std::vector<uint16_t> rdir;
  route_segments(pb.data(), P, h->rsegs, &h->nrsegs, rdir);
  std::vector<uint32_t> dead((kMaxParts + 1) / 32, 0u);
  for (uint32_t q = 0; q < P; q++) {
    bool d = true;
    for (uint32_t e = parts[q].e0; d && e < parts[q].e0 + parts[q].ne; e++) d = dev[e].free == 0;
    if (d) dead[q >> 5] |= 1u << (q & 31);
  }
  RouteTable& rt = h->rt;
  HIP_TRY(h, alloc_copy(h, rt.d_pdead, dead));
  HIP_TRY(h, alloc_copy(h, rt.d_parts, parts));
  HIP_TRY(h, alloc_copy(h, rt.d_pbounds, pb));
  HIP_TRY(h, alloc_copy(h, rt.d_pdir, rdir));
  HIP_TRY(h, alloc_copy(h, rt.d_pe_keys, pk));
  HIP_TRY(h, alloc_copy(h, rt.d_pe_nodes, pn));
  HIP_TRY(h, alloc_copy(h, rt.d_pe_pnode, ppn));
  HIP_TRY(h, alloc_copy(h, rt.d_pe_old, pold));
  HIP_TRY(h, alloc_copy(h, rt.d_pe_oinf, poinf));
  HIP_TRY(h, alloc_copy(h, rt.d_pe_info, pinf));
  HIP_TRY(h, alloc_copy(h, rt.d_pe_dir, pdir));
  if (ids) {
    HIP_TRY(h, alloc_copy(h, rt.d_pe_ids, ids, entry_off[K]));
    HIP_TRY(h, alloc_copy(h, rt.d_pe_lrel, lrel));
    if (!cmap.empty()) HIP_TRY(h, alloc_copy(h, rt.d_pe_cmap, cmap));
  }
  HIP_TRY(h, hipStreamSynchronize(h->stream));
  rt.nparts = P;
  rt.ok = true;
  return NMG_OK;
}

extern "C" int nmg_set_objects(nmg_engine* h, const uint64_t* keys, const uint32_t* entry_off,
                               uint32_t nb_keys, const nmg_object* entries, uint32_t nb_entries) {
  if (h) h->epoch++;
  if (h) h->counters_fresh = false;
  if (h) h->snap.lay.meta_dirty = h->cprep.lay.meta_dirty = true;
  Range range("nmg_set_objects");
  if (!h || (nb_keys && (!keys || !entry_off)) || (nb_entries && !entries))
    return NMG_ERR_INVALID;
  int rc = check_table(h, keys, entry_off, nb_keys, nb_entries);
  if (rc) return rc;
  if (nb_entries >= (1u << 31)) return fail(h, NMG_ERR_RANGE, "too many entries");
  HIP_TRY(h, hipSetDevice(h->device));
  HIP_TRY(h, hipStreamSynchronize(h->stream));
  free_table(h);
  h->cnt = Counters();
  h->tl = Timeline();
  h->lk.K = nb_keys;
  h->E = nb_entries;

  EntryTable& tab = h->tab;
  tab = EntryTable();
  tab.cur.threads = h->T;
  tab.cur.budget_cells = h->hist_budget / 4;
  tab.resize(nb_entries);
  h->order.clear();
  const bool want_hist = (h->flags & NMG_F_PAGE_HIST) && (h->flags & NMG_F_MATCH_SAMPLES);
  for (uint32_t e = 0; e < nb_entries; e++) {
    const nmg_object& o = entries[e];
    tab.describe(e, o);
    tab.npages[e] = o.buffer_size / kPageSize + 1;
    if (want_hist && tab.place(e, tab.npages[e], false) == kPlaceSparseFull)
      return fail(h, NMG_ERR_CAPACITY, "too many sparse entries");
    tab.dev_entries[e] = tab.dev_entry(e, o);
  }
  tab.cur.cells = tab.cur.padded_cells();
  HIP_TRY(h, alloc_copy(h, h->d_entries, tab.dev_entries));
  rc = build_lookup(h, h->lk, keys, entry_off, nb_keys, tab.dev_entries, h->d_entries);
  if (rc) return rc;
  rc = build_partitions(h, keys, entry_off, nb_keys, tab.dev_entries, nullptr);
  if (rc) return rc;
  h->cnt.set_sizes(nb_entries, h->flags & NMG_F_OBJECT_LEVELS);
  HIP_TRY(h, h->cnt.d_sum64.alloc(h->cnt.n_sum64));
  HIP_TRY(h, h->cnt.d_min64.alloc(h->cnt.n_min64));
  HIP_TRY(h, h->cnt.d_max64.alloc(h->cnt.n_max64));
  HIP_TRY(h, h->d_found.reserve(1));
  if (nb_entries > kObjSlots) {
    HIP_TRY(h, h->cnt.d_pk64.alloc((size_t)nb_entries * 2));
    HIP_TRY(h, hipMemset(h->cnt.d_pk64, 0, (size_t)nb_entries * 2 * 8));
  }
  if (h->tab.cells()) HIP_TRY(h, h->cnt.d_hist.alloc(h->tab.cells() * h->T));
  if (!h->tab.sparse_entries.empty()) {
    HIP_TRY(h, h->cnt.d_sparse_keys.alloc(h->sparse_cap));
    HIP_TRY(h, h->cnt.d_sparse_vals.alloc(h->sparse_cap));
    HIP_TRY(h, h->cnt.d_sparse_dirty.alloc(2));
    const uint32_t ones[2] = {1u, 1u};
    HIP_TRY(h, hipMemcpy(h->cnt.d_sparse_dirty, ones, 8, hipMemcpyHostToDevice));
  }
  h->have_table = true;
  HIP_TRY(h, hipStreamSynchronize(h->stream));
  for (nmg_engine* w : h->workers) {
    const int rc = nmg_set_objects(w, keys, entry_off, nb_keys, entries, nb_entries);
    if (rc) return fail(h, rc, w->last_error);
  }
  return nmg_reset_counters(h);
}


extern "C" int nmg_set_timeline(nmg_engine* h, const nmg_timeline_options* o) {
  if (!h) return NMG_ERR_INVALID;
  h->epoch++;
  if (h->multi || !h->workers.empty()) return fail(h, NMG_ERR_INVALID, "nmg_set_timeline: not on a multi-GPU handle");
  constexpr uint32_t kNeed = NMG_F_MATCH_SAMPLES | NMG_F_PAGE_HIST;
  if ((h->flags & kNeed) != kNeed)
    return fail(h, NMG_ERR_INVALID, "nmg_set_timeline needs an engine created with NMG_F_MATCH_SAMPLES | NMG_F_PAGE_HIST");
  if (o && (o->bin_shift > 63 || o->nb_bins < 1 || o->nb_bins > 4096 || o->row_shift > 20 || o->reserved != 0))
    return fail(h, NMG_ERR_INVALID, "nmg_set_timeline: option out of range (bin_shift <= 63, nb_bins 1..4096, "
                                    "row_shift <= 20, reserved 0)");
  if (!h->have_table) return fail(h, NMG_ERR_STATE, "nmg_set_timeline before nmg_set_objects");
  if (h->streaming) return fail(h, NMG_ERR_STATE, "nmg_set_timeline while a stream is open");
  HIP_TRY(h, hipSetDevice(h->device));
  int rc = route_settle(h);
  if (rc) return rc;
  HIP_TRY(h, hipStreamSynchronize(h->stream));
  if (!o) {
    h->tl = Timeline();
    return NMG_OK;
  }
  EntryTable& tab = h->tab;
  const uint32_t E = h->E, T = h->T;
  Timeline t;
  t.opt = *o;
  if (const char* r = getenv("NMG_TL_ROUNDS")) t.rounds = (uint32_t)std::min(64, std::max(0, atoi(r)));
  const uint64_t budget = o->budget_bytes ? o->budget_bytes : (1ull << 30);
  unsigned __int128 need = 0;
  for (uint32_t e = 0; e < E; e++) {
    if (tab.hist_base[e] == kHistSparse || tab.buffer_size[e] < o->min_object_bytes) continue;
    const uint64_t R = (tab.buffer_size[e] / kPageSize + 1 + (1ull << o->row_shift) - 1) >> o->row_shift;
    if (need <= 0xffffffffull) {
      t.ids.push_back(e);
      t.base.push_back((uint32_t)need);
      t.nrows.push_back((uint32_t)R);
    }
    need += (unsigned __int128)R * o->nb_bins * T;
  }
  const unsigned __int128 bytes = need * 4;
  if (need > 0xffffffffull || bytes > budget) {
    char msg[160];
    snprintf(msg, sizeof(msg), "nmg_set_timeline: the cells need %llu bytes (budget %llu, at most 2^32 - 1 cells)",
             bytes > ~0ull ? ~0ull : (unsigned long long)bytes, (unsigned long long)budget);
    return fail(h, NMG_ERR_CAPACITY, msg);
  }
  t.ncells = (uint64_t)need;
  t.base.push_back((uint32_t)t.ncells);
  std::vector<DevEntry> dev = tab.dev_entries;
  for (DevEntry& d : dev) d.pad1 = kTlNone;
  for (size_t k = 0; k < t.ids.size(); k++) dev[t.ids[k]].pad1 = tl_pad(t.base[k], t.nrows[k]);
  HIP_TRY(h, t.d_cells.alloc(t.ncells));
  HIP_TRY(h, hipMemsetAsync(t.d_cells, 0, t.ncells * 4, h->stream));
  HIP_TRY(h, alloc_copy(h, t.d_ids, t.ids));
  HIP_TRY(h, alloc_copy(h, t.d_base, t.base));
  HIP_TRY(h, alloc_copy(h, t.d_nrows, t.nrows));
  if (E) HIP_TRY(h, hipMemcpyAsync(h->d_entries, dev.data(), (size_t)E * sizeof(DevEntry), hipMemcpyHostToDevice, h->stream));
  HIP_TRY(h, hipStreamSynchronize(h->stream));
  tab.dev_entries = std::move(dev);
  t.on = true;
  h->tl = std::move(t);
  return NMG_OK;
}

int grow_entries(nmg_engine* h, uint32_t newE, const uint32_t* ids, const nmg_object* objs, uint32_t n) {
  const uint32_t oldE = h->E;
  const uint64_t T = h->T;
  const bool want_hist = (h->flags & NMG_F_PAGE_HIST) && (h->flags & NMG_F_MATCH_SAMPLES);
  const bool levels = h->flags & NMG_F_OBJECT_LEVELS;
  EntryTable& tab = h->tab;
  const CellCursor cur0 = tab.cur;
  const uint64_t oldCells = cur0.cells;
  struct Old {
    uint32_t id;
    uint64_t hist, np;
  };
  std::vector<Old> changed;
  auto fail_rb = [&](int code, const std::string& msg) {
    for (auto it = changed.rbegin(); it != changed.rend(); ++it) {
      tab.dev_entries[it->id].hist = tab.hist_base[it->id] = it->hist;
      tab.npages[it->id] = it->np;
    }
    tab.truncate(oldE, cur0);
    return fail(h, code, msg);
  };
  tab.resize(newE);
  for (uint32_t j = 0; j < n; j++) {
    const uint32_t id = ids[j];
    const uint64_t np = objs[j].buffer_size / kPageSize + 1;
    if (id >= oldE) {
      tab.npages[id] = np;
      if (want_hist && tab.place(id, np, false) == kPlaceSparseFull)
        return fail_rb(NMG_ERR_CAPACITY, "too many sparse entries");
    } else if (np > tab.npages[id]) {
      changed.push_back({id, tab.hist_base[id], tab.npages[id]});
      if (want_hist && tab.hist_base[id] != kHistSparse && tab.place(id, np, true) != kPlaceDense)
        return fail_rb(NMG_ERR_CAPACITY, "an object outgrew its page cells past the histogram budget");
      tab.npages[id] = np;
    }
  }
  const uint64_t cells = tab.cur.cells = tab.cur.padded_cells();
  const uint64_t n_sum = sum64_words(newE, levels), n_min = min64_words(newE);
  DevBuf<uint64_t> sum, mn, skeys;
  DevBuf<uint32_t> hist, svals, sdirty;
  DevBuf<unsigned long long> pk;
  DevBuf<DevEntry> ent;
  const bool new_sparse = cur0.nsparse == 0 && tab.cur.nsparse && !h->cnt.d_sparse_keys;
  auto undo = [&](hipError_t e, const char* what) {
    (void)hipStreamSynchronize(h->stream);
    return fail_rb(NMG_ERR_HIP, std::string("nmg_update_objects: ") + what + ": " + hipGetErrorString(e));
  };
  hipError_t e;
  if ((e = sum.alloc(n_sum)) != hipSuccess) return undo(e, "counters");
  if ((e = mn.alloc(n_min)) != hipSuccess) return undo(e, "ordinals");
  if (cells && cells * T != oldCells * T && (e = hist.alloc(cells * T)) != hipSuccess)
    return undo(e, "page histogram");
  if (newE > kObjSlots && (e = pk.alloc((size_t)newE * 2)) != hipSuccess) return undo(e, "packed counters");
  if ((e = ent.alloc(newE)) != hipSuccess) return undo(e, "entries");
  hipStream_t st = h->stream;
  if (new_sparse) {
    if ((e = skeys.alloc(h->sparse_cap)) != hipSuccess || (e = svals.alloc(h->sparse_cap)) != hipSuccess ||
        (e = sdirty.alloc(2)) != hipSuccess || (e = hipMemsetAsync(skeys, 0xff, h->sparse_cap * 8, st)) != hipSuccess ||
        (e = hipMemsetAsync(svals, 0, h->sparse_cap * 4, st)) != hipSuccess ||
        (e = hipMemsetAsync(sdirty, 0, 2 * 4, st)) != hipSuccess)
      return undo(e, "sparse page table");
  }
  const uint64_t* osum = h->cnt.d_sum64;
  const uint64_t* omin = h->cnt.d_min64;
  if ((e = hipMemsetAsync(sum, 0, n_sum * 8, st)) != hipSuccess ||
      (e = hipMemcpyAsync(sum, osum, kCwBase * 8, hipMemcpyDeviceToDevice, st)) != hipSuccess ||
      (oldE && (e = hipMemcpy2DAsync(sum + kCwBase, (size_t)newE * 8, osum + kCwBase, (size_t)oldE * 8, (size_t)oldE * 8,
                                     kCwRows, hipMemcpyDeviceToDevice, st)) != hipSuccess) ||
      (levels && oldE &&
       (e = hipMemcpyAsync(sum + levels_base(newE), osum + levels_base(oldE), (size_t)oldE * 2 * kLevelWords * 8,
                           hipMemcpyDeviceToDevice, st)) != hipSuccess) ||
      (e = hipMemsetAsync(mn, 0xff, n_min * 8, st)) != hipSuccess ||
      (e = hipMemcpyAsync(mn, omin, first_index(oldE) * 8, hipMemcpyDeviceToDevice, st)) != hipSuccess ||
      (e = hipMemcpyAsync(mn + error_index(newE), omin + error_index(oldE), 8, hipMemcpyDeviceToDevice, st)) !=
          hipSuccess ||
      (pk && (e = hipMemsetAsync(pk, 0, (size_t)newE * 2 * 8, st)) != hipSuccess) ||
      (e = hipMemcpyAsync(ent, tab.dev_entries.data(), (size_t)newE * sizeof(DevEntry), hipMemcpyHostToDevice, st)) !=
          hipSuccess)
    return undo(e, "re-layout");
  if (hist) {
    if ((e = hipMemsetAsync(hist, 0, cells * T * 4, st)) != hipSuccess ||
        (oldCells && (e = hipMemcpy2DAsync(hist, cells * 4, h->cnt.d_hist, oldCells * 4, oldCells * 4, T,
                                           hipMemcpyDeviceToDevice, st)) != hipSuccess))
      return undo(e, "page histogram re-layout");
    for (const Old& m : changed)
      if (m.hist != tab.hist_base[m.id] &&
          ((e = hipMemcpy2DAsync(hist + tab.hist_base[m.id], cells * 4, hist + m.hist, cells * 4, m.np * 4, T,
                                 hipMemcpyDeviceToDevice, st)) != hipSuccess ||
           (e = hipMemset2DAsync(hist + m.hist, cells * 4, 0, m.np * 4, T, st)) != hipSuccess))
        return undo(e, "page cells of a grown object");
  }
  if ((e = hipStreamSynchronize(st)) != hipSuccess) return undo(e, "re-layout");
  if (!h->lk.own_chain) h->lk.chain = ent;
  h->cnt.d_sum64 = std::move(sum);
  h->cnt.d_min64 = std::move(mn);
  h->cnt.d_pk64 = std::move(pk);
  h->d_entries = std::move(ent);
  if (hist) h->cnt.d_hist = std::move(hist);
  h->cnt.set_sizes(newE, levels);
  h->E = newE;
  if (new_sparse) {
    h->cnt.d_sparse_keys = std::move(skeys);
    h->cnt.d_sparse_vals = std::move(svals);
    h->cnt.d_sparse_dirty = std::move(sdirty);
  }
  return NMG_OK;
}

extern "C" int nmg_update_objects(nmg_engine* h, const uint64_t* keys, const uint32_t* entry_off,
                                  uint32_t nb_keys, const uint32_t* entry_ids, const nmg_object* objects) {
  if (h) h->epoch++;
  if (h) h->counters_fresh = false;
  if (h) h->snap.lay.meta_dirty = h->cprep.lay.meta_dirty = true;
  Range range("nmg_update_objects");
  if (!h || (nb_keys && (!keys || !entry_off || !entry_ids || !objects))) return NMG_ERR_INVALID;
  if (!h->have_table) return fail(h, NMG_ERR_STATE, "nmg_update_objects before nmg_set_objects");
  const uint32_t n = nb_keys ? entry_off[nb_keys] : 0;
  int rc = check_table(h, keys, nb_keys ? entry_off : nullptr, nb_keys, n);
  if (rc) return rc;
  if (h->tl.on)
    for (uint32_t j = 0; j < n; j++)
      if (entry_ids[j] >= h->E || objects[j].buffer_size != h->tab.buffer_size[entry_ids[j]])
        return fail(h, NMG_ERR_STATE, "nmg_update_objects: with a timeline set, a table may only list existing "
                                      "entries with their sizes unchanged (drop it with nmg_set_timeline(h, NULL))");
  uint32_t newE = h->E;
  for (uint32_t j = 0; j < n; j++) newE = std::max(newE, entry_ids[j] + 1);
  if (entry_ids && n && (uint64_t)newE > (1ull << 31)) return fail(h, NMG_ERR_RANGE, "too many entries");
  uint64_t nb_grown = 0;
  {
    std::vector<uint8_t> seen(newE, 0);
    for (uint32_t j = 0; j < n; j++) {
      const uint32_t id = entry_ids[j];
      if (seen[id]) return fail(h, NMG_ERR_INVALID, "an entry id listed twice in one table");
      seen[id] = 1;
      if (id < h->E && objects[j].buffer_size / kPageSize + 1 > h->tab.npages[id]) nb_grown++;
    }
    for (uint32_t id = h->E; id < newE; id++)
      if (!seen[id]) return fail(h, NMG_ERR_RANGE, "new entry ids must be consecutive from the current entry count");
  }
  HIP_TRY(h, hipSetDevice(h->device));
  if (h->streaming) {
    rc = stream_flush(h);
    if (rc) return rc;
  }
  rc = route_settle(h);
  if (rc) return rc;
  HIP_TRY(h, hipStreamSynchronize(h->stream));
  if (h->multi_pending) {
    rc = multi_finish(h);
    if (rc) return rc;
  }
  if (newE > h->E || nb_grown) {
    rc = grow_entries(h, newE, entry_ids, objects, n);
    if (rc) return rc;
  }
  std::vector<DevEntry> chain(n);
  for (uint32_t j = 0; j < n; j++) chain[j] = h->tab.dev_entry(entry_ids[j], objects[j]);
  h->rt = RouteTable();
  LookupSet next;
  rc = build_lookup(h, next, keys, entry_off, nb_keys, chain, nullptr);
  if (rc == NMG_OK && hipStreamSynchronize(h->stream) != hipSuccess)
    rc = fail(h, NMG_ERR_HIP, "nmg_update_objects: table upload failed");
  if (rc) {
    (void)hipStreamSynchronize(h->stream);
    return rc;
  }
  h->lk = std::move(next);
  for (uint32_t j = 0; j < n; j++) h->tab.describe(entry_ids[j], objects[j]);
  if (n == h->E) {
    bool identity = true;
    for (uint32_t j = 0; j < n && identity; j++) identity = entry_ids[j] == j;
    if (identity) h->order.clear();
    else h->order.assign(entry_ids, entry_ids + n);
  } else if (!h->order.empty()) {
    for (uint32_t id = (uint32_t)h->order.size(); id < h->E; id++) h->order.push_back(id);
  }
  if (build_partitions(h, keys, entry_off, nb_keys, chain, entry_ids) != NMG_OK) {
    (void)hipGetLastError();
    h->rt = RouteTable();
  }
  for (nmg_engine* w : h->workers) {
    rc = nmg_update_objects(w, keys, entry_off, nb_keys, entry_ids, objects);
    if (rc) return fail(h, rc, w->last_error);
  }
  return NMG_OK;
}
```

Measured before the change: 45.42 billion.

## Shrink routed sample records to 12 bytes with adaptive bit layout

Compresses each routed record from 16 to 12 bytes. Address and quantized-timestamp field widths are now sized from the actual address span and time range in the table, and the buffer-group index is stored relative to the block's range base, carried alongside in the chunk list. Exact timestamps for ambiguous or older matches are re-read from the raw sample buffer, and the overflow path packs its base into the record. The aim is to cut global memory traffic for record writes and reads in the route and local kernels. In exchange there are extra raw-buffer reads on ambiguous paths and a wider clist entry.

Result: slower. 43.32 billion (-4.6%).

```diff
diff --git a/numamma_amd/csrc/nmg_engine_impl.h b/numamma_amd/csrc/nmg_engine_impl.h
--- a/numamma_amd/csrc/nmg_engine_impl.h
+++ b/numamma_amd/csrc/nmg_engine_impl.h
@@ -118,18 +118,17 @@
 };
 
 struct RoutePool {
-  DevBuf<uint4> d_rec16;
+  DevBuf<CRec> d_rec;
   DevBuf<uint32_t> d_cmeta;
   DevBuf<unsigned long long> d_cmatch;
-  DevBuf<uint32_t> d_clist;
+  DevBuf<uint2> d_clist;
   DevBuf<uint4> d_items;
   DevBuf<uint32_t> d_chunk0;
   DevBuf<uint32_t> d_used;
   DevBuf<uint32_t> d_pcnt;
   DevBuf<uint32_t> d_pbase;
   DevBuf<uint32_t> d_ctl;
-  DevBuf<uint4> d_ovf16;
-  DevBuf<unsigned long long> d_ovfx;
+  DevBuf<uint4> d_ovfrec;
 };
 
 struct EntryTable {
@@ -344,6 +343,9 @@
   uint64_t route_launches = 0;
   RSeg rsegs[kRouteSegs];
   uint64_t route_tbase = 0;
+  uint64_t route_aspan = 0;
+  uint64_t route_tqmax = 0;
+  std::vector<uint32_t> route_ranges;
   uint32_t nrsegs = 0;
   RoutePool rpool;
   bool sched_route = false;
@@ -379,6 +381,7 @@
   const uint32_t* chunk0;
   uint32_t grid, index_base;
   bool settle_now;
+  const uint32_t* h_ranges;
 };
 
 #pragma GCC visibility push(hidden)
@@ -428,7 +431,8 @@
 int launch_attribution(nmg_engine* h, const uint8_t* data, const BufDesc* sdescs, const uint32_t* ranges,
                               uint32_t nb, uint32_t grid, uint64_t nbytes);
 uint32_t bits_for(uint64_t v);
-bool route_layout(nmg_engine* h, const std::vector<BufDesc>& descs, XLayout& xl);
+bool route_layout(nmg_engine* h, const std::vector<BufDesc>& descs, const uint32_t* ranges, uint32_t grid,
+                  XLayout& xl);
 bool route_eligible(nmg_engine* h, const std::vector<BufDesc>& descs);
 bool route_eligible(nmg_engine* h);
 int route_pool(nmg_engine* h, const std::vector<BufDesc>& descs, uint32_t grid, const uint32_t* ranges,
diff --git a/numamma_amd/csrc/nmg_route.h b/numamma_amd/csrc/nmg_route.h
--- a/numamma_amd/csrc/nmg_route.h
+++ b/numamma_amd/csrc/nmg_route.h
@@ -58,13 +58,22 @@
 };
 static_assert(sizeof(PartInfo) == 48, "PartInfo");
 
-constexpr uint32_t kAddrBits = 40;
+struct CRec {
+  uint32_t x, y, z;
+};
+static_assert(sizeof(CRec) == 12, "CRec");
+constexpr uint32_t kRecWords = 3;
+constexpr uint32_t kMaxAddrBits = 40;
+constexpr uint32_t kMaxTqBits = 32;
 constexpr uint32_t kMinWeightBits = 11;
-constexpr uint32_t kTsBits = 40;
+constexpr uint32_t kMaxLocBits = 48 - kMinWeightBits;
 struct XLayout {
   uint32_t gbits, obits, tbits, wbits;
+  uint32_t abits, tqbits;
+  uint32_t wsh, lsh;
   uint64_t wesc;
   uint64_t tbase;
+  uint64_t asat, tqsat;
 };
 
 struct RouteParams {
@@ -77,12 +86,11 @@
   uint32_t nparts;
   XLayout xl;
   uint64_t seq0;
-  uint4* rec16;
+  CRec* rec;
   uint32_t* cmeta;
   const uint32_t* chunk0;
   uint32_t* used;
-  uint4* ovf16;
-  unsigned long long* ovfx;
+  uint4* ovfrec;
   uint32_t* ovf_cnt;
   uint32_t ovf_cap;
 };
@@ -101,7 +109,8 @@
   const uint32_t* used;
   const uint32_t* pcnt;
   const uint32_t* pbase;
-  uint32_t* clist;
+  uint2* clist;
+  const uint32_t* ranges;
   uint32_t nparts;
 };
 
@@ -118,9 +127,9 @@
   const uint32_t* pe_ids;
   const uint32_t* pe_lrel;
   const uint32_t* pe_cmap;
-  const uint4* rec16;
+  const CRec* rec;
   const uint32_t* cmeta;
-  const uint32_t* clist;
+  const uint2* clist;
   const uint4* items;
   uint32_t* ctl;
   unsigned long long* cmatch;
@@ -136,7 +145,7 @@
   const uint32_t* used;
   const uint32_t* cmeta;
   const unsigned long long* cmatch;
-  const uint4* rec16;
+  const CRec* rec;
   uint32_t* bufcnt;
   uint32_t nb_bufs, gbits, gshift;
 };
diff --git a/numamma_amd/csrc/nmg_route.hip b/numamma_amd/csrc/nmg_route.hip
--- a/numamma_amd/csrc/nmg_route.hip
+++ b/numamma_amd/csrc/nmg_route.hip
@@ -10,6 +10,7 @@
 
 struct XRec {
   uint64_t addr, ts, w;
+  uint32_t tq;
   uint64_t loc;
   uint32_t th, acc;
   bool esc;
@@ -17,38 +18,45 @@
   __device__ __forceinline__ uint32_t off(const XLayout& xl) const {
     return uint32_t(loc & ((1ull << xl.obits) - 1)) << 3;
   }
+  __device__ __forceinline__ void rebase(const XLayout& xl, uint32_t g0) { loc += uint64_t(g0) << xl.obits; }
 };
 
 __device__ __forceinline__ uint4 x_encode(const XLayout& xl, uint64_t pb, uint64_t addr, uint64_t ts, uint64_t w,
                                           uint32_t g, uint32_t off, uint32_t th, uint32_t acc) {
-  const uint64_t ar = addr - pb, tr = ts - xl.tbase;
-  const bool fit = (ar >> kAddrBits) == 0 && ts >= xl.tbase && (tr >> kTsBits) == 0 && w < xl.wesc;
+  const uint64_t ar = min(addr - pb, xl.asat), tr = min((ts - xl.tbase) >> kPnQShift, xl.tqsat);
+  const bool fit = (ar >> xl.abits) == 0 && ts >= xl.tbase && (tr >> xl.tqbits) == 0 && w < xl.wesc;
   const uint64_t a = fit ? ar : 0ull, t = fit ? tr : 0ull, wq = fit ? w : xl.wesc;
   const uint64_t loc = uint64_t(off >> 3) | (uint64_t(g) << xl.obits);
-  const uint64_t lo = a | (t << kAddrBits);
-  const uint64_t hi = (t >> (64 - kAddrBits)) | (wq << 16) | (loc << (16 + xl.wbits)) |
-                      (uint64_t(th) << (63 - xl.tbits)) | (uint64_t(acc) << 63);
-  return make_uint4((uint32_t)lo, (uint32_t)(lo >> 32), (uint32_t)hi, (uint32_t)(hi >> 32));
-}
-
-__device__ __forceinline__ XRec x_decode_rel(const XLayout& xl, uint4 v) {
+  const uint64_t lo = a | (t << xl.abits);
+  const uint64_t hi = (lo >> 32) | (wq << xl.wsh) | (loc << xl.lsh) | (uint64_t(th) << (63 - xl.tbits)) |
+                      (uint64_t(acc) << 63);
+  return make_uint4((uint32_t)lo, (uint32_t)hi, (uint32_t)(hi >> 32), 0u);
+}
+__device__ __forceinline__ CRec crec(uint4 v) {
+  CRec r;
+  r.x = v.x;
+  r.y = v.y;
+  r.z = v.z;
+  return r;
+}
+
+__device__ __forceinline__ XRec x_decode_rel(const XLayout& xl, uint32_t x, uint32_t y, uint32_t z) {
   XRec r;
-  r.addr = u64of(v.x, v.y & 0xffu);
-  r.ts = u64of(__builtin_amdgcn_alignbit(v.z, v.y, 8), (v.z >> 8) & 0xffu);
+  const uint64_t lo = u64of(x, y), hi = u64of(y, z);
+  r.addr = lo & ((1ull << xl.abits) - 1);
+  r.tq = (uint32_t)(lo >> xl.abits) & (uint32_t)((1ull << xl.tqbits) - 1);
+  r.ts = 0;
   const uint32_t wesc = (uint32_t)xl.wesc;
-  r.w = __builtin_amdgcn_alignbit(v.w, v.z, 16) & wesc;
+  r.w = (uint32_t)(hi >> xl.wsh) & wesc;
   r.esc = r.w == wesc;
-  r.loc = (u64of(v.z, v.w) >> (16 + xl.wbits)) & ((1ull << (xl.obits + xl.gbits)) - 1);
-  r.th = (v.w >> (31 - xl.tbits)) & ((1u << xl.tbits) - 1);
-  r.acc = v.w >> 31;
+  r.loc = (hi >> xl.lsh) & ((1ull << (xl.obits + xl.gbits)) - 1);
+  r.th = (z >> (31 - xl.tbits)) & ((1u << xl.tbits) - 1);
+  r.acc = z >> 31;
   return r;
 }
 
-__device__ __forceinline__ XRec x_decode(const XLayout& xl, uint64_t pb, uint4 v) {
-  XRec r = x_decode_rel(xl, v);
-  r.addr += pb;
-  r.ts += xl.tbase;
-  return r;
+__device__ __forceinline__ uint64_t raw_ts(const uint8_t* data, const BufDesc* descs, uint32_t g, uint32_t off) {
+  return reinterpret_cast<const uint64_t*>(data + descs[g].offset + off)[1];
 }
 
 __device__ __forceinline__ void x_resolve(XRec& r, const XLayout& xl, const uint8_t* data, const BufDesc* descs) {
@@ -56,6 +64,13 @@
   r.ts = q[1];
   r.addr = q[2];
   r.w = q[3];
+}
+
+__device__ __forceinline__ XRec x_decode_full(const XLayout& xl, uint4 v, const uint8_t* data, const BufDesc* descs) {
+  XRec r = x_decode_rel(xl, v.x, v.y, v.z);
+  r.rebase(xl, v.w);
+  x_resolve(r, xl, data, descs);
+  return r;
 }
 
 __device__ __forceinline__ uint32_t raw_mem_lvl(const uint8_t* data, uint64_t pos) {
@@ -403,7 +418,7 @@
   __shared__ unsigned long long s_gsums[2][kGlobalSums], s_gmins[2][kBuckets], s_gmaxs[2][kBuckets];
   __shared__ SegL s_seg[kRouteSegs];
   __shared__ uint64_t s_segst[kRouteSegs];
-  __shared__ uint4 s_line[kLineParts * 4];
+  __shared__ CRec s_line[kLineParts * 4];
   __shared__ LineWord s_lw[kLineParts];
   __shared__ uint32_t s_ldst[kLineParts];
   __shared__ uint2 s_tab[kWaves][64];
@@ -627,7 +642,7 @@
       X.q = q;
       X.lvl = uint32_t(rec.dsrc >> 5) & 0x3fff;
       X.routed = routed;
-      if (routed) X.a = x_encode(rp.xl, s_pb[q], rec.addr, rec.ts, rec.w, dw.pad, roff, dw.thread_rank(), acc_l);
+      if (routed) X.a = x_encode(rp.xl, s_pb[q], rec.addr, rec.ts, rec.w, dw.pad - r0, roff, dw.thread_rank(), acc_l);
       rt_stamp<TIMING>(rt, 4);
     };
 
@@ -670,7 +685,7 @@
         staged = counts && ahead == 0 && dst != ~0ull;
         if (lined && !(lw & kLwBroken) && ahead >= ahead_max) atomicOr(&s_lw[X.q], kLwBroken);
         if (staged) {
-          s_line[X.q * 4 + j] = X.a;
+          s_line[X.q * 4 + j] = crec(X.a);
           s_ldst[X.q] = (uint32_t)(dst >> 2);
         }
         __builtin_amdgcn_fence(__ATOMIC_RELEASE, "workgroup", "local");
@@ -709,7 +724,7 @@
             if (jj < nd) {
               const uint2 t = s_tab[wave][jj];
               const uint32_t tq = t.x & 2047u, tm = (t.x >> 11) & 15u, k = lane & 3;
-              if ((tm >> k) & 1) rp.rec16[uint64_t(t.y) * 4 + k] = s_line[tq * 4 + k];
+              if ((tm >> k) & 1) rp.rec[uint64_t(t.y) * 4 + k] = s_line[tq * 4 + k];
               piece_done(t, k);
             }
           }
@@ -721,21 +736,19 @@
       rt_stamp<TIMING>(rt, 9);
       const bool straight = dst != ~0ull && !counts;
       const bool alone = straight || (counts && !staged && dst != ~0ull);
-      if (alone) rp.rec16[dst] = X.a;
+      if (alone) rp.rec[dst] = crec(X.a);
       if (TIMING) {
         rt.acc[6] += (uint64_t)__popcll(__ballot(staged));
         rt.acc[7] += (uint64_t)__popcll(__ballot(straight));
       }
       if (__ballot(ovf)) {
         if (ovf) {
-          const uint64_t pbq = s_pb[X.q];
           const uint32_t o = atomicAdd(rp.ovf_cnt, 1u);
+          const uint4 xa = make_uint4(X.a.x, X.a.y, X.a.z, r0);
           if (o < rp.ovf_cap) {
-            rp.ovf16[o] = X.a;
-            rp.ovfx[o] = pbq;
+            rp.ovfrec[o] = xa;
           } else {
-            XRec xr = x_decode(rp.xl, pbq, X.a);
-            if (xr.esc) x_resolve(xr, rp.xl, p.data, p.sbufs);
+            const XRec xr = x_decode_full(rp.xl, xa, p.data, p.sbufs);
             direct_attribute<TL>(p, xr.addr, xr.ts, xr.w, xr.th, xr.acc, X.lvl, rp.seq0 + xr.g(rp.xl), xr.off(rp.xl),
                              xr.g(rp.xl));
           }
@@ -786,7 +799,7 @@
     if (q < nlp) {
       const uint32_t m = lw_mask(s_lw[q]);
       for (uint32_t j = 0; j < 4; j++)
-        if ((m >> j) & 1u) rp.rec16[uint64_t(s_ldst[q]) * 4 + j] = s_line[q * 4 + j];
+        if ((m >> j) & 1u) rp.rec[uint64_t(s_ldst[q]) * 4 + j] = s_line[q * 4 + j];
     }
   }
   if (tid == 0) rp.used[blockIdx.x] = min(s_taken, capl);
@@ -796,8 +809,7 @@
 __global__ __launch_bounds__(256) void overflow_kernel(RouteParams rp) {
   const uint32_t n = min(*rp.ovf_cnt, rp.ovf_cap);
   for (uint32_t i = blockIdx.x * 256 + threadIdx.x; i < n; i += gridDim.x * 256) {
-    XRec xr = x_decode(rp.xl, rp.ovfx[i], rp.ovf16[i]);
-    if (xr.esc) x_resolve(xr, rp.xl, rp.p.data, rp.p.sbufs);
+    const XRec xr = x_decode_full(rp.xl, rp.ovfrec[i], rp.p.data, rp.p.sbufs);
     const uint32_t lvl = (rp.p.flags & NMG_F_OBJECT_LEVELS)
                              ? raw_mem_lvl(rp.p.data, rp.p.sbufs[xr.g(rp.xl)].offset + xr.off(rp.xl))
                              : 0u;
@@ -927,6 +939,7 @@
   for (uint32_t q = tid; q < P; q += kWG) s_cnt[q] = r.pbase[q] + off[q];
   __syncthreads();
   const uint32_t c0 = r.chunk0[w], n = r.used[w];
+  const uint32_t g0 = r.ranges[w];
   constexpr uint32_t kU = 8;
   for (uint32_t b = 0; b < n; b += kU * kWG) {
     uint32_t m[kU];
@@ -939,7 +952,7 @@
     for (uint32_t u = 0; u < kU; u++) {
       if (!(m[u] >> 24)) continue;
       const uint32_t k = atomicAdd(&s_cnt[m[u] & 0xffffffu], 1u);
-      r.clist[k] = (c0 + b + u * kWG + tid) | ((m[u] >> 24) << kChunkIdBits);
+      r.clist[k] = make_uint2((c0 + b + u * kWG + tid) | ((m[u] >> 24) << kChunkIdBits), g0);
     }
   }
 }
@@ -983,7 +996,7 @@
   __shared__ unsigned long long s_owt[2][kPartEntries];
   __shared__ unsigned long long s_first[kPartEntries];
   __shared__ uint32_t s_pg[kPartCells / 2];
-  __shared__ uint32_t s_clist[kItemChunks];
+  __shared__ uint2 s_clist[kItemChunks];
   __shared__ uint32_t s_item, s_cnext, s_nfound, s_big, s_took;
   __shared__ uint4 s_nx[4];
 
@@ -998,6 +1011,7 @@
   rt.last = TIMING ? stamp() : 0;
   uint32_t nchunks = 0, nit = 0;
   uint64_t textra = 0;
+  uint64_t nesc = 0;
   uint32_t nfound = 0;
   if (tid == 0) s_nfound = 0;
   for (uint32_t i = tid; i < kPartEntries; i += kLWG) {
@@ -1043,7 +1057,8 @@
       uint64_t key = 0;
       uint4 pn = make_uint4(0, 0, 0, 0), od = pn;
       uint2 inf = make_uint2(0, 0);
-      uint32_t oi = 0, cl[kClPer];
+      uint32_t oi = 0;
+      uint2 cl[kClPer];
       if (tid < nk) {
         key = lp.pe_keys[uint64_t(q) * kPartSlots + tid];
         pn = lp.pe_pnode[uint64_t(q) * kPartSlots + tid];
@@ -1055,7 +1070,7 @@
         oi = lp.pe_oinf[uint64_t(q) * kOldLds + tid];
       }
 #pragma unroll
-      for (uint32_t u = 0; u < kClPer; u++) cl[u] = tid + u * kLWG < ncl ? lp.clist[item.y + tid + u * kLWG] : 0u;
+      for (uint32_t u = 0; u < kClPer; u++) cl[u] = tid + u * kLWG < ncl ? lp.clist[item.y + tid + u * kLWG] : make_uint2(0u, 0u);
       if (tid < nk) {
         s_keys[tid] = key;
         s_pn[tid] = pn;
@@ -1083,20 +1098,21 @@
     rt_stamp<TIMING>(rt, 7);
 
     const uint32_t nl = item.z - item.y;
-    auto chunk_load = [&](uint32_t l, uint4& a) {
-      const uint32_t e = l < nl ? s_clist[l] : 0u;
-      a = lp.rec16[uint64_t(e & ((1u << kChunkIdBits) - 1)) * kChunk + lane];
+    auto chunk_load = [&](uint32_t l, CRec& a) {
+      const uint32_t e = l < nl ? s_clist[l].x : 0u;
+      a = lp.rec[uint64_t(e & ((1u << kChunkIdBits) - 1)) * kChunk + lane];
     };
-    auto process = [&](uint32_t l0, const uint4 (&a16)[kLC]) {
-      uint32_t li[kLC];
+    auto process = [&](uint32_t l0, const CRec (&a12)[kLC]) {
+      uint32_t li[kLC], gb[kLC];
       bool valid[kLC];
-      uint64_t addr[kLC], ts[kLC], w[kLC];
+      uint64_t addr[kLC], w[kLC];
       XRec xr[kLC];
 #pragma unroll
       for (int j = 0; j < kLC; j++) {
         li[j] = l0 + j;
-        const uint32_t fill = li[j] < nl ? s_clist[li[j]] >> kChunkIdBits : 0u;
-        valid[j] = (uint32_t)lane < fill;
+        const uint2 ce = li[j] < nl ? s_clist[li[j]] : make_uint2(0u, 0u);
+        valid[j] = (uint32_t)lane < (ce.x >> kChunkIdBits);
+        gb[j] = __builtin_amdgcn_readfirstlane(ce.y);
       }
       if (TIMING) {
         asm volatile("s_waitcnt vmcnt(2)" ::: "memory");
@@ -1107,15 +1123,17 @@
 #pragma unroll
         for (int j = 0; j < kLC; j++)
           if (lane == 0 && li[j] < nl)
-            lp.cmatch[s_clist[li[j]] & ((1u << kChunkIdBits) - 1)] = a16[j].x ^ a16[j].y ^ a16[j].z ^ a16[j].w;
+            lp.cmatch[s_clist[li[j]].x & ((1u << kChunkIdBits) - 1)] = a12[j].x ^ a12[j].y ^ a12[j].z;
         return;
       }
       bool esc = false;
 #pragma unroll
       for (int j = 0; j < kLC; j++) {
-        xr[j] = x_decode_rel(lp.xl, a16[j]);
+        xr[j] = x_decode_rel(lp.xl, a12[j].x, a12[j].y, a12[j].z);
+        xr[j].rebase(lp.xl, gb[j]);
         esc |= valid[j] && xr[j].esc;
       }
+      if (TIMING) nesc += (uint64_t)__popcll(__ballot(esc));
       if (__ballot(esc)) {
 #pragma unroll
         for (int j = 0; j < kLC; j++)
@@ -1128,7 +1146,6 @@
 #pragma unroll
       for (int j = 0; j < kLC; j++) {
         addr[j] = xr[j].addr;
-        ts[j] = xr[j].ts;
         w[j] = valid[j] ? xr[j].w : 0ull;
       }
       rt_stamp<TIMING>(rt, 1);
@@ -1182,6 +1199,9 @@
         (void)__builtin_amdgcn_readfirstlane(__ballot(any));
       }
       rt_stamp<TIMING>(rt, 2);
+      auto exact_ts = [&](int j) -> uint64_t {
+        return raw_ts(p.data, lp.descs, xr[j].g(lp.xl), xr[j].off(lp.xl));
+      };
       int32_t erel[kLC];
       uint64_t pofs[kLC];
       uint32_t hrel[kLC], pnw[kLC], tq[kLC];
@@ -1194,7 +1214,7 @@
         older[j] = false;
         amb[j] = false;
         pnw[j] = 0;
-        tq[j] = __builtin_amdgcn_alignbit((uint32_t)(ts[j] >> 32), (uint32_t)ts[j], kPnQShift);
+        tq[j] = xr[j].tq;
         if (r[j] >= 0 && !(p.flags & kDbgLocalNoSearch)) {
           const uint4 pn = s_pn[r[j]];
           const uint2 inf = s_info[r[j]];
@@ -1220,7 +1240,7 @@
 #pragma unroll
         for (int j = 0; j < kLC; j++) {
           if (!amb[j]) continue;
-          const uint64_t fa = k0key + addr[j], ft = xr[j].esc ? ts[j] : lp.xl.tbase + ts[j];
+          const uint64_t fa = k0key + addr[j], ft = exact_ts(j);
           const uint4* gq = lp.pe_nodes + (uint64_t(q) * kPartSlots + (uint32_t)r[j]) * 2;
           const uint4 na = gq[0], nb = gq[1];
           if (entry_match(na, nb, fa, ft)) {
@@ -1266,7 +1286,7 @@
 #pragma unroll
         for (int j = 0; j < kLC; j++) {
           if (!older[j]) continue;
-          const uint64_t fa = k0key + addr[j], ft = xr[j].esc ? ts[j] : lp.xl.tbase + ts[j];
+          const uint64_t fa = k0key + addr[j], ft = exact_ts(j);
           const uint4 d = reinterpret_cast<const uint4*>(p.nodes + pi.k0 + (uint32_t)r[j])[3];
           uint64_t hist = kHistSparse, baddr = 0;
           const int32_t pos = match_older_pos(p, d.y, d.x, fa, ft, baddr, hist);
@@ -1290,7 +1310,7 @@
           mine = lane == j ? fm : mine;
           ml = lane == j ? li[j] : ml;
         }
-        if (lane < kLC && ml < nl) lp.cmatch[s_clist[ml] & ((1u << kChunkIdBits) - 1)] = mine;
+        if (lane < kLC && ml < nl) lp.cmatch[s_clist[ml].x & ((1u << kChunkIdBits) - 1)] = mine;
       }
       rt_stamp<TIMING>(rt, 3);
       const bool noobj = (p.flags & kDbgLocalNoObj) != 0;
@@ -1399,15 +1419,17 @@
             }
           }
           if (tlon) {
-            uint64_t pad[kLC];
-#pragma unroll
-            for (int j = 0; j < kLC; j++)
-              pad[j] = need[j] && erel[j] >= 0 ? p.entries[eid[j]].pad1 : kTlNone;
+            uint64_t pad[kLC], ft[kLC];
 #pragma unroll
             for (int j = 0; j < kLC; j++) {
-              const uint64_t ft = xr[j].esc ? ts[j] : lp.xl.tbase + ts[j];
+              const bool hit = need[j] && erel[j] >= 0;
+              pad[j] = hit ? p.entries[eid[j]].pad1 : kTlNone;
+              ft[j] = hit ? exact_ts(j) : 0ull;
+            }
+#pragma unroll
+            for (int j = 0; j < kLC; j++) {
               timeline_add(p, pad[j] != kTlNone,
-                           timeline_cell(p, pad[j], ft, xr[j].th, uint32_t(int(pofs[j] / kPageSize))), p.tl_rounds);
+                           timeline_cell(p, pad[j], ft[j], xr[j].th, uint32_t(int(pofs[j] / kPageSize))), p.tl_rounds);
             }
           }
           vm_drain();
@@ -1419,7 +1441,7 @@
         }
       }
     };
-    uint4 A[kLC], B[kLC];
+    CRec A[kLC], B[kLC];
     auto grab = [&]() -> uint32_t {
       uint32_t t = 0;
       if (lane == 0) t = atomicAdd(&s_cnext, (uint32_t)kLC);
@@ -1526,6 +1548,7 @@
     o[12] = rt.acc[10];
     o[13] = rt.acc[11];
     o[14] = textra;
+    o[15] = nesc;
   }
 }
 
@@ -1539,6 +1562,7 @@
   __syncthreads();
   const uint64_t k0 = uint64_t(r.chunk0[w]) * kChunk, k1 = k0 + uint64_t(r.used[w]) * kChunk;
   const uint64_t gmask = (1ull << r.gbits) - 1;
+  const uint32_t* rw = reinterpret_cast<const uint32_t*>(r.rec);
   constexpr int kU = 4;
   for (uint64_t k = k0 + tid; k < k1; k += kU * kWG) {
     uint64_t bits[kU], xw[kU];
@@ -1546,14 +1570,14 @@
     for (int u = 0; u < kU; u++) {
       const uint64_t kk = k + u * kWG;
       bits[u] = kk < k1 && (r.cmeta[kk / kChunk] >> 24) ? r.cmatch[kk / kChunk] : 0ull;
-      xw[u] = ((bits[u] >> lane) & 1) ? reinterpret_cast<const uint64_t*>(r.rec16)[2 * kk + 1] >> r.gshift : 0ull;
+      xw[u] = ((bits[u] >> lane) & 1) ? u64of(rw[kRecWords * kk + 1], rw[kRecWords * kk + 2]) >> r.gshift : 0ull;
     }
 #pragma unroll
     for (int u = 0; u < kU; u++) {
       if (!((bits[u] >> lane) & 1)) continue;
       const uint32_t g = (uint32_t)(xw[u] & gmask);
-      if (g - g0 < nl) atomicAdd(&s_found[g - g0], 1u);
-      else atomicAdd(r.bufcnt + r.nb_bufs + g, 1u);
+      if (g < nl) atomicAdd(&s_found[g], 1u);
+      else atomicAdd(r.bufcnt + r.nb_bufs + g0 + g, 1u);
     }
   }
   __syncthreads();
diff --git a/numamma_amd/csrc/nmg_route_host.hip b/numamma_amd/csrc/nmg_route_host.hip
--- a/numamma_amd/csrc/nmg_route_host.hip
+++ b/numamma_amd/csrc/nmg_route_host.hip
@@ -7,16 +7,37 @@
   return b;
 }
 
-bool route_layout(nmg_engine* h, const std::vector<BufDesc>& descs, XLayout& xl) {
+bool route_layout(nmg_engine* h, const std::vector<BufDesc>& descs, const uint32_t* ranges, uint32_t grid,
+                  XLayout& xl) {
   uint64_t maxlen = 1;
   for (const BufDesc& d : descs) maxlen = std::max<uint64_t>(maxlen, d.len);
-  xl.gbits = bits_for(descs.size() - 1);
+  uint64_t gmax = descs.size();
+  if (ranges) {
+    gmax = 1;
+    for (uint32_t w = 0; w < grid; w++) gmax = std::max<uint64_t>(gmax, ranges[w + 1] - ranges[w]);
+  }
+  xl.gbits = bits_for(gmax - 1);
   xl.obits = bits_for((maxlen - 1) / 8);
   xl.tbits = bits_for(h->T - 1);
   const uint32_t loc = xl.gbits + xl.obits + xl.tbits + 1;
-  if (loc > 48 - kMinWeightBits || xl.gbits > 31 || xl.obits > 31 || xl.tbits > 31) return false;
-  xl.wbits = std::min<uint32_t>(48 - loc, 16);
+  if (loc > kMaxLocBits || xl.gbits > 31 || xl.obits > 31 || xl.tbits > 31) return false;
+  const uint32_t avail = 32 * kRecWords - loc;
+  const uint32_t a_need = bits_for(h->route_aspan), t_need = bits_for(h->route_tqmax + 1);
+  uint32_t a = std::min(a_need, kMaxAddrBits), t = std::min(t_need, kMaxTqBits);
+  const uint32_t room = std::min<uint32_t>(64, avail - kMinWeightBits);
+  while (a + t > room) {
+    if (a > 32) a--;
+    else if (t > 24) t--;
+    else a--;
+  }
+  xl.abits = a;
+  xl.tqbits = t;
+  xl.asat = a == a_need ? h->route_aspan : ~0ull;
+  xl.tqsat = t == t_need ? h->route_tqmax + 1 : ~0ull;
+  xl.wbits = std::min<uint32_t>(avail - a - t, 16);
   xl.wesc = (1ull << xl.wbits) - 1;
+  xl.wsh = avail - xl.wbits - 32;
+  xl.lsh = xl.wsh + xl.wbits;
   xl.tbase = h->route_tbase;
   return true;
 }
@@ -33,7 +54,7 @@
   const uint64_t chunks = (bytes / kRecBytes + descs.size()) / kChunk + (uint64_t)h->num_cus * (2 * h->rt.nparts + 2);
   if (chunks >= (1ull << kChunkIdBits)) return false;
   XLayout xl;
-  return route_layout(h, descs, xl);
+  return route_layout(h, descs, nullptr, 0, xl);
 }
 bool route_eligible(nmg_engine* h) { return route_eligible(h, h->descs); }
 
@@ -56,11 +77,11 @@
   for (const BufDesc& d : descs) recs += (d.len + kRecBytes - 1) / kRecBytes;
   const size_t ovf = (size_t)((h->flags & kDbgTinyPool) ? recs : recs / 4 + std::min<uint64_t>(3 * recs, 4u << 20)) + 65536;
   RoutePool& rp = h->rpool;
-  if (tot > rp.d_cmeta.cap() || items > rp.d_items.cap() || grid > rp.d_used.cap() || ovf > rp.d_ovfx.cap()) {
+  if (tot > rp.d_cmeta.cap() || items > rp.d_items.cap() || grid > rp.d_used.cap() || ovf > rp.d_ovfrec.cap()) {
     HIP_TRY(h, hipStreamSynchronize(h->stream));
     rp = RoutePool();
     const size_t cap = std::max<size_t>(tot, 1);
-    HIP_TRY(h, rp.d_rec16.alloc(cap * kChunk));
+    HIP_TRY(h, rp.d_rec.alloc(cap * kChunk));
     HIP_TRY(h, rp.d_cmeta.alloc(cap));
     HIP_TRY(h, rp.d_cmatch.alloc(cap));
     HIP_TRY(h, rp.d_clist.alloc(cap));
@@ -71,8 +92,7 @@
     HIP_TRY(h, rp.d_pbase.alloc(kMaxParts + 1));
     HIP_TRY(h, rp.d_ctl.alloc(4));
     HIP_TRY(h, hipMemset(rp.d_ctl, 0, 4 * 4));
-    HIP_TRY(h, rp.d_ovf16.alloc(ovf));
-    HIP_TRY(h, rp.d_ovfx.alloc(ovf));
+    HIP_TRY(h, rp.d_ovfrec.alloc(ovf));
   }
   return NMG_OK;
 }
@@ -83,6 +103,7 @@
   if (rc) return rc;
   const int rc2 = stage_h2d(h, h->rpool.d_chunk0, c0.data(), (grid + 1) * 4);
   if (rc2) return rc2;
+  h->route_ranges = ranges;
   h->route_sched_key = h->rt.nparts | ((h->flags & kDbgTinyPool) ? 0x80000000u : 0u);
   return NMG_OK;
 }
@@ -90,14 +111,16 @@
 
 int route_analyze(nmg_engine* h, uint32_t nb, uint32_t grid) {
   (void)nb;
-  RouteJob job{&h->descs, h->d_data, h->d_sdescs, h->d_ranges, h->rpool.d_chunk0, grid, 0, false};
+  if (h->route_ranges.size() != (size_t)grid + 1) return fail(h, NMG_ERR_STATE, "route schedule");
+  RouteJob job{&h->descs, h->d_data, h->d_sdescs, h->d_ranges, h->rpool.d_chunk0, grid, 0, false,
+               h->route_ranges.data()};
   return route_analyze_job(h, job);
 }
 
 int route_analyze_job(nmg_engine* h, const RouteJob& job) {
   Range range("nmg_route");
   XLayout xl;
-  if (!route_layout(h, *job.descs, xl)) return fail(h, NMG_ERR_STATE, "route layout");
+  if (!route_layout(h, *job.descs, job.h_ranges, job.grid, xl)) return fail(h, NMG_ERR_STATE, "route layout");
   const uint32_t grid = job.grid;
   Params base = base_params(h, job.data, job.sdescs, job.ranges);
   base.bufcnt = h->d_bufcnt + job.index_base;
@@ -118,14 +141,13 @@
   rp.nparts = h->rt.nparts;
   rp.xl = xl;
   rp.seq0 = seq0;
-  rp.rec16 = h->rpool.d_rec16;
+  rp.rec = h->rpool.d_rec;
   rp.cmeta = h->rpool.d_cmeta;
   rp.chunk0 = job.chunk0;
   rp.used = h->rpool.d_used;
-  rp.ovf16 = h->rpool.d_ovf16;
-  rp.ovfx = h->rpool.d_ovfx;
+  rp.ovfrec = h->rpool.d_ovfrec;
   rp.ovf_cnt = h->rpool.d_ctl + 2;
-  rp.ovf_cap = (uint32_t)std::min<size_t>(h->rpool.d_ovfx.cap(), 0xffffffffu);
+  rp.ovf_cap = (uint32_t)std::min<size_t>(h->rpool.d_ovfrec.cap(), 0xffffffffu);
   if (h->flags & kDbgTinyOvf) rp.ovf_cap = std::min<uint32_t>(rp.ovf_cap, 64);
   if (h->flags & kDbgRouteTiming) {
     rc = ensure_dbg(h, (size_t)grid * (kWG / 64) * kRouteTimingWords);
@@ -142,6 +164,7 @@
   sc.pcnt = h->rpool.d_pcnt;
   sc.pbase = h->rpool.d_pbase;
   sc.clist = h->rpool.d_clist;
+  sc.ranges = job.ranges;
   sc.nparts = h->rt.nparts;
   CountParams cp;
   memset(&cp, 0, sizeof(cp));
@@ -170,7 +193,7 @@
   lp.pe_ids = h->rt.d_pe_ids;
   lp.pe_lrel = h->rt.d_pe_lrel;
   lp.pe_cmap = h->rt.d_pe_cmap;
-  lp.rec16 = h->rpool.d_rec16;
+  lp.rec = h->rpool.d_rec;
   lp.cmeta = h->rpool.d_cmeta;
   lp.clist = h->rpool.d_clist;
   lp.items = h->rpool.d_items;
@@ -198,11 +221,11 @@
     f.used = h->rpool.d_used;
     f.cmeta = h->rpool.d_cmeta;
     f.cmatch = h->rpool.d_cmatch;
-    f.rec16 = h->rpool.d_rec16;
+    f.rec = h->rpool.d_rec;
     f.bufcnt = h->d_bufcnt + job.index_base;
     f.nb_bufs = (uint32_t)h->bufcnt_stride;
     f.gbits = xl.gbits;
-    f.gshift = 16 + xl.wbits + xl.obits;
+    f.gshift = xl.lsh + xl.obits;
     HIP_TRY(h, launch_found(grid, h->stream, f));
     return NMG_OK;
   }
@@ -221,11 +244,11 @@
   f.used = h->rpool.d_used;
   f.cmeta = h->rpool.d_cmeta;
   f.cmatch = h->rpool.d_cmatch;
-  f.rec16 = h->rpool.d_rec16;
+  f.rec = h->rpool.d_rec;
   f.bufcnt = h->d_bufcnt;
   f.nb_bufs = (uint32_t)h->bufcnt_stride;
   f.gbits = h->route_xl.gbits;
-  f.gshift = 16 + h->route_xl.wbits + h->route_xl.obits;
+  f.gshift = h->route_xl.lsh + h->route_xl.obits;
   HIP_TRY(h, hipSetDevice(h->device));
   HIP_TRY(h, launch_found(h->route_grid, h->stream, f));
   return NMG_OK;
diff --git a/numamma_amd/csrc/nmg_submit.hip b/numamma_amd/csrc/nmg_submit.hip
--- a/numamma_amd/csrc/nmg_submit.hip
+++ b/numamma_amd/csrc/nmg_submit.hip
@@ -247,7 +247,8 @@
   const BufDesc* d_sdescs = reinterpret_cast<const BufDesc*>(sl.d_sched.get());
   const uint32_t* d_ranges = reinterpret_cast<const uint32_t*>(d_sdescs + nb);
   if (route) {
-    const RouteJob job{&sl.descs, sl.d_arena, d_sdescs, d_ranges, d_ranges + grid + 1, grid, index_base, true};
+    const RouteJob job{&sl.descs, sl.d_arena, d_sdescs, d_ranges, d_ranges + grid + 1, grid, index_base, true,
+                       h_ranges};
     rc = route_analyze_job(h, job);
   } else {
     rc = launch_attribution(h, sl.d_arena, d_sdescs, d_ranges, nb, grid, sl.len);
diff --git a/numamma_amd/csrc/nmg_table.hip b/numamma_amd/csrc/nmg_table.hip
--- a/numamma_amd/csrc/nmg_table.hip
+++ b/numamma_amd/csrc/nmg_table.hip
@@ -177,7 +177,7 @@
     pi.cmap = ~0u;
     uint64_t cb = ~0ull, ce = 0, cc = 0;
     while (k < K && k - pi.k0 < kPartKeys) {
-      if (k > pi.k0 && keys[k] - keys[pi.k0] >= (1ull << (kAddrBits - 1))) break;
+      if (k > pi.k0 && keys[k] - keys[pi.k0] >= (1ull << (kMaxAddrBits - 1))) break;
       const uint32_t ea = entry_off[k], eb = entry_off[k + 1];
       if (eb - pi.e0 > kPartEntries) {
         if (k == pi.k0) return NMG_OK;
@@ -226,6 +226,17 @@
   for (const DevEntry& d : dev)
     if (d.alloc) h->route_tbase = std::min<uint64_t>(h->route_tbase, d.alloc);
   if (h->route_tbase == ~0ull) h->route_tbase = 0;
+  h->route_aspan = 0;
+  h->route_tqmax = 0;
+  for (const PartInfo& pi : parts) {
+    const uint64_t f = keys[pi.k0];
+    for (uint32_t e = pi.e0; e < pi.e0 + pi.ne; e++) {
+      const DevEntry& d = dev[e];
+      if (d.free < h->route_tbase) continue;
+      if (d.end > f) h->route_aspan = std::max<uint64_t>(h->route_aspan, d.end - f);
+      h->route_tqmax = std::max<uint64_t>(h->route_tqmax, (std::max(d.alloc, d.free) - h->route_tbase) >> kPnQShift);
+    }
+  }
   const uint64_t tb = h->route_tbase;
   std::vector<uint64_t> pk((size_t)P * kPartSlots, ~0ull);
   std::vector<uint4> pn((size_t)P * kPartSlots * 2, make_uint4(0, 0, 0, 0));
```
